# Nishad-Sharma/gpuRaytracer

Measured on AMD Instinct MI355X. Metric: Msamples/sec (pixels×spp) Cornell box 1080p at 1/2/4/8 MI355X; HBM GB/s, higher is better.
Workload: dtype f32; 1 GPU; cornell_1920x1080_256spp_b3; width=1920, height=1080, spp_per_gpu=256, spp_frame=256, bounces=3, parallelism=single GPU

## Files before the change

gpuraytracer_amd/_native.py:

```python
from __future__ import annotations

import ctypes
import os

ABI_VERSION = 11
_HERE = os.path.dirname(os.path.abspath(__file__))
library_path = os.environ.get("RTPT_LIB") or os.path.join(_HERE, "librtpt.so")


class float3(ctypes.Structure):

    _fields_ = [("x", ctypes.c_float), ("y", ctypes.c_float), ("z", ctypes.c_float),
                ("_pad", ctypes.c_float)]

    def __iter__(self):
        return iter((self.x, self.y, self.z))


class float4(ctypes.Structure):
    _fields_ = [("x", ctypes.c_float), ("y", ctypes.c_float), ("z", ctypes.c_float),
                ("w", ctypes.c_float)]


class int2(ctypes.Structure):
# ... 43 lines not shown
                ("device", ctypes.c_int32)]


class RenderParamsC(ctypes.Structure):
    _fields_ = [(n, ctypes.c_uint32) for n in
                ("spp", "bounces", "sample_base", "row_start", "row_step", "row_count",
                 "accumulate", "flags")]


class SceneInfo(ctypes.Structure):
    _fields_ = [(n, ctypes.c_uint32) for n in
                ("n_triangles", "n_triangle_pairs", "n_spheres", "lds_bytes",
                 "n_sphere_nodes", "n_triangle_bvh_nodes", "n_box_clusters", "pair_free_mask",
                 "sphere_kernel_lds_bytes", "kernel_layout", "kernel_lds_bytes")]


class CreateOptions(ctypes.Structure):
    _fields_ = [("scene_layout", ctypes.c_uint32), ("lanes_per_pixel", ctypes.c_uint32),
                ("tri_bvh_build", ctypes.c_uint32), ("tri_leaf_max", ctypes.c_uint32),
                ("tri_leaf_cost", ctypes.c_float), ("sphere_leaf_max", ctypes.c_uint32),
                ("sphere_median", ctypes.c_uint32), ("walk_scheduler", ctypes.c_uint32),
                ("walk_leaf_den", ctypes.c_uint32), ("reserved", ctypes.c_uint32 * 7)]


assert ctypes.sizeof(CreateOptions) == 64

LAYOUTS = {"auto": 0, "pairs": 1, "single": 2, "global": 3, "smem": 3, "pairsmem": 4, "sorted": 5, "bvh": 6}
TRI_BUILDS = {"default": 0, "host": 1, "lbvh": 2, "gpusah": 3}
WALKS = {"auto": 0, "lockstep": 1, "free": 2, "sorted": 3}

RT_OK = 0
RT_OUT_DEVICE, RT_OUT_FP16, RT_OUT_NONE, RT_KEEP_SUM, RT_OUT_RGBA8 = 0x1, 0x2, 0x4, 0x8, 0x10
RT_RAYS_ANY, RT_RAYS_EXACT = 0x100, 0x200
RT_AOV_CENTER = 0x400
RT_RAYS_CHUNK = 2048
RT_MAX_BOUNCES = 4
RT_COMM_ID_BYTES = 128
STATUS = {0: "RT_OK", 1: "RT_ERR_INVALID_ARG", 2: "RT_ERR_NO_DEVICE", 3: "RT_ERR_OUT_OF_MEMORY",
          4: "RT_ERR_LAUNCH", 5: "RT_ERR_STATE", 6: "RT_ERR_COMM"}

class LaunchInfo(ctypes.Structure):
    _fields_ = [("kernel", ctypes.c_char * 96)] + [(n, ctypes.c_uint32) for n in
                ("lanes_per_pixel", "halton_tables", "small_index", "block_threads", "grid_x",
                 "grid_y", "lds_bytes")]

    def as_dict(self) -> dict:
        d = {k: getattr(self, k) for k, _ in self._fields_}
        d["kernel"] = self.kernel.decode()
        return d


class BuildStats(ctypes.Structure):
    _fields_ = [("tri_bvh_build", ctypes.c_uint32), ("tri_bvh_nodes", ctypes.c_uint32),
                ("tri_bvh_build_ms", ctypes.c_float), ("scene_compile_ms", ctypes.c_float),
                ("tri_bvh_temp_kib", ctypes.c_uint32)]


class TriBvhDump(ctypes.Structure):
    _fields_ = [("n_triangles", ctypes.c_uint32), ("nodes_per_layout", ctypes.c_uint32),
                ("leaf_max", ctypes.c_uint32), ("margin", ctypes.c_float),
                ("nodes", ctypes.c_void_p), ("sorted", ctypes.c_void_p),
                ("perm", ctypes.c_void_p), ("isect", ctypes.c_void_p)]


assert ctypes.sizeof(TriBvhDump) == 48

RT_UPDATE_REBUILD = 0x1


class UpdateStats(ctypes.Structure):
    _fields_ = [("tri_bvh", ctypes.c_uint32), ("updates", ctypes.c_uint32), ("compile_ms", ctypes.c_float),
                ("upload_ms", ctypes.c_float), ("tri_bvh_ms", ctypes.c_float), ("total_ms", ctypes.c_float),
                ("reserved", ctypes.c_uint32 * 2)]


assert ctypes.sizeof(UpdateStats) == 32


class TileLayout(ctypes.Structure):
    _fields_ = [("rows", ctypes.c_uint32), ("rows_max", ctypes.c_uint32),
                ("row_bytes", ctypes.c_uint64), ("tile_bytes", ctypes.c_uint64)]


class Ray(ctypes.Structure):
    _fields_ = [("origin", ctypes.c_float * 3), ("tmin", ctypes.c_float),
                ("dir", ctypes.c_float * 3), ("tmax", ctypes.c_float)]


class RayHit(ctypes.Structure):
    _fields_ = [("t", ctypes.c_float), ("id", ctypes.c_int32)]


class RayDomainInfo(ctypes.Structure):
    _fields_ = [(n, ctypes.c_float) for n in ("origin_max", "dir_len2_min", "dir_len2_max", "tmax_max")]


assert ctypes.sizeof(Ray) == 32 and ctypes.sizeof(RayHit) == 8 and Ray.dir.offset == 16


class PathParamsC(ctypes.Structure):
    _fields_ = [("spp", ctypes.c_uint32), ("bounces", ctypes.c_uint32), ("sample_base", ctypes.c_uint32),
                ("lanes_per_ray", ctypes.c_uint32), ("seed_key", ctypes.c_uint64), ("flags", ctypes.c_uint32),
                ("reserved", ctypes.c_uint32)]


assert ctypes.sizeof(PathParamsC) == 32 and PathParamsC.seed_key.offset == 16 and PathParamsC.flags.offset == 24


class AovParams(ctypes.Structure):
    _fields_ = [(n, ctypes.c_uint32) for n in
                ("spp", "sample_base", "row_start", "row_step", "row_count", "flags")]


class AovBuffers(ctypes.Structure):
    _fields_ = [("albedo", ctypes.c_void_p), ("normal_depth", ctypes.c_void_p),
                ("first_hit", ctypes.c_void_p)]


assert ctypes.sizeof(AovParams) == 24 and ctypes.sizeof(AovBuffers) == 24


class DenoiseParams(ctypes.Structure):
    _fields_ = [("iterations", ctypes.c_uint32), ("normal_power_log2", ctypes.c_uint32),
                ("sigma_luminance", ctypes.c_float), ("sigma_depth", ctypes.c_float),
                ("depth_floor", ctypes.c_float), ("flags", ctypes.c_uint32), ("reserved", ctypes.c_uint32 * 2)]


class DenoiseBuffers(ctypes.Structure):
    _fields_ = [(n, ctypes.c_void_p) for n in ("color_a", "color_b", "albedo", "normal_depth", "out")]


assert ctypes.sizeof(DenoiseParams) == 32 and ctypes.sizeof(DenoiseBuffers) == 40 and DenoiseBuffers.out.offset == 32


RT_PLAN_RELATIVE = 0x800


class PlanParams(ctypes.Structure):
    _fields_ = [("budget", ctypes.c_uint64), ("count_min", ctypes.c_uint32), ("count_max", ctypes.c_uint32),
                ("luminance_floor", ctypes.c_float), ("radius", ctypes.c_uint32), ("rows", ctypes.c_uint32),
                ("flags", ctypes.c_uint32), ("reserved", ctypes.c_uint32 * 2)]


class PlanStats(ctypes.Structure):
    _fields_ = [("weight_sum", ctypes.c_uint64), ("samples", ctypes.c_uint64),
                ("count_max_seen", ctypes.c_uint32), ("at_cap", ctypes.c_uint32),
                ("reserved", ctypes.c_uint32 * 2)]

    def as_dict(self) -> dict:
        return {k: int(getattr(self, k)) for k, _ in self._fields_ if k != "reserved"}


assert ctypes.sizeof(PlanParams) == 40 and ctypes.sizeof(PlanStats) == 32


class MisParamsC(ctypes.Structure):
    _fields_ = [(n, ctypes.c_uint32) for n in
                ("camera_rays", "mis_samples", "row_start", "row_step", "row_count", "flags")]


MATH_FNS = {n: k for k, n in enumerate(
    ("sin", "cos", "log", "exp", "pow_gamma", "sqrt", "rcp", "f2h", "h2f", "tonemap", "mis_unit",
     "halton_loop", "halton_small", "halton_tab"))}
RT_MATH_HOST, RT_MATH_DEVICE = 0, 1
RT_MATH_VALUES_MAX = 1 << 24

_P = ctypes.c_void_p
SIGNATURES = {
    "rt_create": (ctypes.c_int, [ctypes.POINTER(SceneDesc), ctypes.POINTER(_P)]),
    "rt_create_ex": (ctypes.c_int, [ctypes.POINTER(SceneDesc), ctypes.POINTER(CreateOptions),
                                    ctypes.POINTER(_P)]),
    "rt_create_options_default": (None, [ctypes.POINTER(CreateOptions)]),
    "rt_set_seeds": (ctypes.c_int, [_P, _P, ctypes.c_int32, ctypes.c_int32]),
    "rt_fill_seeds": (ctypes.c_int, [_P, ctypes.c_uint64]),
    "rt_render": (ctypes.c_int, [_P, ctypes.POINTER(RenderParamsC), _P]),
    "rt_render_async": (ctypes.c_int, [_P, ctypes.POINTER(RenderParamsC), _P, _P]),
    "rt_trace_rays": (ctypes.c_int, [_P, _P, ctypes.c_uint64, ctypes.c_uint32, _P]),
    "rt_trace_rays_async": (ctypes.c_int, [_P, _P, ctypes.c_uint64, ctypes.c_uint32, _P, _P]),
    "rt_path_params_default": (None, [ctypes.POINTER(PathParamsC)]),
    "rt_trace_paths": (ctypes.c_int, [_P, ctypes.POINTER(PathParamsC), _P, _P, ctypes.c_uint64, _P, _P]),
    "rt_trace_paths_async": (ctypes.c_int, [_P, ctypes.POINTER(PathParamsC), _P, _P, ctypes.c_uint64, _P, _P, _P]),
    "rt_render_aov": (ctypes.c_int, [_P, ctypes.POINTER(AovParams), ctypes.POINTER(AovBuffers)]),
    "rt_render_aov_async": (ctypes.c_int, [_P, ctypes.POINTER(AovParams), ctypes.POINTER(AovBuffers), _P]),
    "rt_denoise_params_default": (None, [ctypes.POINTER(DenoiseParams)]),
    "rt_denoise": (ctypes.c_int, [_P, ctypes.POINTER(DenoiseParams), ctypes.POINTER(DenoiseBuffers)]),
    "rt_denoise_async": (ctypes.c_int, [_P, ctypes.POINTER(DenoiseParams), ctypes.POINTER(DenoiseBuffers), _P]),
    "rt_render_counts": (ctypes.c_int, [_P, ctypes.POINTER(RenderParamsC), _P, _P, _P]),
    "rt_render_counts_async": (ctypes.c_int, [_P, ctypes.POINTER(RenderParamsC), _P, _P, _P, _P]),
    "rt_plan_params_default": (None, [ctypes.POINTER(PlanParams)]),
    "rt_plan_samples": (ctypes.c_int, [_P, ctypes.POINTER(PlanParams), _P, _P, _P, ctypes.POINTER(PlanStats)]),
    "rt_plan_samples_async": (ctypes.c_int, [_P, ctypes.POINTER(PlanParams), _P, _P, _P, _P, _P]),
    "rt_plan_samples_host": (ctypes.c_int, [ctypes.c_int32, ctypes.POINTER(PlanParams), _P, _P, _P,
                                            ctypes.POINTER(PlanStats)]),
    "rt_debug_ray_domain": (ctypes.c_int, [ctypes.POINTER(SceneDesc), ctypes.POINTER(RayDomainInfo)]),
    "rt_last_kernel_ms": (ctypes.c_int, [_P, ctypes.POINTER(ctypes.c_float)]),
    "rt_destroy": (ctypes.c_int, [_P]),
    "rt_last_launch": (ctypes.c_int, [_P, ctypes.POINTER(LaunchInfo)]),
    "rt_build_info": (ctypes.c_int, [_P, ctypes.POINTER(BuildStats)]),
    "rt_debug_tri_bvh": (ctypes.c_int, [_P, ctypes.POINTER(TriBvhDump)]),
    "rt_debug_tri_bvh_host": (ctypes.c_int, [ctypes.POINTER(SceneDesc), ctypes.POINTER(CreateOptions),
                                             ctypes.POINTER(TriBvhDump)]),
    "rt_update_scene": (ctypes.c_int, [_P, ctypes.POINTER(SceneDesc), ctypes.c_uint32]),
    "rt_update_info": (ctypes.c_int, [_P, ctypes.POINTER(UpdateStats)]),
    "rt_debug_tri_bvh_refit_host": (ctypes.c_int, [ctypes.POINTER(SceneDesc), ctypes.POINTER(CreateOptions),
                                                   ctypes.POINTER(SceneDesc), ctypes.POINTER(TriBvhDump)]),
    "rt_math_selfcheck": (ctypes.c_int, [ctypes.POINTER(ctypes.c_uint64)]),
    "rt_debug_math_values": (ctypes.c_int, [ctypes.c_uint32, ctypes.c_uint32, _P, ctypes.c_uint64, _P]),
    "rt_debug_math_sums": (ctypes.c_int, [ctypes.c_uint32, ctypes.c_uint32, ctypes.c_uint32, ctypes.c_uint64,
                                          ctypes.c_uint32, ctypes.c_uint32, _P]),
    "rt_comm_unique_id": (ctypes.c_int, [_P]),
    "rt_comm_init": (ctypes.c_int, [_P, ctypes.c_int32, ctypes.c_int32, _P]),
    "rt_render_gather": (ctypes.c_int, [_P, ctypes.POINTER(RenderParamsC), _P, _P]),
    "rt_comm_info": (ctypes.c_int, [_P, ctypes.POINTER(ctypes.c_int32), ctypes.POINTER(ctypes.c_int32)]),
    "rt_tile_layout": (ctypes.c_int, [ctypes.c_int32, ctypes.c_int32, ctypes.c_int32, ctypes.c_int32,
                                      ctypes.c_uint32, ctypes.POINTER(TileLayout)]),
    "rt_place_tiles": (ctypes.c_int, [_P, _P, ctypes.c_int32, ctypes.c_uint32, _P, _P]),
    "rt_place_tiles_host": (ctypes.c_int, [_P, ctypes.c_int32, ctypes.c_int32, ctypes.c_int32,
                                           ctypes.c_uint32, _P]),
    "rt_build_sha": (ctypes.c_char_p, []),
    "rt_debug_stats": (ctypes.c_int, [_P, _P, ctypes.c_int]),
    "rt_last_error": (ctypes.c_char_p, [_P]),
    "rt_status_string": (ctypes.c_char_p, [ctypes.c_int]),
    "rt_abi_version": (ctypes.c_int, []),
    "rt_seed_splitmix": (None, [ctypes.c_uint64, _P, ctypes.c_size_t]),
    "rt_scene_cornell_box": (ctypes.c_int, [ctypes.c_int32, ctypes.c_int32,
                                            ctypes.POINTER(CameraGPU),
                                            ctypes.POINTER(MaterialGPU),
                                            ctypes.POINTER(float3),
                                            ctypes.POINTER(SquareLightGPU),
                                            ctypes.POINTER(ctypes.c_uint32)]),
    "rt_scene_random_spheres": (ctypes.c_int, [ctypes.c_int32, ctypes.c_int32, ctypes.c_uint32,
                                               ctypes.c_uint64, ctypes.POINTER(CameraGPU),
                                               ctypes.POINTER(MaterialGPU),
                                               ctypes.POINTER(float3),
                                               ctypes.POINTER(SquareLightGPU),
                                               ctypes.POINTER(ctypes.c_uint32),
                                               ctypes.POINTER(SphereGPU)]),
    "rt_render_mis": (ctypes.c_int, [_P, ctypes.POINTER(MisParamsC), _P, _P]),
    "rt_scene_cornell_box_mis": (ctypes.c_int, [ctypes.c_int32, ctypes.c_int32,
                                                ctypes.POINTER(CameraGPU),
                                                ctypes.POINTER(MaterialGPU),
                                                ctypes.POINTER(float3),
                                                ctypes.POINTER(SquareLightGPU),
                                                ctypes.POINTER(ctypes.c_uint32)]),
    "rt_tonemap_rgba8": (None, [_P, ctypes.c_size_t, _P]),
    "rt_scene_describe": (ctypes.c_int, [ctypes.POINTER(SceneDesc), ctypes.POINTER(SceneInfo)]),
    "rt_scene_describe_ex": (ctypes.c_int, [ctypes.POINTER(SceneDesc), ctypes.POINTER(CreateOptions),
                                            ctypes.POINTER(SceneInfo)]),
    "rt_debug_camera_candidates": (ctypes.c_int, [ctypes.POINTER(SceneDesc)] + [ctypes.c_int32] * 4 + [_P]),
    "rt_debug_shadow_candidates": (ctypes.c_int, [ctypes.POINTER(SceneDesc)] + [ctypes.c_int32] * 4 +
                                   [_P, ctypes.POINTER(ctypes.c_int32)]),
    "rt_debug_cluster_kinds": (ctypes.c_int, [ctypes.POINTER(SceneDesc), ctypes.POINTER(ctypes.c_uint32),
                                              ctypes.c_uint32, ctypes.POINTER(ctypes.c_uint32)]),
    "rt_debug_light_mask": (ctypes.c_int, [ctypes.POINTER(SceneDesc), ctypes.POINTER(ctypes.c_uint64), _P,
                                           ctypes.c_uint32]),
    "rt_debug_halton_table": (ctypes.c_int, [_P, ctypes.c_uint32, ctypes.POINTER(ctypes.c_uint32), _P, _P]),
    "rt_debug_halton_table_device": (ctypes.c_int, [_P, _P, ctypes.c_uint32]),
}


class RtError(RuntimeError):

    def __init__(self, status: int, message: str):
        super().__init__(f"{STATUS.get(status, status)}: {message}")
        self.status = status


def _preload_hip_runtime():
    if os.environ.get("RTPT_SYSTEM_HIP") == "1":
        return
    import importlib.util
    spec = importlib.util.find_spec("torch")
    if spec is None or not spec.submodule_search_locations:
        return
    for d in spec.submodule_search_locations:
        cand = os.path.join(d, "lib", "libamdhip64.so")
        if os.path.exists(cand):
            ctypes.CDLL(cand, mode=ctypes.RTLD_GLOBAL)
            return


def _load():
    if not os.path.exists(library_path):
        raise ImportError(
            f"{library_path} is missing: build the HIP extension first "
            "(`make` or `python -c 'import __graft_entry__ as g; g.build()'`). "
            "There is no CPU fallback.")
    _preload_hip_runtime()
    handle = ctypes.CDLL(library_path)
    for name, (res, args) in SIGNATURES.items():
        fn = getattr(handle, name)
        fn.restype = res
        fn.argtypes = args
    if handle.rt_abi_version() != ABI_VERSION:
        raise ImportError(f"librtpt.so ABI {handle.rt_abi_version()} != {ABI_VERSION}")
    if not os.environ.get("RTPT_LIB"):
        from .srchash import have_sources, kernel_source_sha
        built = handle.rt_build_sha().decode()
        if not have_sources() or built == "unknown":
            import warnings
            warnings.warn(f"{library_path}: source hash not checked (library hash {built!r}, "
                          f"sources {'present' if have_sources() else 'absent'})")
        elif built != kernel_source_sha():
            raise ImportError(f"{library_path} was built from other sources (hash {built}, "
                              f"tree {kernel_source_sha()}): rebuild it with `make`")
    return handle


lib = _load()
```

gpuraytracer_amd/csrc/rt_api.cpp:

```cpp
#include <rccl/rccl.h>

#include <stdio.h>
#include <stdlib.h>
#include <string.h>

#include <chrono>
#include <new>
#include <vector>

#include "rt_api_internal.hpp"

using namespace rtapi;

namespace {

class DevBuf {
public:
    DevBuf() = default;
    DevBuf(DevBuf&& o) noexcept : p_(o.p_), bytes_(o.bytes_) { o.p_ = nullptr; o.bytes_ = 0; }
    DevBuf& operator=(DevBuf&& o) noexcept {
        std::swap(p_, o.p_);
        std::swap(bytes_, o.bytes_);
        return *this;
    }
    ~DevBuf() { reset(); }

    void reset() {
        if (p_) (void)hipFree(p_);
        p_ = nullptr;
        bytes_ = 0;
    }
    hipError_t reserve(size_t bytes) { return bytes_ >= bytes ? hipSuccess : allocate(bytes); }
    hipError_t resize_exact(size_t bytes) { return bytes_ == bytes ? hipSuccess : allocate(bytes); }
    void adopt(void* p, size_t bytes) {
        reset();
        p_ = p;
        bytes_ = bytes;
    }
    template <typename T>
    T* as() const { return static_cast<T*>(p_); }
    size_t bytes() const { return bytes_; }
    explicit operator bool() const { return p_ != nullptr; }

private:
    hipError_t allocate(size_t bytes) {
        reset();
        if (bytes == 0) return hipSuccess;
        const hipError_t e = hipMalloc(&p_, bytes);
        if (e != hipSuccess) p_ = nullptr;
        else bytes_ = bytes;
        return e;
    }
    void* p_ = nullptr;
    size_t bytes_ = 0;
};

template <typename H, hipError_t (*Destroy)(H)>
struct Owned {
    H h = nullptr;
    Owned() = default;
    Owned(const Owned&) = delete;
    Owned& operator=(const Owned&) = delete;
    ~Owned() { if (h) (void)Destroy(h); }
    operator H() const { return h; }
};
using Stream = Owned<hipStream_t, hipStreamDestroy>;
using Event = Owned<hipEvent_t, hipEventDestroy>;

enum SceneArray {
    kTriIsect, kTriShade, kPairIsect, kClusters, kSphLds, kSphLdsId,
    kSphBox,
    kSphIsect, kSphShade, kSphNodes, kSphPerm, kMisShade, kSceneArrays
};

}

struct rt_ctx {
    int device = 0;
    Stream stream;
    Event ev0, ev1;
    Event ev_u0, ev_u1;
    Event ev_tiles;
    rt::CompiledScene scene;
    DevBuf d_scene[kSceneArrays];
    DevBuf d_tri_nodes;
    uint32_t tri_build = kDefaultTriBuild;
    DevBuf d_tri_sorted, d_tri_perm;
    DevBuf d_refit;
    uint32_t tri_bvh_nodes = 0;
    rt::SceneTables tab{};
    bool sph_compact = false;
    uint64_t light_mask = 0;
    DevBuf d_halton_tab;
    uint32_t tri_bvh_build_used = 0;
    uint32_t tri_leaf_max = 1;
    float tri_bvh_build_ms = 0.0f;
    size_t tri_bvh_temp_bytes = 0;
    float scene_compile_ms = 0.0f;
    DevBuf d_mis_tab;
    uint32_t mis_tab_S = 0;
    DevBuf d_mis_part;
    DevBuf d_out, d_out8;
    DevBuf d_rays, d_hits;
    DevBuf d_ray_seeds, d_radiance;
    DevBuf d_aov[3];
    DevBuf d_den[6];
    DevBuf d_counts, d_totals;
    DevBuf d_plan_in[2];
    DevBuf d_plan;
    DevBuf d_seeds;
    bool seeds_ready = false;
    uint32_t seed_max = 0xFFFFFFFFu;
    DevBuf d_sum;
    bool sum_valid = false;
    uint32_t sum_row_start = 0, sum_row_step = 0, sum_row_count = 0;
    uint32_t sum_first = 0, sum_samples = 0;
    bool sum_counts = false;
    bool timed = false;
    rt::LaunchInfo launch{};
    bool launched = false;
    ncclComm_t comm = nullptr;
    int rank = 0, world = 1;
    DevBuf d_tile;
    DevBuf d_gather;
    bool tiles_pending = false;
    uint32_t lanes = 0;
    rt::SceneMem scene_mem = rt::SceneMem::kAuto;
    uint32_t walk = 0;
    uint32_t walk_leaf_den = 0;
    uint32_t tri_leaf_opt = rt::kTriLeafMax;
    double tri_leaf_cost = 1.0;
    rt::BuildOptions build_opt;
    std::string broken;
    bool updated = false;
    rt_update_stats update{};
    std::string err;

    ~rt_ctx() {
        if (tiles_pending) (void)hipEventSynchronize(ev_tiles);
        if (comm) (void)ncclCommDestroy(comm);
    }
};

namespace {
thread_local std::string g_create_err = "no error";
}

int rtapi::fail(rt_ctx* ctx, int status, const std::string& msg) {
    if (ctx)
        ctx->err = msg;
    else
        g_create_err = msg;
    return status;
}

namespace {

int nccl_fail(rt_ctx* ctx, const char* what, ncclResult_t r) {
    return fail(ctx, RT_ERR_COMM, std::string(what) + ": " + ncclGetErrorString(r));
}

struct DeviceGuard {
    int prev = -1;
    explicit DeviceGuard(int dev) {
        if (hipGetDevice(&prev) != hipSuccess) prev = -1;
        if (prev != dev) (void)hipSetDevice(dev);
    }
    ~DeviceGuard() {
        int cur = -1;
        if (prev >= 0 && hipGetDevice(&cur) == hipSuccess && cur != prev) (void)hipSetDevice(prev);
    }
};

int reserve(rt_ctx* c, DevBuf& b, size_t bytes, const char* what) {
    const hipError_t e = b.reserve(bytes);
    return e == hipSuccess ? RT_OK : hip_fail(c, RT_ERR_OUT_OF_MEMORY, what, e);
}

int copy_down(rt_ctx* c, void* host, const void* dev, size_t bytes, hipStream_t stream, const char* what) {
    const hipError_t e = hipMemcpyAsync(host, dev, bytes, hipMemcpyDeviceToHost, stream);
    return e == hipSuccess ? RT_OK : hip_fail(c, RT_ERR_LAUNCH, what, e);
}

hipError_t upload(DevBuf& b, const void* src, size_t bytes, hipStream_t s) {
    hipError_t e = b.resize_exact(bytes);
    if (e != hipSuccess || bytes == 0) return e;
    if ((e = hipMemcpyAsync(b.as<void>(), src, bytes, hipMemcpyHostToDevice, s)) != hipSuccess) return e;
    return hipStreamSynchronize(s);
}

template <typename F>
int timed_launch(rt_ctx* c, hipStream_t stream, const char* what, rt::LaunchInfo* info, F launch) {
    (void)hipEventRecord(c->ev0, stream);
    const hipError_t e = launch(info);
    if (e != hipSuccess) return hip_fail(c, RT_ERR_LAUNCH, (std::string(what) + " launch").c_str(), e);
    if (info) c->launched = true;
    (void)hipEventRecord(c->ev1, stream);
    c->timed = true;
    return RT_OK;
}

template <typename P>
void set_camera(P* K, const rt::CamConst& cam) {
    memcpy(K->cam_pos, cam.pos, sizeof(K->cam_pos));
    memcpy(K->cam_u, cam.u, sizeof(K->cam_u));
    memcpy(K->cam_v, cam.v, sizeof(K->cam_v));
    memcpy(K->cam_w, cam.w, sizeof(K->cam_w));
    K->halfW = cam.halfW;
    K->halfH = cam.halfH;
    K->W = cam.W;
    K->H = cam.H;
}

uint32_t halton_max_index(const rt_ctx* c, uint32_t sample_base, uint32_t spp) {
    const uint64_t imax = (uint64_t)c->seed_max + sample_base + (spp ? spp - 1u : 0u);
    return imax > 0xFFFFFFFFull ? 0xFFFFFFFFu : (uint32_t)imax;
}

int check_out_format(rt_ctx* c, uint32_t flags) {
    if ((flags & RT_OUT_FP16) && (flags & RT_OUT_RGBA8))
        return fail(c, RT_ERR_INVALID_ARG, "RT_OUT_FP16 and RT_OUT_RGBA8 are exclusive");
    return RT_OK;
}

void set_tables(rt::KParams* K, const rt::SceneTables& t) {
    K->tri_isect = t.tri_isect;
    K->pair_isect = t.pair_isect;
    K->clusters = t.clusters;
    K->sph_isect = t.sph_isect;
    K->sph_nodes = t.sph_nodes;
    K->sph_perm = t.sph_perm;
    K->sph_box = t.sph_box;
    K->tri_nodes = t.tri_nodes;
    K->tri_sorted = t.tri_sorted;
    K->tri_perm = t.tri_perm;
    K->nT = t.nT;
    K->nP = t.nP;
    K->nS = t.nS;
    K->nN = t.nN;
    K->nTN = t.nTN;
    K->nC = t.nC;
    K->pair_free = t.pair_free;
}

void set_scene(rt::KParams* K, const rt_ctx* c) {
    memset(K, 0, sizeof(*K));
    set_tables(K, c->tab);
    K->tri_shade = c->d_scene[kTriShade].as<float4>();
    K->light_mask = c->light_mask;
    K->halton_tab = c->d_halton_tab.as<float>();
    K->sph_lds = c->sph_compact ? c->d_scene[kSphLds].as<uint32_t>() : nullptr;
    K->sph_lds_id = c->d_scene[kSphLdsId].as<uint16_t>();
    K->sph_shade = c->d_scene[kSphShade].as<float4>();
    K->nE = c->scene.sph_lds_entries;
    memcpy(K->light_center, c->scene.light.center, sizeof(K->light_center));
    {
        uint32_t by, bz;
        memcpy(&by, &K->light_center[1], 4);
        memcpy(&bz, &K->light_center[2], 4);
        K->light_plain = (by != 0x80000000u && bz != 0x80000000u) ? 1u : 0u;
    }
    memcpy(K->light_color, c->scene.light.color, sizeof(K->light_color));
}

hipError_t upload_scene(rt_ctx* c) {
    const rt::CompiledScene& s = c->scene;
    hipError_t e = hipSuccess;
    auto put = [&](SceneArray k, const auto& v) {
        const size_t bytes = v.size() * sizeof(v[0]);
        DevBuf& b = c->d_scene[k];
        if (e == hipSuccess) e = b.resize_exact(bytes);
        if (e == hipSuccess && bytes)
            e = hipMemcpyAsync(b.as<void>(), v.data(), bytes, hipMemcpyHostToDevice, c->stream);
    };
    put(kTriIsect, s.tri_isect);
    put(kTriShade, s.tri_shade);
    put(kPairIsect, s.pair_isect);
    put(kClusters, s.clusters);
    put(kSphLds, s.sph_lds);
    put(kSphLdsId, s.sph_lds_id);
    put(kSphBox, s.sph_box);
    put(kSphIsect, s.sph_isect);
    put(kSphShade, s.sph_shade);
    put(kSphNodes, s.sph_nodes);
    put(kSphPerm, s.sph_perm);
    put(kMisShade, s.mis_shade);
    return e != hipSuccess ? e : hipStreamSynchronize(c->stream);
}

bool needs_tri_bvh(const rt_ctx* c) { return rtapi::needs_tri_bvh(scene_counts(c->scene, 0), c->scene_mem); }

void free_tri_bvh(rt_ctx* c) {
    c->d_tri_nodes.reset();
    c->d_tri_sorted.reset();
    c->d_tri_perm.reset();
    c->d_refit.reset();
    c->tri_bvh_nodes = 0;
    c->tri_bvh_build_used = 0;
    c->tri_bvh_temp_bytes = 0;
}

int build_tri_bvh(rt_ctx* c, std::string* msg) {
    using clk = std::chrono::steady_clock;
    free_tri_bvh(c);
    const rt::CompiledScene& s = c->scene;
    const uint32_t nT = (uint32_t)s.tri_isect.size();
    const size_t nn = 2 * (size_t)nT - 1;
    const auto t_build = clk::now();
    hipError_t e;
    if (c->tri_build == RT_TRI_BVH_GPU_SAH || c->tri_build == RT_TRI_BVH_GPU_LBVH) {
        if ((e = c->d_tri_nodes.reserve(rt::kTriCompactLayouts * nn * sizeof(uint4))) != hipSuccess ||
            (e = c->d_tri_sorted.reserve(3 * (size_t)nT * sizeof(float4))) != hipSuccess ||
            (e = c->d_tri_perm.reserve((size_t)nT * sizeof(uint32_t))) != hipSuccess) {
            *msg = std::string("hipMalloc(triangle BVH): ") + hipGetErrorString(e);
            return RT_ERR_OUT_OF_MEMORY;
        }
    }
    const float4* d_tri = c->d_scene[kTriIsect].as<float4>();
    uint4* d_nodes = c->d_tri_nodes.as<uint4>();
    float4* d_sorted = c->d_tri_sorted.as<float4>();
    uint32_t* d_perm = c->d_tri_perm.as<uint32_t>();
    if (c->tri_build == RT_TRI_BVH_GPU_SAH) {
        uint32_t total = 0;
        size_t temp = 0;
        if ((e = rt::build_tri_gsah(d_tri, nT, s.margin, c->tri_leaf_opt, c->tri_leaf_cost, d_nodes, d_sorted, d_perm,
                                    &total, &temp, c->stream)) != hipSuccess) {
            *msg = std::string("triangle BVH build: ") + hipGetErrorString(e);
            return (e == hipErrorInvalidValue) ? RT_ERR_INVALID_ARG
                   : (e == hipErrorOutOfMemory) ? RT_ERR_OUT_OF_MEMORY : RT_ERR_LAUNCH;
        }
        c->tri_bvh_nodes = total;
        c->tri_bvh_temp_bytes = temp;
    } else if (c->tri_build == RT_TRI_BVH_GPU_LBVH) {
        if ((e = rt::build_tri_lbvh(d_tri, nT, s.tri_lo, s.tri_hi, s.margin, d_nodes, d_sorted, d_perm, c->stream)) !=
            hipSuccess) {
            *msg = std::string("triangle BVH build: ") + hipGetErrorString(e);
            return (e == hipErrorInvalidValue) ? RT_ERR_INVALID_ARG : RT_ERR_LAUNCH;
        }
        c->tri_bvh_nodes = (uint32_t)nn;
    } else {
        std::vector<uint32_t> nodes, perm;
        std::vector<rt::TriIsect> sorted;
        if (!rt::build_tri_sah(s.tri_isect, s.margin, &nodes, &sorted, &perm, c->tri_leaf_opt, c->tri_leaf_cost)) {
            *msg = "triangle BVH build: too many triangles (2^24)";
            return RT_ERR_INVALID_ARG;
        }
        if ((e = upload(c->d_tri_nodes, nodes.data(), nodes.size() * sizeof(uint32_t), c->stream)) != hipSuccess ||
            (e = upload(c->d_tri_sorted, sorted.data(), sorted.size() * sizeof(rt::TriIsect), c->stream)) != hipSuccess ||
            (e = upload(c->d_tri_perm, perm.data(), perm.size() * sizeof(uint32_t), c->stream)) != hipSuccess) {
            *msg = std::string("triangle BVH upload: ") + hipGetErrorString(e);
            return RT_ERR_OUT_OF_MEMORY;
        }
        c->tri_bvh_nodes = (uint32_t)(nodes.size() / (4 * rt::kTriCompactLayouts));
    }
    c->tri_leaf_max = c->tri_build == RT_TRI_BVH_GPU_LBVH ? 1u : tri_leaf_clamp(c->tri_leaf_opt);
    c->tri_bvh_build_used = c->tri_build;
    c->tri_bvh_build_ms = std::chrono::duration<float, std::milli>(clk::now() - t_build).count();
    return RT_OK;
}

void finish_scene(rt_ctx* c) {
    c->sph_compact = rt::sphere_compact_usable(c->scene);
    c->light_mask = rt::light_mask(c->scene);
    rt::SceneTables& t = c->tab = scene_counts(c->scene, c->tri_bvh_nodes);
    t.tri_isect = c->d_scene[kTriIsect].as<float4>();
    t.pair_isect = c->d_scene[kPairIsect].as<float4>();
    t.clusters = c->d_scene[kClusters].as<float4>();
    t.sph_isect = c->d_scene[kSphIsect].as<float4>();
    t.sph_nodes = c->d_scene[kSphNodes].as<float4>();
    t.sph_perm = c->d_scene[kSphPerm].as<uint32_t>();
    t.sph_box = c->sph_compact ? c->d_scene[kSphBox].as<uint4>() : nullptr;
    t.tri_nodes = c->d_tri_nodes.as<uint4>();
    t.tri_sorted = c->d_tri_sorted.as<float4>();
    t.tri_perm = c->d_tri_perm.as<uint32_t>();
}

bool resolve_rows(const rt_ctx* c, uint32_t row_start, uint32_t row_step, uint32_t row_count, uint32_t* start,
                  uint32_t* step, uint32_t* count) {
    const uint32_t H = (uint32_t)c->scene.cam.H;
    *start = row_start;
    *step = row_step ? row_step : 1u;
    if (*start >= H) return false;
    const uint32_t avail = (H - 1u - *start) / *step + 1u;
    *count = row_count ? row_count : avail;
    return *count <= avail;
}

struct CountsArgs {
    const uint32_t* counts;
    uint32_t* totals;
};

int render_impl(rt_ctx* c, const rt_render_params* p, void* out, bool out_is_device,
                hipStream_t stream, bool sync, const CountsArgs* ca = nullptr) {
    if (!p) return fail(c, RT_ERR_INVALID_ARG, "params is null");
    if (ca && !ca->counts) return fail(c, RT_ERR_INVALID_ARG, "rt_render_counts: counts is null");
    if (!c->broken.empty()) return fail(c, RT_ERR_STATE, c->broken);
    if (p->bounces > RT_MAX_BOUNCES)
        return fail(c, RT_ERR_INVALID_ARG,
                    "bounces > 4: Halton dimensions would leave primes[24] (sampling.metal:97)");
    if (!c->seeds_ready) return fail(c, RT_ERR_STATE, "seeds not set (rt_set_seeds/rt_fill_seeds)");
    uint32_t start, step, count;
    if (!resolve_rows(c, p->row_start, p->row_step, p->row_count, &start, &step, &count))
        return fail(c, RT_ERR_INVALID_ARG, "row partition outside the frame");
    const bool want_out = !(p->flags & RT_OUT_NONE);
    const bool keep_sum = (p->flags & RT_KEEP_SUM) != 0;
    const bool sums = keep_sum || p->accumulate;
    if (want_out && !out) return fail(c, RT_ERR_INVALID_ARG, "out is null");
    if (p->accumulate) {
        const bool rows_same = c->sum_valid && c->sum_row_start == start && c->sum_row_step == step &&
                               c->sum_row_count == count;
        if (ca) {
            if (!rows_same || c->sum_first != p->sample_base)
                return fail(c, RT_ERR_STATE,
                            "rt_render_counts: accumulate: context sum does not start at sample_base for these rows "
                            "(render with RT_KEEP_SUM first)");
        } else {
            if (rows_same && c->sum_counts)
                return fail(c, RT_ERR_STATE,
                            "accumulate: context sum holds per-pixel sample counts (rt_render_counts): "
                            "continue it with rt_render_counts");
            if (!rows_same || (uint64_t)c->sum_first + c->sum_samples != (uint64_t)p->sample_base)
                return fail(c, RT_ERR_STATE,
                            "accumulate: context sum does not end at sample_base for these rows "
                            "(render with RT_KEEP_SUM first)");
        }
    }
    const uint64_t total = (uint64_t)(p->accumulate ? c->sum_samples : 0u) + p->spp;
    if (ca) {
        if (total > (1ull << 24))
            return fail(c, RT_ERR_INVALID_ARG,
                        "rt_render_counts: the bound of the per-pixel totals (the caps spp of the calls into this "
                        "sum) must stay <= 2^24");
    } else if (total == 0 || total > 0xFFFFFFFFull) {
        return fail(c, RT_ERR_INVALID_ARG, "samples in the sum must be in [1, 2^32)");
    }

    const size_t pixels = (size_t)count * (size_t)c->scene.cam.W;
    int st;
    if ((st = check_out_format(c, p->flags)) != RT_OK) return st;
    const size_t out_bytes = pixels * pixel_bytes(p->flags);
    if (sums) {
        if (c->d_sum.bytes() < pixels * sizeof(float4)) c->sum_valid = false;
        if ((st = reserve(c, c->d_sum, pixels * sizeof(float4), "hipMalloc(sum)")) != RT_OK) return st;
    }
    void* kout = want_out ? out : nullptr;
    if (want_out && !out_is_device) {
        if ((st = reserve(c, c->d_out, out_bytes, "hipMalloc(out staging)")) != RT_OK) return st;
        kout = c->d_out.as<void>();
    }
    const uint32_t* kcounts = ca ? ca->counts : nullptr;
    uint32_t* ktotals = ca ? ca->totals : nullptr;
    if (ca && !out_is_device) {
        if ((st = reserve(c, c->d_counts, pixels * sizeof(uint32_t), "hipMalloc(counts staging)")) != RT_OK) return st;
        const hipError_t e = hipMemcpyAsync(c->d_counts.as<void>(), ca->counts, pixels * sizeof(uint32_t),
                                            hipMemcpyHostToDevice, stream);
        if (e != hipSuccess) return hip_fail(c, RT_ERR_LAUNCH, "hipMemcpyAsync(counts)", e);
        kcounts = c->d_counts.as<uint32_t>();
        if (ca->totals) {
            if ((st = reserve(c, c->d_totals, pixels * sizeof(uint32_t), "hipMalloc(totals staging)")) != RT_OK)
                return st;
            ktotals = c->d_totals.as<uint32_t>();
        }
    }

    rt::KParams K;
    set_scene(&K, c);
    K.seeds = c->d_seeds.as<uint32_t>();
    K.sum = sums ? c->d_sum.as<float4>() : nullptr;
    K.out = kout;
    set_camera(&K, c->scene.cam);
    K.spp = p->spp;
    K.sample_base = p->sample_base;
    K.row_start = start;
    K.row_step = step;
    K.row_count = count;
    K.accumulate = p->accumulate ? 1u : 0u;
    K.samples_total = (uint32_t)total;
    K.flags = ((p->flags & RT_OUT_FP16) ? rt::kOutFp16 : 0u) | ((p->flags & RT_OUT_RGBA8) ? rt::kOutRgba8 : 0u);
    K.lanes = c->lanes;
    K.walk = c->walk;
    K.walk_leaf_den = c->walk_leaf_den;
    K.max_index = halton_max_index(c, p->sample_base, ca ? (uint32_t)total : p->spp);

    if (keep_sum && !p->accumulate) c->sum_valid = false;
    if ((st = timed_launch(c, stream, ca ? "path_counts" : "path_trace", &c->launch, [&](rt::LaunchInfo* info) {
             return ca ? rt::launch_path_counts(K, kcounts, ktotals, p->bounces, c->scene_mem, stream, info)
                       : rt::launch_path_trace(K, p->bounces, c->scene_mem, stream, info);
         })) != RT_OK)
        return st;
    if (sums) {
        c->sum_valid = true;
        c->sum_row_start = start;
        c->sum_row_step = step;
        c->sum_row_count = count;
        if (!p->accumulate) c->sum_first = p->sample_base;
        c->sum_samples = (uint32_t)total;
        c->sum_counts = ca != nullptr;
    }
    if (ca && ca->totals && !out_is_device &&
        (st = copy_down(c, ca->totals, ktotals, pixels * sizeof(uint32_t), stream, "hipMemcpyAsync(totals)")) != RT_OK)
        return st;
    if (want_out && !out_is_device &&
        (st = copy_down(c, out, kout, out_bytes, stream, "hipMemcpyAsync(out)")) != RT_OK)
        return st;
    if (sync) {
        hipError_t e;
        if ((e = hipStreamSynchronize(stream)) != hipSuccess)
            return hip_fail(c, RT_ERR_LAUNCH, "path_trace execution", e);
        uint32_t short_end = 0;
        if (rt::lds_check_result(&short_end) == hipSuccess && short_end)
            return fail(c, RT_ERR_LAUNCH, "LDS overflow: staged records end at byte " + std::to_string(short_end) +
                                              ", past the dispatch's dynamic LDS");
    }
    return RT_OK;
}

int place_tiles_impl(rt_ctx* c, const void* gathered, uint32_t N, uint32_t flags, void* frame,
                     hipStream_t stream) {
    const uint32_t W = (uint32_t)c->scene.cam.W, H = (uint32_t)c->scene.cam.H;
    const TileLayout L = tile_layout(W, H, N, 0, flags);
    const bool dev = (flags & RT_OUT_DEVICE) != 0;
    const size_t frame_bytes = (size_t)H * L.row_bytes;
    void* dst = frame;
    int st;
    if (!dev) {
        if ((st = reserve(c, c->d_out, frame_bytes, "hipMalloc(frame staging)")) != RT_OK) return st;
        dst = c->d_out.as<void>();
    }
    hipError_t e = rt::launch_place_tiles(gathered, dst, L.row_bytes, L.tile_bytes, H, N, stream);
    if (e != hipSuccess) return hip_fail(c, RT_ERR_LAUNCH, "place_tiles launch", e);
    if (!dev) {
        if ((e = hipStreamSynchronize(stream)) != hipSuccess ||
            (e = hipMemcpyAsync(frame, dst, frame_bytes, hipMemcpyDeviceToHost, stream)) != hipSuccess ||
            (e = hipStreamSynchronize(stream)) != hipSuccess)
            return hip_fail(c, RT_ERR_LAUNCH, "frame copy to host", e);
    }
    return RT_OK;
}

int render_gather_impl(rt_ctx* c, const rt_render_params* p, void* frame, hipStream_t stream) {
    if (!p) return fail(c, RT_ERR_INVALID_ARG, "params is null");
    if (!c->comm) return fail(c, RT_ERR_STATE, "no communicator (rt_comm_init)");
    if (p->row_start || p->row_step > 1 || p->row_count)
        return fail(c, RT_ERR_INVALID_ARG, "rt_render_gather partitions the rows itself: "
                                           "params must name the whole frame (row_start 0, "
                                           "row_step 0 or 1, row_count 0)");
    int st;
    if ((st = check_out_format(c, p->flags)) != RT_OK) return st;
    const bool want_out = !(p->flags & RT_OUT_NONE);
    const bool dev = (p->flags & RT_OUT_DEVICE) != 0;
    if (want_out && c->rank == 0 && !frame) return fail(c, RT_ERR_INVALID_ARG, "frame is null on rank 0");
    const uint32_t H = (uint32_t)c->scene.cam.H, W = (uint32_t)c->scene.cam.W, N = (uint32_t)c->world;
    const TileLayout L = tile_layout(W, H, N, (uint32_t)c->rank, p->flags);
    hipError_t e;
    if (c->tiles_pending && (e = hipStreamWaitEvent(stream, c->ev_tiles, 0)) != hipSuccess)
        return hip_fail(c, RT_ERR_LAUNCH, "hipStreamWaitEvent(previous gather)", e);
    if (want_out && (st = reserve(c, c->d_tile, L.tile_bytes, "hipMalloc(tile)")) != RT_OK) return st;
    if (L.rows > 0) {
        rt_render_params q = *p;
        q.row_start = (uint32_t)c->rank;
        q.row_step = N;
        q.row_count = L.rows;
        q.flags = p->flags | RT_OUT_DEVICE;
        if ((st = render_impl(c, &q, c->d_tile.as<void>(), true, stream, false)) != RT_OK) return st;
    }
    if (!want_out) return RT_OK;
    if (c->rank == 0 && (st = reserve(c, c->d_gather, L.tile_bytes * N, "hipMalloc(gather)")) != RT_OK) return st;
    ncclResult_t r = ncclGather(c->d_tile.as<void>(), c->rank == 0 ? c->d_gather.as<void>() : nullptr, L.tile_bytes,
                                ncclUint8, 0, c->comm, stream);
    if (r != ncclSuccess) return nccl_fail(c, "ncclGather", r);
    if (c->rank == 0 && (st = place_tiles_impl(c, c->d_gather.as<void>(), N, p->flags, frame, stream)) != RT_OK)
        return st;
    if ((e = hipEventRecord(c->ev_tiles, stream)) != hipSuccess)
        return hip_fail(c, RT_ERR_LAUNCH, "hipEventRecord(gather)", e);
    c->tiles_pending = true;
    if (!dev) {
        e = hipStreamSynchronize(stream);
        if (e != hipSuccess) return hip_fail(c, RT_ERR_COMM, "render+gather execution", e);
    }
    return RT_OK;
}

int mis_table(rt_ctx* c, uint32_t S) {
    if (c->d_mis_tab && c->mis_tab_S == S) return RT_OK;
    std::vector<float> t((size_t)S * 12u);
    for (uint32_t i = 0; i < S; ++i) {
        float* q = &t[(size_t)i * 12u];
        q[0] = halton_host(i, 0);
        q[1] = halton_host(i, 1);
        q[2] = 0.0f;
        q[3] = 0.0f;
        q[4] = halton_host(i + S, 2);
        q[5] = halton_host(i + S, 3);
        q[6] = halton_host(i, 6);
        q[7] = halton_host(i, 7);
        q[8] = halton_host(i + 2 * S, 4);
        q[9] = halton_host(i + 2 * S, 5);
        q[10] = halton_host(i + S, 6);
        q[11] = halton_host(i + S, 7);
    }
    c->d_mis_tab.reset();
    c->mis_tab_S = 0;
    hipError_t e = upload(c->d_mis_tab, t.data(), t.size() * sizeof(float), c->stream);
    if (e != hipSuccess) return hip_fail(c, RT_ERR_OUT_OF_MEMORY, "MIS table upload", e);
    c->mis_tab_S = S;
    return RT_OK;
}

int render_mis_impl(rt_ctx* c, const rt_mis_params* p, float* out, uint8_t* out8) {
    if (!p) return fail(c, RT_ERR_INVALID_ARG, "params is null");
    if (!c->broken.empty()) return fail(c, RT_ERR_STATE, c->broken);
    if (!out && !out8) return fail(c, RT_ERR_INVALID_ARG, "both outputs are null");
    if (!c->scene.sph_isect.empty())
        return fail(c, RT_ERR_INVALID_ARG,
                    "the MIS integrator traces triangle scenes only (shaders.metal:459-509)");
    if (c->scene.tri_isect.empty()) return fail(c, RT_ERR_INVALID_ARG, "scene has no triangles");
    if (p->camera_rays == 0) return fail(c, RT_ERR_INVALID_ARG, "camera_rays must be >= 1");
    if (p->mis_samples < 3 || p->mis_samples / 3u > (1u << 20))
        return fail(c, RT_ERR_INVALID_ARG, "mis_samples must be in [3, 3 * 2^20]");
    uint32_t start, step, count;
    if (!resolve_rows(c, p->row_start, p->row_step, p->row_count, &start, &step, &count))
        return fail(c, RT_ERR_INVALID_ARG, "row partition outside the frame");
    const uint32_t S = p->mis_samples / 3u;
    int st = mis_table(c, S);
    if (st != RT_OK) return st;
    const bool dev = (p->flags & RT_OUT_DEVICE) != 0;
    const size_t pixels = (size_t)count * (size_t)c->scene.cam.W;
    float4* kout = reinterpret_cast<float4*>(out);
    uchar4* kout8 = reinterpret_cast<uchar4*>(out8);
    if (out && !dev) {
        if ((st = reserve(c, c->d_out, pixels * 16u, "hipMalloc(out staging)")) != RT_OK) return st;
        kout = c->d_out.as<float4>();
    }
    if (out8 && !dev) {
        if ((st = reserve(c, c->d_out8, pixels * 4u, "hipMalloc(out8 staging)")) != RT_OK) return st;
        kout8 = c->d_out8.as<uchar4>();
    }

    rt::MisParams K;
    memset(&K, 0, sizeof(K));
    K.tab = c->tab;
    K.mis_shade = c->d_scene[kMisShade].as<float4>();
// ... 315 lines not shown
    K.count_min = p->count_min;
    K.count_max = p->count_max;
    K.luminance_floor = p->luminance_floor;
    K.radius = p->radius;
    K.W = c->scene.cam.W;
    K.rows = (int32_t)rows;
    K.flags = p->flags & RT_PLAN_RELATIVE;
    if ((st = timed_launch(c, stream, "plan", &c->launch,
                           [&](rt::LaunchInfo* info) { return rt::launch_plan(K, stream, info); })) != RT_OK)
        return st;
    if (!dev && (st = copy_down(c, counts, kcounts, cnt_bytes, stream, "hipMemcpyAsync(counts)")) != RT_OK) return st;
    if (stats) {
        e = hipMemcpyAsync(stats, K.acc, sizeof(rt_plan_stats), sync ? hipMemcpyDeviceToHost : hipMemcpyDeviceToDevice,
                           stream);
        if (e != hipSuccess) return hip_fail(c, RT_ERR_LAUNCH, "hipMemcpyAsync(plan stats)", e);
    }
    if (sync && (e = hipStreamSynchronize(stream)) != hipSuccess)
        return hip_fail(c, RT_ERR_LAUNCH, "plan execution", e);
    return RT_OK;
}

}

extern "C" {

const char* rt_last_error(const rt_ctx* ctx) {
    return ctx ? ctx->err.c_str() : g_create_err.c_str();
}

int rt_create(const rt_scene_desc* d, rt_ctx** out_ctx) { return rt_create_ex(d, nullptr, out_ctx); }

int rt_create_ex(const rt_scene_desc* d, const rt_create_options* opt, rt_ctx** out_ctx) {
    if (!out_ctx) return fail(nullptr, RT_ERR_INVALID_ARG, "out_ctx is null");
    *out_ctx = nullptr;
    if (!d) return fail(nullptr, RT_ERR_INVALID_ARG, "scene desc is null");
    if (!d->camera) return fail(nullptr, RT_ERR_INVALID_ARG, "camera is null");
    if (!d->square_lights || d->n_square_lights < 1)
        return fail(nullptr, RT_ERR_INVALID_ARG, "square_lights[0] is required (raytrace.metal:22)");
    Resolved ro;
    const char* why = nullptr;
    if (!resolve_options(opt, &ro, &why)) return fail(nullptr, RT_ERR_INVALID_ARG, why);
    int count = 0;
    hipError_t e = hipGetDeviceCount(&count);
    if (e != hipSuccess || count <= 0)
        return fail(nullptr, RT_ERR_NO_DEVICE,
                    std::string("no HIP device: ") + (e != hipSuccess ? hipGetErrorString(e) : "count 0"));
    if (d->device < 0 || d->device >= count)
        return fail(nullptr, RT_ERR_NO_DEVICE, "device ordinal out of range");

    rt_ctx* c = new (std::nothrow) rt_ctx();
    if (!c) return fail(nullptr, RT_ERR_OUT_OF_MEMORY, "host allocation");
    c->device = d->device;
    c->lanes = ro.lanes;
    c->tri_build = ro.tri_build;
    c->scene_mem = ro.mem;
    c->walk = ro.walk;
    c->walk_leaf_den = ro.walk_leaf_den;
    c->tri_leaf_opt = ro.tri_leaf_max;
    c->tri_leaf_cost = ro.tri_leaf_cost;
    c->build_opt = ro.build;
    DeviceGuard g(c->device);
    const char* err = nullptr;
    using clk = std::chrono::steady_clock;
    const auto t_compile = clk::now();
    if (!compile_desc(d, ro.build, &c->scene, &err)) {
        delete c;
        return fail(nullptr, RT_ERR_INVALID_ARG, err);
    }
    c->scene_compile_ms = std::chrono::duration<float, std::milli>(clk::now() - t_compile).count();
    int status = RT_OK;
    std::string msg;
    do {
        if ((e = hipStreamCreateWithFlags(&c->stream.h, hipStreamNonBlocking)) != hipSuccess) {
            status = RT_ERR_NO_DEVICE; msg = std::string("hipStreamCreate: ") + hipGetErrorString(e); break;
        }
        if ((e = hipEventCreate(&c->ev0.h)) != hipSuccess || (e = hipEventCreate(&c->ev1.h)) != hipSuccess ||
            (e = hipEventCreateWithFlags(&c->ev_tiles.h, hipEventDisableTiming)) != hipSuccess) {
            status = RT_ERR_NO_DEVICE; msg = std::string("hipEventCreate: ") + hipGetErrorString(e); break;
        }
        if ((e = upload_scene(c)) != hipSuccess) {
            status = RT_ERR_OUT_OF_MEMORY; msg = std::string("scene upload: ") + hipGetErrorString(e); break;
        }
        if (needs_tri_bvh(c) && (status = build_tri_bvh(c, &msg)) != RT_OK) break;
        const size_t npx = (size_t)c->scene.cam.W * (size_t)c->scene.cam.H;
        if ((e = c->d_seeds.reserve(npx * sizeof(uint32_t))) != hipSuccess) {
            status = RT_ERR_OUT_OF_MEMORY; msg = std::string("hipMalloc(seeds): ") + hipGetErrorString(e); break;
        }
        if ((e = c->d_halton_tab.resize_exact(sizeof(float) * rt::kHaltonTabLdsFloats)) != hipSuccess) {
            status = RT_ERR_OUT_OF_MEMORY; msg = std::string("hipMalloc(halton tables): ") + hipGetErrorString(e); break;
        }
        if ((e = rt::launch_fill_halton_tables(c->d_halton_tab.as<float>(), c->stream)) != hipSuccess ||
            (e = hipStreamSynchronize(c->stream)) != hipSuccess) {
            status = RT_ERR_LAUNCH; msg = std::string("halton tables: ") + hipGetErrorString(e); break;
        }
    } while (0);
    if (status != RT_OK) {
        delete c;
        return fail(nullptr, status, msg);
    }
    finish_scene(c);
    *out_ctx = c;
    return RT_OK;
}

int rt_destroy(rt_ctx* c) {
    if (!c) return RT_OK;
    DeviceGuard g(c->device);
    delete c;
    return RT_OK;
}

int rt_update_scene(rt_ctx* c, const rt_scene_desc* d, uint32_t flags) {
    static_assert(sizeof(rt_update_stats) == 32, "rt_update_stats layout");
    if (!c) return fail(nullptr, RT_ERR_INVALID_ARG, "ctx is null");
    if (!d) return fail(c, RT_ERR_INVALID_ARG, "rt_update_scene: scene is null");
    if (!d->camera) return fail(c, RT_ERR_INVALID_ARG, "rt_update_scene: camera is null");
    if (!d->square_lights || d->n_square_lights < 1)
        return fail(c, RT_ERR_INVALID_ARG, "rt_update_scene: square_lights[0] is required");
    if (flags & ~(uint32_t)RT_UPDATE_REBUILD) return fail(c, RT_ERR_INVALID_ARG, "rt_update_scene: unknown bits in flags");
    if (d->n_triangles != c->scene.tri_isect.size())
        return fail(c, RT_ERR_INVALID_ARG, "rt_update_scene: n_triangles differs from the context's (" +
                                               std::to_string(c->scene.tri_isect.size()) + ")");
    if (d->n_spheres != c->scene.sph_shade.size())
        return fail(c, RT_ERR_INVALID_ARG, "rt_update_scene: n_spheres differs from the context's (" +
                                               std::to_string(c->scene.sph_shade.size()) + ")");
    if (d->camera->resolution.x != c->scene.cam.W || d->camera->resolution.y != c->scene.cam.H)
        return fail(c, RT_ERR_INVALID_ARG, "rt_update_scene: camera resolution differs from the context's");
    if (d->device != c->device) return fail(c, RT_ERR_INVALID_ARG, "rt_update_scene: device differs from the context's");
    using clk = std::chrono::steady_clock;
    auto ms_since = [](clk::time_point t) { return std::chrono::duration<float, std::milli>(clk::now() - t).count(); };
    const auto t_all = clk::now();
    rt::CompiledScene next;
    const char* err = nullptr;
    if (!compile_desc(d, c->build_opt, &next, &err))
        return fail(c, RT_ERR_INVALID_ARG, std::string("rt_update_scene: ") + err);
    if (next.tri_isect.size() != c->scene.tri_isect.size() || next.sph_shade.size() != c->scene.sph_shade.size())
        return fail(c, RT_ERR_INVALID_ARG, "rt_update_scene: the compiled scene changed its primitive counts");
    rt_update_stats st{};
    st.compile_ms = ms_since(t_all);

    DeviceGuard g(c->device);
    auto broken = [&](int status, const std::string& what) {
        c->broken = "the context holds a half-updated scene (" + what + "): rt_update_scene must succeed first";
        return fail(c, status, "rt_update_scene: " + what);
    };
    hipError_t e;
    if (c->tiles_pending) (void)hipEventSynchronize(c->ev_tiles);
    if ((e = hipStreamSynchronize(c->stream)) != hipSuccess) return broken(RT_ERR_LAUNCH, std::string("stream: ") + hipGetErrorString(e));
    if (!c->ev_u0.h && ((e = hipEventCreate(&c->ev_u0.h)) != hipSuccess || (e = hipEventCreate(&c->ev_u1.h)) != hipSuccess))
        return broken(RT_ERR_OUT_OF_MEMORY, std::string("hipEventCreate: ") + hipGetErrorString(e));
    c->broken = "rt_update_scene in progress";
    c->sum_valid = false;
    c->scene = std::move(next);
    const auto t_up = clk::now();
    if ((e = upload_scene(c)) != hipSuccess) return broken(RT_ERR_OUT_OF_MEMORY, std::string("scene upload: ") + hipGetErrorString(e));
    st.upload_ms = ms_since(t_up);

    const bool need = needs_tri_bvh(c), have = c->tri_bvh_build_used && c->d_tri_nodes;
    const auto t_bvh = clk::now();
    if (need && have && !(flags & RT_UPDATE_REBUILD)) {
        uint32_t* table = c->d_refit.as<uint32_t>();
        bool table_made = false;
        e = rt::refit_tri_bvh(c->d_scene[kTriIsect].as<float4>(), (uint32_t)c->scene.tri_isect.size(), c->scene.margin,
                              c->d_tri_nodes.as<uint4>(), c->tri_bvh_nodes, c->d_tri_sorted.as<float4>(),
                              c->d_tri_perm.as<uint32_t>(), &table, &table_made, c->ev_u0, c->ev_u1, c->stream);
        if (table_made) c->d_refit.adopt(table, rt::tri_refit_table_bytes(c->tri_bvh_nodes));
        if (e == hipSuccess) e = hipStreamSynchronize(c->stream);
        if (e != hipSuccess)
            return broken(e == hipErrorOutOfMemory ? RT_ERR_OUT_OF_MEMORY : RT_ERR_LAUNCH,
                          std::string("triangle BVH refit: ") + hipGetErrorString(e));
        uint32_t bad = 0;
        if (table_made && ((e = rt::refit_format_errors(table, c->tri_bvh_nodes, &bad)) != hipSuccess || bad))
            return broken(RT_ERR_LAUNCH, "triangle BVH refit: the tree is outside the format of its builders");
        if ((e = hipEventElapsedTime(&st.tri_bvh_ms, c->ev_u0, c->ev_u1)) != hipSuccess)
            return broken(RT_ERR_LAUNCH, std::string("hipEventElapsedTime: ") + hipGetErrorString(e));
        st.tri_bvh = 1;
    } else if (need) {
        std::string msg;
        const int status = build_tri_bvh(c, &msg);
        if (status != RT_OK) return broken(status == RT_ERR_INVALID_ARG ? RT_ERR_LAUNCH : status, msg);
        st.tri_bvh_ms = ms_since(t_bvh);
        st.tri_bvh = 2;
        c->scene_compile_ms = st.compile_ms;
    } else {
        free_tri_bvh(c);
    }
    finish_scene(c);
    c->broken.clear();
    st.updates = c->update.updates + 1;
    st.total_ms = ms_since(t_all);
    c->update = st;
    c->updated = true;
    return RT_OK;
}

int rt_update_info(const rt_ctx* c, rt_update_stats* info) {
    if (!c || !info) return fail(nullptr, RT_ERR_INVALID_ARG, "null argument");
    if (!c->updated)
        return fail(const_cast<rt_ctx*>(c), RT_ERR_STATE, "rt_update_info: no successful rt_update_scene on this context yet");
    *info = c->update;
    return RT_OK;
}

int rt_set_seeds(rt_ctx* c, const uint32_t* seeds, int32_t width, int32_t height) {
    if (!c) return fail(nullptr, RT_ERR_INVALID_ARG, "ctx is null");
    if (!seeds) return fail(c, RT_ERR_INVALID_ARG, "seeds is null");
    if (width != c->scene.cam.W || height != c->scene.cam.H)
        return fail(c, RT_ERR_INVALID_ARG, "seed texture size must equal the camera resolution");
    DeviceGuard g(c->device);
    const size_t bytes = (size_t)width * (size_t)height * sizeof(uint32_t);
    hipError_t e = hipMemcpyAsync(c->d_seeds.as<void>(), seeds, bytes, hipMemcpyHostToDevice, c->stream);
    if (e == hipSuccess) e = hipStreamSynchronize(c->stream);
    if (e != hipSuccess) return hip_fail(c, RT_ERR_LAUNCH, "seed upload", e);
    uint32_t mx = 0;
    for (size_t k = 0, n = (size_t)width * (size_t)height; k < n; ++k) mx = seeds[k] > mx ? seeds[k] : mx;
    c->seed_max = mx;
    c->seeds_ready = true;
    return RT_OK;
}

int rt_fill_seeds(rt_ctx* c, uint64_t key) {
    if (!c) return fail(nullptr, RT_ERR_INVALID_ARG, "ctx is null");
    DeviceGuard g(c->device);
    const uint64_t n = (uint64_t)c->scene.cam.W * (uint64_t)c->scene.cam.H;
    hipError_t e = rt::launch_fill_seeds(c->d_seeds.as<uint32_t>(), key, n, c->stream);
    if (e == hipSuccess) e = hipStreamSynchronize(c->stream);
    if (e != hipSuccess) return hip_fail(c, RT_ERR_LAUNCH, "fill_seeds", e);
    c->seed_max = 0xFFFFFu;
    c->seeds_ready = true;
    return RT_OK;
}

int rt_render(rt_ctx* c, const rt_render_params* p, void* out) {
    if (!c) return fail(nullptr, RT_ERR_INVALID_ARG, "ctx is null");
    DeviceGuard g(c->device);
    const bool dev = p && (p->flags & RT_OUT_DEVICE);
    return render_impl(c, p, out, dev, c->stream, true);
}

int rt_render_async(rt_ctx* c, const rt_render_params* p, void* out_device, void* hip_stream) {
    if (!c) return fail(nullptr, RT_ERR_INVALID_ARG, "ctx is null");
    DeviceGuard g(c->device);
    return render_impl(c, p, out_device, true, (hipStream_t)hip_stream, false);
}

int rt_render_mis(rt_ctx* ctx, const rt_mis_params* params, float* out_rgba32f, uint8_t* out_rgba8) {
    if (!ctx) return fail(nullptr, RT_ERR_INVALID_ARG, "ctx is null");
    DeviceGuard g(ctx->device);
    return render_mis_impl(ctx, params, out_rgba32f, out_rgba8);
}

int rt_trace_rays(rt_ctx* c, const rt_ray* rays, uint64_t n, uint32_t flags, rt_ray_hit* hits) {
    if (!c) return fail(nullptr, RT_ERR_INVALID_ARG, "ctx is null");
    DeviceGuard g(c->device);
    return trace_rays_impl(c, rays, n, flags, hits, (flags & RT_OUT_DEVICE) != 0, c->stream, true);
}

int rt_trace_rays_async(rt_ctx* c, const rt_ray* rays_dev, uint64_t n, uint32_t flags, rt_ray_hit* hits_dev,
                        void* hip_stream) {
    if (!c) return fail(nullptr, RT_ERR_INVALID_ARG, "ctx is null");
    DeviceGuard g(c->device);
    return trace_rays_impl(c, rays_dev, n, flags, hits_dev, true, (hipStream_t)hip_stream, false);
}

int rt_trace_paths(rt_ctx* c, const rt_path_params* p, const rt_ray* rays, const uint32_t* seeds, uint64_t n,
                   float* radiance, rt_ray_hit* first_hits) {
    if (!c) return fail(nullptr, RT_ERR_INVALID_ARG, "ctx is null");
    DeviceGuard g(c->device);
    return trace_paths_impl(c, p, rays, seeds, n, radiance, first_hits, p && (p->flags & RT_OUT_DEVICE), c->stream,
                            true);
}

int rt_trace_paths_async(rt_ctx* c, const rt_path_params* p, const rt_ray* rays_dev, const uint32_t* seeds_dev,
                         uint64_t n, float* radiance_dev, rt_ray_hit* first_hits_dev, void* hip_stream) {
    if (!c) return fail(nullptr, RT_ERR_INVALID_ARG, "ctx is null");
    DeviceGuard g(c->device);
    return trace_paths_impl(c, p, rays_dev, seeds_dev, n, radiance_dev, first_hits_dev, true, (hipStream_t)hip_stream,
                            false);
}

int rt_render_aov(rt_ctx* c, const rt_aov_params* p, const rt_aov_buffers* b) {
    if (!c) return fail(nullptr, RT_ERR_INVALID_ARG, "ctx is null");
    DeviceGuard g(c->device);
    return render_aov_impl(c, p, b, p && (p->flags & RT_OUT_DEVICE), c->stream, true);
}

int rt_render_aov_async(rt_ctx* c, const rt_aov_params* p, const rt_aov_buffers* b_dev, void* hip_stream) {
    if (!c) return fail(nullptr, RT_ERR_INVALID_ARG, "ctx is null");
    DeviceGuard g(c->device);
    return render_aov_impl(c, p, b_dev, true, (hipStream_t)hip_stream, false);
}

int rt_denoise(rt_ctx* c, const rt_denoise_params* p, const rt_denoise_buffers* b) {
    if (!c) return fail(nullptr, RT_ERR_INVALID_ARG, "ctx is null");
    DeviceGuard g(c->device);
    return denoise_impl(c, p, b, p && (p->flags & RT_OUT_DEVICE), c->stream, true);
}

int rt_denoise_async(rt_ctx* c, const rt_denoise_params* p, const rt_denoise_buffers* b_dev, void* hip_stream) {
    if (!c) return fail(nullptr, RT_ERR_INVALID_ARG, "ctx is null");
    DeviceGuard g(c->device);
    return denoise_impl(c, p, b_dev, true, (hipStream_t)hip_stream, false);
}

int rt_render_counts(rt_ctx* c, const rt_render_params* p, const uint32_t* counts, void* out, uint32_t* totals) {
    if (!c) return fail(nullptr, RT_ERR_INVALID_ARG, "ctx is null");
    DeviceGuard g(c->device);
    const CountsArgs ca{counts, totals};
    return render_impl(c, p, out, p && (p->flags & RT_OUT_DEVICE), c->stream, true, &ca);
}

int rt_render_counts_async(rt_ctx* c, const rt_render_params* p, const uint32_t* counts_dev, void* out_dev,
                           uint32_t* totals_dev, void* hip_stream) {
    if (!c) return fail(nullptr, RT_ERR_INVALID_ARG, "ctx is null");
    DeviceGuard g(c->device);
    const CountsArgs ca{counts_dev, totals_dev};
    return render_impl(c, p, out_dev, true, (hipStream_t)hip_stream, false, &ca);
}

int rt_plan_samples(rt_ctx* c, const rt_plan_params* p, const float* first, const float* all, uint32_t* counts,
                    rt_plan_stats* stats) {
    if (!c) return fail(nullptr, RT_ERR_INVALID_ARG, "ctx is null");
    DeviceGuard g(c->device);
    return plan_impl(c, p, first, all, counts, stats, p && (p->flags & RT_OUT_DEVICE), c->stream, true);
}

int rt_plan_samples_async(rt_ctx* c, const rt_plan_params* p, const float* first_dev, const float* all_dev,
                          uint32_t* counts_dev, rt_plan_stats* stats_dev, void* hip_stream) {
    if (!c) return fail(nullptr, RT_ERR_INVALID_ARG, "ctx is null");
    DeviceGuard g(c->device);
    return plan_impl(c, p, first_dev, all_dev, counts_dev, stats_dev, true, (hipStream_t)hip_stream, false);
}

int rt_last_kernel_ms(rt_ctx* c, float* ms) {
    if (!c || !ms) return fail(c, RT_ERR_INVALID_ARG, "null argument");
    if (!c->timed) return fail(c, RT_ERR_STATE, "no render or ray query yet");
    DeviceGuard g(c->device);
    hipError_t e = hipEventSynchronize(c->ev1);
    if (e == hipSuccess) e = hipEventElapsedTime(ms, c->ev0, c->ev1);
    if (e != hipSuccess) return hip_fail(c, RT_ERR_LAUNCH, "hipEventElapsedTime", e);
    return RT_OK;
}

int rt_comm_unique_id(uint8_t id[RT_COMM_ID_BYTES]) {
    if (!id) return fail(nullptr, RT_ERR_INVALID_ARG, "id is null");
    static_assert(sizeof(ncclUniqueId) == RT_COMM_ID_BYTES, "ncclUniqueId size");
    ncclUniqueId u;
    const ncclResult_t r = ncclGetUniqueId(&u);
    if (r != ncclSuccess) return nccl_fail(nullptr, "ncclGetUniqueId", r);
    memcpy(id, &u, sizeof(u));
    return RT_OK;
}

int rt_comm_init(rt_ctx* c, int32_t rank, int32_t world, const uint8_t id[RT_COMM_ID_BYTES]) {
    if (!c) return fail(nullptr, RT_ERR_INVALID_ARG, "ctx is null");
    if (!id) return fail(c, RT_ERR_INVALID_ARG, "id is null");
    if (world < 1 || rank < 0 || rank >= world)
        return fail(c, RT_ERR_INVALID_ARG, "need 0 <= rank < world");
    if (c->comm) return fail(c, RT_ERR_STATE, "context already has a communicator");
    DeviceGuard g(c->device);
    ncclUniqueId u;
    memcpy(&u, id, sizeof(u));
    ncclComm_t comm = nullptr;
    const ncclResult_t r = ncclCommInitRank(&comm, world, u, rank);
    if (r != ncclSuccess) return nccl_fail(c, "ncclCommInitRank", r);
    c->comm = comm;
    c->rank = rank;
    c->world = world;
    return RT_OK;
}

int rt_render_gather(rt_ctx* c, const rt_render_params* p, void* frame, void* hip_stream) {
    if (!c) return fail(nullptr, RT_ERR_INVALID_ARG, "ctx is null");
    DeviceGuard g(c->device);
    hipStream_t s = (hipStream_t)hip_stream;
    return render_gather_impl(c, p, frame, s);
}

int rt_comm_info(const rt_ctx* c, int32_t* count, int32_t* rank) {
    if (!c || !count || !rank) return fail(nullptr, RT_ERR_INVALID_ARG, "null argument");
    rt_ctx* m = const_cast<rt_ctx*>(c);
    if (!c->comm) return fail(m, RT_ERR_STATE, "rt_comm_info: no communicator (rt_comm_init first)");
    int n = 0, r = 0;
    ncclResult_t res = ncclCommCount(c->comm, &n);
    if (res != ncclSuccess) return nccl_fail(m, "ncclCommCount", res);
    res = ncclCommUserRank(c->comm, &r);
    if (res != ncclSuccess) return nccl_fail(m, "ncclCommUserRank", res);
    *count = n;
    *rank = r;
    return RT_OK;
}

int rt_place_tiles(rt_ctx* c, const void* gathered_device, int32_t world, uint32_t flags, void* frame,
                   void* hip_stream) {
    if (!c) return fail(nullptr, RT_ERR_INVALID_ARG, "ctx is null");
    if (!gathered_device || !frame || world < 1) return fail(c, RT_ERR_INVALID_ARG, "null buffer or world < 1");
    if (const int st = check_out_format(c, flags)) return st;
    DeviceGuard g(c->device);
    hipStream_t s = (hipStream_t)hip_stream;
    return place_tiles_impl(c, gathered_device, (uint32_t)world, flags, frame, s);
}

int rt_build_info(const rt_ctx* c, rt_build_stats* info) {
    if (!c || !info) return fail(nullptr, RT_ERR_INVALID_ARG, "null argument");
    memset(info, 0, sizeof(*info));
    info->tri_bvh_build = c->tri_bvh_build_used;
    info->tri_bvh_nodes = c->tri_bvh_nodes;
    info->tri_bvh_build_ms = c->tri_bvh_build_ms;
    info->scene_compile_ms = c->scene_compile_ms;
    info->tri_bvh_temp_kib = (uint32_t)((c->tri_bvh_temp_bytes + 1023) / 1024);
    return RT_OK;
}

int rt_debug_tri_bvh(const rt_ctx* c, rt_tri_bvh_dump* dump) {
    if (!c || !dump) return fail(nullptr, RT_ERR_INVALID_ARG, "null argument");
    if (!c->broken.empty()) return fail(const_cast<rt_ctx*>(c), RT_ERR_STATE, c->broken);
    if (!c->tri_bvh_build_used || !c->d_tri_nodes) return RT_ERR_STATE;
    const size_t nT = c->scene.tri_isect.size(), nn = c->tri_bvh_nodes;
    dump->n_triangles = (uint32_t)nT;
    dump->nodes_per_layout = (uint32_t)nn;
    dump->leaf_max = c->tri_leaf_max;
    dump->margin = c->scene.margin;
    DeviceGuard g(c->device);
    const struct { void* dst; const DevBuf& src; size_t bytes; } copies[4] = {
        {dump->nodes, c->d_tri_nodes, rt::kTriCompactLayouts * nn * sizeof(uint4)},
        {dump->sorted, c->d_tri_sorted, nT * sizeof(rt::TriIsect)},
        {dump->perm, c->d_tri_perm, nT * sizeof(uint32_t)},
        {dump->isect, c->d_scene[kTriIsect], nT * sizeof(rt::TriIsect)}};
    for (const auto& cp : copies) {
        if (!cp.dst) continue;
        const hipError_t e = hipMemcpy(cp.dst, cp.src.as<void>(), cp.bytes, hipMemcpyDeviceToHost);
        if (e != hipSuccess) return RT_ERR_LAUNCH;
    }
    return RT_OK;
}

int rt_debug_halton_table_device(const rt_ctx* c, float* table, uint32_t capacity) {
    if (!c || !table) return fail(nullptr, RT_ERR_INVALID_ARG, "null argument");
    if (capacity < rt::kHaltonTabLdsFloats)
        return fail(const_cast<rt_ctx*>(c), RT_ERR_INVALID_ARG, "rt_debug_halton_table_device: capacity below the table's size");
    if (!c->d_halton_tab) return RT_ERR_STATE;
    DeviceGuard g(c->device);
    const hipError_t e =
        hipMemcpy(table, c->d_halton_tab.as<void>(), sizeof(float) * rt::kHaltonTabLdsFloats, hipMemcpyDeviceToHost);
    return e == hipSuccess ? RT_OK : RT_ERR_LAUNCH;
}

int rt_last_launch(const rt_ctx* c, rt_launch_info* info) {
    if (!c || !info) return fail(nullptr, RT_ERR_INVALID_ARG, "null argument");
    if (!c->launched) return RT_ERR_STATE;
    memset(info, 0, sizeof(*info));
    static_assert(sizeof(info->kernel) == sizeof(c->launch.kernel), "kernel name buffer");
    memcpy(info->kernel, c->launch.kernel, sizeof(info->kernel));
    info->kernel[sizeof(info->kernel) - 1] = 0;
    info->lanes_per_pixel = c->launch.lanes;
    info->halton_tables = c->launch.tables;
    info->small_index = c->launch.small;
    info->block_threads = c->launch.threads;
    info->grid_x = c->launch.grid_x;
    info->grid_y = c->launch.grid_y;
    info->lds_bytes = c->launch.lds;
    return RT_OK;
}

int rt_debug_stats(rt_ctx* c, uint64_t* out, int n) {
    if (!c || !out || n <= 0) return fail(c, RT_ERR_INVALID_ARG, "null argument");
    DeviceGuard g(c->device);
    hipError_t e = rt::read_debug_stats(reinterpret_cast<unsigned long long*>(out), n);
    if (e == hipErrorNotSupported) return fail(c, RT_ERR_STATE, "not an RT_STATS build");
    if (e != hipSuccess) return hip_fail(c, RT_ERR_LAUNCH, "read stats", e);
    return RT_OK;
}

#ifndef RT_SRC_SHA
#define RT_SRC_SHA "unknown"
#endif
const char* rt_build_sha(void) { return RT_SRC_SHA; }

}
```

gpuraytracer_amd/csrc/rt_api_host.cpp:

```cpp
#include <string.h>

#include <thread>
#include <vector>

#include "rt_api_internal.hpp"
#include "rt_beam.hpp"
#include "rt_halton.hpp"
#include "rt_mathcheck.hpp"
#include "rt_shaft.hpp"

namespace rtapi {

bool resolve_options(const rt_create_options* o, Resolved* r, const char** why) {
    *r = Resolved();
    if (!o) return true;
    for (uint32_t v : o->reserved)
        if (v != 0) { *why = "rt_create_options.reserved must be zero"; return false; }
    switch (o->scene_layout) {
        case RT_LAYOUT_AUTO: r->mem = rt::SceneMem::kAuto; break;
        case RT_LAYOUT_PAIRS: r->mem = rt::SceneMem::kPairLds; break;
        case RT_LAYOUT_SINGLE: r->mem = rt::SceneMem::kLdsSingle; break;
        case RT_LAYOUT_GLOBAL: r->mem = rt::SceneMem::kSmem; break;
        case RT_LAYOUT_PAIRS_SMEM: r->mem = rt::SceneMem::kPairSmem; break;
        case RT_LAYOUT_SORTED: r->mem = rt::SceneMem::kPairSorted; break;
// ... 188 lines not shown
    if (const char* why = rtapi::plan_params_error(p, RT_PLAN_RELATIVE))
        return rtapi::fail(nullptr, RT_ERR_INVALID_ARG, std::string("rt_plan_samples_host: ") + why);
    if (!first || !all || !counts)
        return rtapi::fail(nullptr, RT_ERR_INVALID_ARG, "rt_plan_samples_host: first, all or counts is null");
    if (width < 1 || p->rows < 1 || p->rows > 0x7FFFFFFFu)
        return rtapi::fail(nullptr, RT_ERR_INVALID_ARG, "rt_plan_samples_host: width and params->rows must be >= 1");
    const int W = width, H = (int)p->rows, R = (int)p->radius;
    const size_t n = (size_t)W * (size_t)H;
    const bool relative = (p->flags & RT_PLAN_RELATIVE) != 0;
    std::vector<uint32_t> q(n);
    for (size_t k = 0; k < n; ++k) {
        const float* f = first + 4 * k;
        const float* a = all + 4 * k;
        q[k] = rt::plan_weight(f[0], f[1], f[2], a[0], a[1], a[2], relative, p->luminance_floor);
    }
    uint64_t Q = 0;
    for (int y = 0; y < H; ++y)
        for (int x = 0; x < W; ++x) {
            uint32_t m = 0;
            for (int j = std::max(0, y - R); j <= std::min(H - 1, y + R); ++j)
                for (int i = std::max(0, x - R); i <= std::min(W - 1, x + R); ++i)
                    m = std::max(m, q[(size_t)j * (size_t)W + (size_t)i]);
            counts[(size_t)y * (size_t)W + (size_t)x] = m;
            Q += m;
        }
    rt_plan_stats s{};
    s.weight_sum = Q;
    for (size_t k = 0; k < n; ++k) {
        const uint64_t share = rt::plan_share(p->budget, counts[k], Q, p->count_min);
        const bool capped = share > (uint64_t)p->count_max;
        const uint32_t c = capped ? p->count_max : (uint32_t)share;
        counts[k] = c;
        s.samples += c;
        s.at_cap += capped ? 1u : 0u;
        s.count_max_seen = std::max(s.count_max_seen, c);
    }
    if (stats) *stats = s;
    return RT_OK;
}

void rt_denoise_params_default(rt_denoise_params* p) {
    if (!p) return;
    memset(p, 0, sizeof(*p));
    p->iterations = 5;
    p->normal_power_log2 = 7;
    p->sigma_luminance = 4.0f;
    p->sigma_depth = 1.0f;
    p->depth_floor = 0.01f;
}

void rt_path_params_default(rt_path_params* p) {
    if (!p) return;
    memset(p, 0, sizeof(*p));
    p->spp = 1;
    p->bounces = 3;
}

int rt_scene_describe(const rt_scene_desc* d, rt_scene_info* info) {
    return rt_scene_describe_ex(d, nullptr, info);
}

int rt_scene_describe_ex(const rt_scene_desc* d, const rt_create_options* opt, rt_scene_info* info) {
    if (!desc_ok(d) || !info) return fail(nullptr, RT_ERR_INVALID_ARG, "null argument");
    Resolved ro;
    const char* why = nullptr;
    if (!resolve_options(opt, &ro, &why)) return fail(nullptr, RT_ERR_INVALID_ARG, why);
    rt::CompiledScene s;
    const char* err = nullptr;
    if (!compile_desc(d, ro.build, &s, &err)) return fail(nullptr, RT_ERR_INVALID_ARG, err);
    rt::SceneTables t = scene_counts(s, 0);
    info->n_triangles = t.nT;
    info->n_triangle_pairs = t.nP;
    info->n_box_clusters = t.nC;
    info->pair_free_mask = t.pair_free;
    info->n_spheres = t.nS;
    info->n_sphere_nodes = t.nN;
    const size_t lds = rt::kernel_lds_bytes(t.nT, t.nP, t.nS, t.nN);
    const bool bvh = needs_tri_bvh(t, ro.mem);
    info->n_triangle_bvh_nodes = t.nTN = bvh ? 2 * t.nT - 1 : 0u;
    info->sphere_kernel_lds_bytes = (rt::sphere_compact_usable(s) && t.nP > 0 && !bvh &&
                                     ro.mem == rt::SceneMem::kAuto && lds <= rt::kSphPairLdsMaxBytes)
                                        ? (uint32_t)lds
                                        : 0u;
    const size_t lds_clu =
        lds + (t.nS ? 0u : 16 * rt::staged_f4<size_t>(rt::kLayPairClu, t.nT, t.nP, t.nC).clu);
    info->lds_bytes = (!bvh && lds <= rt::kMaxLdsBytes)
                          ? (uint32_t)(lds_clu <= rt::kMaxLdsBytes ? lds_clu : lds)
                          : 0u;
    const rt::KernelChoice kc = rt::choose_kernel(t, rt::sphere_compact_usable(s), 3, ro.mem, ro.walk);
    info->kernel_layout = (uint32_t)kc.layout;
    info->kernel_lds_bytes = (uint32_t)kc.lds_bytes;
    return RT_OK;
}

int rt_debug_ray_domain(const rt_scene_desc* d, rt_ray_domain_info* info) {
    if (!desc_ok(d) || !info) return fail(nullptr, RT_ERR_INVALID_ARG, "null argument");
    rt::CompiledScene s;
    const char* err = nullptr;
    if (!compile_desc(d, rt::BuildOptions(), &s, &err)) return fail(nullptr, RT_ERR_INVALID_ARG, err);
    const rt::RayDomain D = rt::ray_domain(s.extent);
    info->origin_max = D.origin_max;
    info->dir_len2_min = D.dir_len2_min;
    info->dir_len2_max = D.dir_len2_max;
    info->tmax_max = D.tmax_max;
    return RT_OK;
}

int rt_debug_camera_candidates(const rt_scene_desc* d, int32_t x0, int32_t x1, int32_t y0, int32_t y1,
                               uint8_t* may_hit) {
    if (!desc_ok(d) || !may_hit || x1 < x0 || y1 < y0 || x0 < 0 || y0 < 0)
        return fail(nullptr, RT_ERR_INVALID_ARG, "null argument or empty rectangle");
    rt::CompiledScene s;
    const char* err = nullptr;
    if (!compile_desc(d, rt::BuildOptions(), &s, &err)) return fail(nullptr, RT_ERR_INVALID_ARG, err);
    memset(may_hit, 1, d->n_triangles);
    const rt::Beam beam = desc_beam(s.cam, x0, x1, y0, y1);
    for (size_t k = 0; k < s.pair_isect.size(); ++k)
        if (rt::beam_excludes_pair(beam, s.pair_isect[k].q)) may_hit[2 * k] = may_hit[2 * k + 1] = 0;
    return RT_OK;
}

int rt_debug_shadow_candidates(const rt_scene_desc* d, int32_t x0, int32_t x1, int32_t y0, int32_t y1,
                               uint8_t* may_occlude, int32_t* available) {
    if (!desc_ok(d) || !may_occlude || !available || x1 < x0 || y1 < y0 || x0 < 0 || y0 < 0)
        return fail(nullptr, RT_ERR_INVALID_ARG, "null argument or empty rectangle");
    rt::CompiledScene s;
    const char* err = nullptr;
    if (!compile_desc(d, rt::BuildOptions(), &s, &err)) return fail(nullptr, RT_ERR_INVALID_ARG, err);
    memset(may_occlude, 1, d->n_triangles);
    *available = 0;
    const size_t nP = s.pair_isect.size();
    if (nP == 0) return RT_OK;
    const rt::Beam beam = desc_beam(s.cam, x0, x1, y0, y1);
    const rt::ShaftLight L = rt::shaft_light(rt::f3{s.light.center[0], s.light.center[1], s.light.center[2]});
    std::vector<uint8_t> keep(nP, 0);
    bool ok = true;
    for (size_t k = 0; k < nP; ++k) {
        if (rt::beam_excludes_pair(beam, s.pair_isect[k].q)) continue;
        for (int tb = 0; tb < 2; ++tb) {
            const float* sh = s.tri_shade[2 * k + tb].s;
            if (sh[3] != 0.0f) continue;
            const rt::ShaftSrc S = rt::shaft_source(beam, s.pair_isect[k].q, tb, rt::f3{sh[0], sh[1], sh[2]}, L);
            ok = ok && S.ok;
            for (size_t j = 0; j < nP; ++j)
                if (!rt::shaft_excludes_pair(S, L, s.pair_isect[j].q)) keep[j] = 1;
        }
    }
    if (!ok) return RT_OK;
    *available = 1;
    for (size_t j = 0; j < nP; ++j) may_occlude[2 * j] = may_occlude[2 * j + 1] = keep[j];
    return RT_OK;
}

int rt_debug_cluster_kinds(const rt_scene_desc* d, uint32_t* flags, uint32_t capacity, uint32_t* n_clusters) {
    if (!desc_ok(d) || !n_clusters || (!flags && capacity)) return fail(nullptr, RT_ERR_INVALID_ARG, "null argument");
    rt::CompiledScene s;
    const char* err = nullptr;
    if (!compile_desc(d, rt::BuildOptions(), &s, &err)) return fail(nullptr, RT_ERR_INVALID_ARG, err);
    const size_t rec = 4 * rt::kCluF4, nC = s.clusters.size() / rec;
    *n_clusters = (uint32_t)nC;
    for (size_t c = 0; c < nC && c < capacity; ++c) memcpy(&flags[c], &s.clusters[c * rec + 15], 4);
    return RT_OK;
}

int rt_debug_light_mask(const rt_scene_desc* d, uint64_t* mask, float* records, uint32_t capacity_triangles) {
    if (!desc_ok(d) || !mask || (!records && capacity_triangles))
        return fail(nullptr, RT_ERR_INVALID_ARG, "null argument");
    rt::CompiledScene s;
    const char* err = nullptr;
    if (!compile_desc(d, rt::BuildOptions(), &s, &err)) return fail(nullptr, RT_ERR_INVALID_ARG, err);
    *mask = rt::light_mask(s);
    for (size_t k = 0; k < s.tri_shade.size() && k < capacity_triangles; ++k)
        memcpy(records + 16 * k, s.tri_shade[k].s, sizeof(s.tri_shade[k].s));
    return RT_OK;
}

int rt_debug_halton_table(float* table, uint32_t capacity, uint32_t* n_floats, uint32_t* offsets, uint32_t* sizes) {
    static_assert(rt::kHaltonTabFloats == rt::kHaltonTabLdsFloats, "rt_kernel.hpp's size of the tables");
    if (!n_floats || (!table && capacity)) return fail(nullptr, RT_ERR_INVALID_ARG, "null argument");
    *n_floats = rt::kHaltonTabFloats;
    for (int D = 0; D < 24; ++D) {
        if (offsets) offsets[D] = rt::tab_offset(D);
        if (sizes) sizes[D] = rt::tab_size(D);
    }
    if (!table) return RT_OK;
    if (capacity < rt::kHaltonTabFloats)
        return fail(nullptr, RT_ERR_INVALID_ARG, "rt_debug_halton_table: capacity below the table's size");
    rt::fill_halton_tables(table, 0u, 1u);
    return RT_OK;
}

int rt_debug_tri_bvh_host(const rt_scene_desc* d, const rt_create_options* opt, rt_tri_bvh_dump* dump) {
    if (!desc_ok(d) || !dump) return fail(nullptr, RT_ERR_INVALID_ARG, "null argument");
    Resolved ro;
    const char* why = nullptr;
    if (!resolve_options(opt, &ro, &why)) return fail(nullptr, RT_ERR_INVALID_ARG, why);
    rt::CompiledScene s;
    const char* err = nullptr;
    if (!compile_desc(d, ro.build, &s, &err)) return fail(nullptr, RT_ERR_INVALID_ARG, err);
    const size_t nT = s.tri_isect.size();
    dump->n_triangles = (uint32_t)nT;
    dump->nodes_per_layout = 0;
    dump->leaf_max = tri_leaf_clamp(ro.tri_leaf_max);
    dump->margin = s.margin;
    if (nT == 0) return fail(nullptr, RT_ERR_INVALID_ARG, "the scene has no triangles");
    if (dump->isect) memcpy(dump->isect, s.tri_isect.data(), nT * sizeof(rt::TriIsect));
    if (!dump->nodes && !dump->sorted && !dump->perm) return RT_OK;
    HostTree t;
    if (!rt::build_tri_sah(s.tri_isect, s.margin, &t.nodes, &t.sorted, &t.perm, ro.tri_leaf_max, ro.tri_leaf_cost))
        return fail(nullptr, RT_ERR_INVALID_ARG, "triangle BVH build: too many triangles (2^24)");
    dump_host_tree(t, dump);
    return RT_OK;
}

int rt_debug_tri_bvh_refit_host(const rt_scene_desc* from, const rt_create_options* opt, const rt_scene_desc* to,
                                rt_tri_bvh_dump* dump) {
    if (!desc_ok(from) || !desc_ok(to) || !dump) return fail(nullptr, RT_ERR_INVALID_ARG, "null argument");
    if (from->n_triangles != to->n_triangles)
        return fail(nullptr, RT_ERR_INVALID_ARG, "rt_debug_tri_bvh_refit_host: n_triangles of the two scenes differ");
    Resolved ro;
    const char* why = nullptr;
    if (!resolve_options(opt, &ro, &why)) return fail(nullptr, RT_ERR_INVALID_ARG, why);
    rt::CompiledScene a, b;
    const char* err = nullptr;
    if (!compile_desc(from, ro.build, &a, &err) || !compile_desc(to, ro.build, &b, &err))
        return fail(nullptr, RT_ERR_INVALID_ARG, err);
    const size_t nT = a.tri_isect.size();
    if (nT == 0) return fail(nullptr, RT_ERR_INVALID_ARG, "the scene has no triangles");
    if (b.tri_isect.size() != nT) return fail(nullptr, RT_ERR_INVALID_ARG, "n_triangles of the compiled scenes differ");
    HostTree t;
    if (!rt::build_tri_sah(a.tri_isect, a.margin, &t.nodes, &t.sorted, &t.perm, ro.tri_leaf_max, ro.tri_leaf_cost))
        return fail(nullptr, RT_ERR_INVALID_ARG, "triangle BVH build: too many triangles (2^24)");
    if (!rt::refit_tri_bvh_host(b.tri_isect, b.margin, &t.nodes, t.perm, &t.sorted))
        return fail(nullptr, RT_ERR_STATE, "triangle BVH refit: the tree is outside the format");
    dump->n_triangles = (uint32_t)nT;
    dump->leaf_max = tri_leaf_clamp(ro.tri_leaf_max);
    dump->margin = b.margin;
    dump_host_tree(t, dump);
    if (dump->isect) memcpy(dump->isect, b.tri_isect.data(), nT * sizeof(rt::TriIsect));
    return RT_OK;
}

int rt_tile_layout(int32_t width, int32_t height, int32_t world, int32_t rank, uint32_t flags,
                   rt_tile_layout_info* out) {
    if (!out || !tile_args_ok(width, height, world) || rank < 0 || rank >= world)
        return RT_ERR_INVALID_ARG;
    const TileLayout L = tile_layout((uint32_t)width, (uint32_t)height, (uint32_t)world, (uint32_t)rank, flags);
    out->rows = L.rows;
    out->rows_max = L.rows_max;
    out->row_bytes = L.row_bytes;
    out->tile_bytes = L.tile_bytes;
    return RT_OK;
}

int rt_place_tiles_host(const void* gathered, int32_t width, int32_t height, int32_t world, uint32_t flags,
                        void* frame) {
    if (!gathered || !frame || !tile_args_ok(width, height, world)) return RT_ERR_INVALID_ARG;
    const uint32_t W = (uint32_t)width, H = (uint32_t)height, N = (uint32_t)world;
    for (uint32_t k = 0; k < N && k < H; ++k) {
        const TileLayout L = tile_layout(W, H, N, k, flags);
        for (uint32_t j = 0; j < L.rows; ++j)
            memcpy(static_cast<char*>(frame) + (size_t)(k + j * N) * L.row_bytes,
                   static_cast<const char*>(gathered) + k * L.tile_bytes + j * L.row_bytes, L.row_bytes);
    }
    return RT_OK;
}

int rt_math_selfcheck(uint64_t* mismatches) {
    if (!mismatches) return fail(nullptr, RT_ERR_INVALID_ARG, "null argument");
    if (const int st = math_device_ready()) return st;
    unsigned long long bad[2] = {0, 0};
    const hipError_t e = rt::math_selfcheck(bad);
    if (e != hipSuccess) return hip_fail(nullptr, RT_ERR_LAUNCH, "math_selfcheck", e);
    mismatches[0] = bad[0];
    mismatches[1] = bad[1];
    return RT_OK;
}

int rt_debug_math_values(uint32_t fn_word, uint32_t where, const uint32_t* in_bits, uint64_t n, uint32_t* out_bits) {
    if (n == 0) return RT_OK;
    if (!in_bits || !out_bits) return fail(nullptr, RT_ERR_INVALID_ARG, "null argument");
    if (n > RT_MATH_VALUES_MAX) return fail(nullptr, RT_ERR_INVALID_ARG, "n > RT_MATH_VALUES_MAX");
    uint32_t fn, D, top = 0;
    if ((fn_word & 0xFFu) >= RT_MATH_HALTON_SMALL)
        for (uint64_t j = 0; j < n; ++j) top = std::max(top, in_bits[j]);
    if (const char* why = math_fn_args(fn_word, where, top, &fn, &D)) return fail(nullptr, RT_ERR_INVALID_ARG, why);
    if (where == RT_MATH_HOST) {
        for (uint64_t j = 0; j < n; ++j) out_bits[j] = math_eval_host(fn, D, in_bits[j]);
        return RT_OK;
    }
    if (const int st = math_device_ready()) return st;
    const hipError_t e = rt::math_values_device(fn, D, in_bits, (uint32_t)n, out_bits);
    if (e != hipSuccess) return hip_fail(nullptr, RT_ERR_LAUNCH, "math_values", e);
    return RT_OK;
}

int rt_debug_math_sums(uint32_t fn_word, uint32_t where, uint32_t first_bits, uint64_t count, uint32_t chunk_log2,
                       uint32_t host_threads, uint64_t* sums) {
    if (count == 0) return RT_OK;
    if (!sums) return fail(nullptr, RT_ERR_INVALID_ARG, "null argument");
    if (chunk_log2 < rt::kMathChunkLog2Min || chunk_log2 > rt::kMathChunkLog2Max)
        return fail(nullptr, RT_ERR_INVALID_ARG, "chunk_log2 outside 6..31");
    if ((uint64_t)first_bits + count > (1ull << 32))
        return fail(nullptr, RT_ERR_INVALID_ARG, "first_bits + count > 2^32");
    uint32_t fn, D;
    if (const char* why = math_fn_args(fn_word, where, (uint64_t)first_bits + count - 1, &fn, &D))
// ... 63 lines not shown
```

gpuraytracer_amd/csrc/rt_api_internal.hpp:

```cpp
#pragma once
#include <hip/hip_runtime.h>

#include <algorithm>
#include <string>

#include "../../include/rtpt.h"
#include "rt_kernel.hpp"
#include "rt_plan.hpp"
#include "rt_scene.hpp"

namespace rtapi {

constexpr uint32_t kDefaultTriBuild = RT_TRI_BVH_GPU_SAH;

int fail(rt_ctx* ctx, int status, const std::string& msg);

inline int hip_fail(rt_ctx* ctx, int status, const char* what, hipError_t e) {
    return fail(ctx, status, std::string(what) + ": " + hipGetErrorString(e));
}

struct Resolved {
    uint32_t lanes = 0, tri_build = RT_TRI_BVH_HOST_SAH, walk = RT_WALK_AUTO, walk_leaf_den = 0;
    rt::SceneMem mem = rt::SceneMem::kAuto;
    uint32_t tri_leaf_max = rt::kTriLeafMax;
    double tri_leaf_cost = 1.0;
    rt::BuildOptions build;
};
bool resolve_options(const rt_create_options* o, Resolved* r, const char** why);

inline bool desc_ok(const rt_scene_desc* d) { return d && d->camera && d->square_lights; }

inline bool compile_desc(const rt_scene_desc* d, const rt::BuildOptions& build, rt::CompiledScene* s,
                         const char** err) {
    return rt::compile_scene(*d->camera, d->materials, d->vertices, d->n_triangles, d->square_lights[0], d->spheres,
                             d->n_spheres, s, err, build);
}

inline rt::SceneTables scene_counts(const rt::CompiledScene& s, uint32_t nTN) {
    rt::SceneTables t{};
    t.nT = (uint32_t)s.tri_isect.size();
    t.nP = (uint32_t)s.pair_isect.size();
    t.nS = (uint32_t)s.sph_isect.size();
    t.nN = s.sph_layout_nodes;
    t.nTN = nTN;
    t.nC = (uint32_t)(s.clusters.size() / (4 * rt::kCluF4));
    t.pair_free = s.pair_free_mask;
    return t;
}

inline bool needs_tri_bvh(const rt::SceneTables& t, rt::SceneMem mem) {
    const size_t lds_pairs = rt::kernel_lds_bytes(t.nT, t.nP, 0, 0);
    const size_t lds_single = rt::kernel_lds_bytes(t.nT, 0, 0, 0);
    return t.nT > 0 && (mem == rt::SceneMem::kTriBvh ||
                        (mem == rt::SceneMem::kAuto &&
                         (t.nT > rt::kTriBvhMinTriangles || std::min(lds_pairs, lds_single) > rt::kMaxLdsBytes)));
}

inline uint32_t tri_leaf_clamp(uint32_t leaf_max) { return std::min(128u, std::max(1u, leaf_max)); }

inline size_t pixel_bytes(uint32_t flags) { return (flags & RT_OUT_RGBA8) ? 4u : (flags & RT_OUT_FP16) ? 8u : 16u; }

struct TileLayout {
    uint32_t rows, rows_max;
    size_t row_bytes, tile_bytes;
};

inline TileLayout tile_layout(uint32_t W, uint32_t H, uint32_t N, uint32_t rank, uint32_t flags) {
    TileLayout L;
    L.rows = rank < H ? (H - 1u - rank) / N + 1u : 0u;
    L.rows_max = (H + N - 1u) / N;
    L.row_bytes = (size_t)W * pixel_bytes(flags);
    L.tile_bytes = (size_t)L.rows_max * L.row_bytes;
    return L;
}

inline const char* plan_params_error(const rt_plan_params* p, uint32_t flags_ok) {
    static_assert(sizeof(rt_plan_params) == 40 && sizeof(rt_plan_stats) == 32 && sizeof(rt::PlanStats) == 32,
                  "rt_plan_params / rt_plan_stats layout");
    if (!p) return "params is null";
    if (p->flags & ~flags_ok) return "unknown flag bits";
    if (p->reserved[0] || p->reserved[1]) return "reserved must be 0";
    if (p->count_max > rt::kPlanCountMax) return "count_max must be <= 2^24";
    if (p->count_min > p->count_max) return "count_min must be <= count_max";
    if (p->budget >= rt::kPlanBudgetEnd) return "budget must be < 2^38";
    if (p->radius > rt::kPlanRadiusMax) return "radius must be in [0, 2]";
    if ((p->flags & RT_PLAN_RELATIVE) && !(p->luminance_floor > 0.0f))
        return "luminance_floor must be > 0 with RT_PLAN_RELATIVE";
    return nullptr;
}

float halton_host(uint32_t i, uint32_t d);

}
```

gpuraytracer_amd/csrc/rt_kernel.hip:

```cpp
#include <hip/hip_runtime.h>
#include <hip/hip_fp16.h>

#include <stddef.h>
#include <stdio.h>
#ifdef RT_LDS_CHECK
#include <hsa/hsa.h>
#endif

#include "rt_kernel.hpp"
#include "rt_halton.hpp"
#include "rt_beam.hpp"
#include "rt_shaft.hpp"
#include "rt_pixel.hpp"
#include "rt_trace.hpp"

namespace rt {

#ifdef RT_LDS_CHECK
__device__ uint32_t g_lds_overflow;
__device__ __forceinline__ bool lds_short(size_t end) {
    const uint32_t grp = ((const uint32_t*)__builtin_amdgcn_dispatch_ptr())[7];
    const size_t dyn = grp - __builtin_amdgcn_groupstaticsize();
    if (end <= dyn) return false;
    if (threadIdx.x == 0) atomicMax(&g_lds_overflow, (uint32_t)end);
// ... 308 lines not shown
    if (P.sum) P.sum[o] = make_float4(lum.x, lum.y, lum.z, (float)P.samples_total);
    if (P.out) {
        const float fs = (float)P.samples_total;
        const float r = lum.x / fs, g = lum.y / fs, bl = lum.z / fs;
        store_pixel(P, o, r, g, bl);
    }
}

constexpr uint32_t kSortBuckets = 9;
constexpr uint32_t kSortA = 0;
constexpr uint32_t kSortB = kBlockThreads;
constexpr uint32_t kSortC = 2 * kBlockThreads;
constexpr uint32_t kSortD = 3 * kBlockThreads;
constexpr uint32_t kSortLum = kSortD + kBlockThreads / 2;
constexpr uint32_t kSortCnt = kSortLum + 3 * kBlockThreads / 4;
constexpr uint32_t kSortF4 = kSortCnt + (kSortBuckets * 4 + 3) / 4;

__device__ __forceinline__ uint32_t sort_octant(f3 d) {
    return (d.x > 0.0f ? 4u : 0u) | (d.y > 0.0f ? 2u : 0u) | (d.z > 0.0f ? 1u : 0u);
}

__device__ __forceinline__ void sort_paths(float4* lds, PathState& s, uint32_t& owner,
                                           bool& alive) {
    const uint32_t tid = threadIdx.x, wave = tid >> 6, lane = tid & 63u;
    uint32_t* counts = reinterpret_cast<uint32_t*>(lds + kSortCnt);
    const uint32_t key = alive ? sort_octant(s.d) : 8u;
    uint32_t my_count = 0, slot = 0;
#pragma unroll
    for (uint32_t k = 0; k < kSortBuckets - 1; ++k) {
        const unsigned long long m = __ballot(key == k);
        if (lane == k) my_count = (uint32_t)__popcll(m);
        if (key == k) slot = (uint32_t)__popcll(m & ((1ull << lane) - 1ull));
    }
    if (lane < kSortBuckets - 1) counts[lane * 4u + wave] = my_count;
    __syncthreads();
    const uint32_t idx = lane & 31u;
    const uint32_t c = counts[idx];
    uint32_t v = c;
#pragma unroll
    for (uint32_t off = 1; off < 32; off <<= 1) {
        const uint32_t t = __shfl_up(v, off);
        if (idx >= off) v += t;
    }
    const uint32_t live = __shfl(v, 31);
    slot += __shfl(v - c, (int)(key * 4u + wave));
    if (alive) {
        lds[kSortA + slot] = make_float4(s.o.x, s.o.y, s.o.z, s.thr.x);
        lds[kSortB + slot] = make_float4(s.d.x, s.d.y, s.d.z, s.thr.y);
        lds[kSortC + slot] = make_float4(s.acc.x, s.acc.y, s.acc.z, s.thr.z);
        reinterpret_cast<uint2*>(lds + kSortD)[slot] = make_uint2(s.i, owner);
    }
    s.thr = f3{0.0f, 0.0f, 0.0f};
    s.acc = f3{0.0f, 0.0f, 0.0f};
    __syncthreads();
    alive = tid < live;
    if (alive) {
        const float4 a = lds[kSortA + tid], bq = lds[kSortB + tid];
        const uint2 dd = reinterpret_cast<const uint2*>(lds + kSortD)[tid];
        s.o = f3{a.x, a.y, a.z};
        s.d = f3{bq.x, bq.y, bq.z};
        s.i = dd.x;
        owner = dd.y;
    }
}

__device__ __forceinline__ void load_thr_acc(const float4* lds, PathState& s) {
    const uint32_t tid = threadIdx.x;
    const float4 c = lds[kSortC + tid];
    s.thr = f3{lds[kSortA + tid].w, lds[kSortB + tid].w, c.w};
    s.acc = f3{c.x, c.y, c.z};
}

__device__ __forceinline__ void deliver(float4* lds, uint32_t owner, f3 acc) {
    float* sum = reinterpret_cast<float*>(lds + kSortLum);
    sum[owner] = sum[owner] + acc.x;
    sum[kBlockThreads + owner] = sum[kBlockThreads + owner] + acc.y;
    sum[2 * kBlockThreads + owner] = sum[2 * kBlockThreads + owner] + acc.z;
}

template <int b, int B, int GEO, bool SPH, bool SMALL>
struct SortedChain {
    __device__ __forceinline__ static void run(const KParams& P, const SceneView& sv, float4* lds,
                                               PathState& s, uint32_t& owner, bool& alive) {
        if (b > 0) sort_paths(lds, s, owner, alive);
        if (alive) {
            float t = 1000.0f;
            constexpr bool cull = GEO == kGeoTriBvh ? b == 0 : true;
            const int id = closest_hit<GEO, SPH, cull, (b == 0 ? 0 : 1)>(sv, s.o, s.d, 0.001f, &t);
            if (b > 0) load_thr_acc(lds, s);
            alive = id >= 0 && shade<b, B, GEO, SPH, SMALL>(P, sv, s, id, t);
            if (!alive || b + 1 == B) deliver(lds, owner, s.acc);
        }
        SortedChain<b + 1, B, GEO, SPH, SMALL>::run(P, sv, lds, s, owner, alive);
    }
};
template <int B, int GEO, bool SPH, bool SMALL>
struct SortedChain<B, B, GEO, SPH, SMALL> {
    __device__ __forceinline__ static void run(const KParams&, const SceneView&, float4*,
                                               PathState&, uint32_t&, bool&) {}
};


}

constexpr int kMinWavesPerEu = 8;
constexpr int kMinWavesPerEuSph = 8;
#ifndef RT_CLU_WAVES
#define RT_CLU_WAVES 7
#endif
constexpr int kMinWavesPerEuClu = RT_CLU_WAVES;
constexpr uint32_t block_threads(int geo) { return geo == kGeoSphLds ? kSphBlockThreads : kBlockThreads; }
constexpr uint32_t waves_per_row(int geo) { return block_threads(geo) >= 128 ? 2u : 1u; }
constexpr uint32_t waves_per_col(int geo) { return block_threads(geo) / 64u / waves_per_row(geo); }

template <int B, int GEO, bool SPH, bool SMALL, int L = 1>
#ifndef RT_TRI_WAVES
#define RT_TRI_WAVES 8
#endif
__global__ __launch_bounds__(block_threads(GEO),
                             SPH ? kMinWavesPerEuSph
                                 : (GEO == kGeoPairClu ? kMinWavesPerEuClu
                                                       : (GEO == kGeoTriBvh ? RT_TRI_WAVES : kMinWavesPerEu)))
void path_trace_kernel(KParams P) {
    constexpr uint32_t NT = block_threads(GEO), WR = waves_per_row(GEO), WC = waves_per_col(GEO);
    extern __shared__ float4 lds[];
    SceneView sv;
    const SceneTables T = tables_of(P);
    if (geo_staged(GEO)) {
        const StagedF4<uint32_t> n = staged_f4(GEO, T.nT, T.nP, T.nC);
        RT_LDS_GUARD(16 * (size_t)(n.rec + n.clu) + (GEO == kGeoPairClu ? 4 * (size_t)kHaltonTabFloats : 0));
        stage_records<GEO, NT>(lds, T);
        if (GEO == kGeoSphLds) {
            __shared__ float sph_stash[GEO == kGeoSphLds ? 6 * kSphBlockThreads : 1];
            sv.xstash = sph_stash;
        }
        if (GEO == kGeoPairClu) {
            const uint32_t tab0 = n.rec + n.clu;
            const bool tab = halton_tables_on(GEO, SMALL, P.spp, L);
            sv.htab = tab ? reinterpret_cast<const float*>(lds + tab0) : nullptr;
            if (tab) copy_halton_tables<NT>(reinterpret_cast<float*>(lds + tab0), P.halton_tab, threadIdx.x);
        }
        __syncthreads();
    }
    bind_scene<GEO, SPH>(sv, T, lds);

    const uint32_t kWX = (L == 1) ? 8u : P.wave_w, kWY = (64u / L) / kWX;
    uint32_t bx, by;
    xcd_tile(bx, by);
    auto pixel_of = [&](uint32_t t, uint32_t& x, uint32_t& j) {
        const uint32_t lane = t & 63u, wave = t >> 6, pix = lane / L;
        x = bx * (WR * kWX) + (wave % WR) * kWX + (pix % kWX);
        j = by * (WC * kWY) + (wave / WR) * kWY + (pix / kWX);
    };
    if constexpr (RT_CAM_CAND && GEO == kGeoPairClu) {
        if (sv.nP - 1u < 32u) {
            const uint32_t wave = wave_uniform(threadIdx.x >> 6);
            const uint32_t wx0 = bx * (WR * kWX) + (wave % WR) * kWX;
            const uint32_t wj0 = by * (WC * kWY) + (wave / WR) * kWY;
            const float y0 = (float)(P.row_start + wj0 * P.row_step);
            const float y1 = (float)(P.row_start + (wj0 + kWY - 1u) * P.row_step);
            const Beam beam = make_beam(ld_f3(P.cam_pos), ld_f3(P.cam_u), ld_f3(P.cam_v), ld_f3(P.cam_w), P.halfW,
                                        P.halfH, (float)P.W, (float)P.H, (float)wx0, (float)(wx0 + kWX - 1u), y0, y1);
            const uint32_t k = threadIdx.x & 63u;
            const uint32_t kc = min(k, sv.nP - 1u);
            const bool keep = !beam_excludes_pair(beam, reinterpret_cast<const float*>(sv.pair + kPairF4 * kc));
            sv.cam_mask = wave_uniform((uint32_t)__builtin_amdgcn_ballot_w64(k < sv.nP && keep));
            sv.cam_avail = true;
            if constexpr (RT_SHD_CAND) {
                const uint32_t tb = k >> 5, kt = min(k & 31u, sv.nP - 1u);
                bool occ = false, bad = (sv.cam_mask & (sv.cam_mask - 1u)) != 0u;
                if (sv.cam_mask != 0u && !bad) {
                    const uint32_t sp = (uint32_t)__builtin_ctz(sv.cam_mask);
                    const float4 s0 = P.tri_shade[4 * (2u * sp + tb)];
                    if (s0.w == 0.0f) {
                        const ShaftLight lq = shaft_light(ld_f3(P.light_center));
                        const ShaftSrc src = shaft_source(beam, reinterpret_cast<const float*>(sv.pair + kPairF4 * sp),
                                                          (int)tb, f3{s0.x, s0.y, s0.z}, lq);
                        bad = !src.ok;
                        occ = !shaft_excludes_pair(src, lq, reinterpret_cast<const float*>(sv.pair + kPairF4 * kt));
                    }
                }
                const unsigned long long ob = __builtin_amdgcn_ballot_w64((k & 31u) < sv.nP && occ);
                sv.shd_mask = wave_uniform((uint32_t)ob | (uint32_t)(ob >> 32));
                sv.shd_avail = __builtin_amdgcn_ballot_w64(bad) == 0ull && sv.nC <= 32u;
                if (sv.nC != 0u) {
                    const uint32_t kc2 = min(k, sv.nC - 1u);
                    const uint32_t all = __float_as_uint(reinterpret_cast<const float*>(sv.clu + kCluF4 * kc2)[22]);
                    sv.shd_cskip = wave_uniform(
                        (uint32_t)__builtin_amdgcn_ballot_w64(k < sv.nC && (all & sv.shd_mask) == 0u));
                }
            }
        }
    }
    constexpr bool kRemat = GEO == kGeoPairClu || GEO == kGeoSphLds;
    auto opaque_tid = []() {
        uint32_t t = threadIdx.x;
        if constexpr (kRemat) asm volatile("" : "+v"(t));
        return t;
    };
    {
        uint32_t x, j;
        pixel_of(threadIdx.x, x, j);
        if (x >= (uint32_t)P.W || j >= P.row_count) return;
    }
    __shared__ uint32_t seed_s[NT];
    __shared__ float lum_s[L > 1 ? 3 * (NT / L) : 1];
    f3 lum{0.0f, 0.0f, 0.0f};
    {
        const uint32_t t = threadIdx.x, sub = t % L;
        uint32_t x, j;
        pixel_of(t, x, j);
        const uint32_t y = P.row_start + j * P.row_step;
        seed_s[t] = P.seeds[(size_t)y * (size_t)P.W + x] + P.sample_base;
        if (P.accumulate) {
            const float4 prev = P.sum[(size_t)j * (size_t)P.W + x];
            lum = f3{prev.x, prev.y, prev.z};
        }
        const uint32_t slot = t / L;
        if (L > 1 && sub == 0) {
            lum_s[3 * slot] = lum.x;
            lum_s[3 * slot + 1] = lum.y;
            lum_s[3 * slot + 2] = lum.z;
        }
    }
    const f3 cu = ld_f3(P.cam_u), cv = ld_f3(P.cam_v), cw = ld_f3(P.cam_w);
    const float fW = (float)P.W, fH = (float)P.H;
    uint32_t rounds = (P.spp + (L - 1)) / L;
    constexpr bool kDeadSkip = RT_CAM_CAND && RT_DEAD_SKIP && GEO == kGeoPairClu && !SPH;
    bool dead = false;
    if constexpr (kDeadSkip) {
        dead = sv.cam_avail && sv.cam_mask == 0u;
        if (dead) rounds = 0u;
    }
    for (uint32_t r = 0; r < rounds; ++r) {
#ifdef RT_STATS
        const unsigned long long t_round = clock64();
#endif
        const uint32_t t = opaque_tid(), sub = t % L;
        const uint32_t n = (L == 1) ? r : min(r * L + sub, P.spp - 1u);
        PathState s;
        s.acc = f3{0.0f, 0.0f, 0.0f};
        {
            uint32_t x, j;
            pixel_of(t, x, j);
            const float fx = (float)x, fy = (float)(P.row_start + j * P.row_step);
            s.i = seed_s[t] + n;
            const float jx = halton_dim<0, SMALL>(s.i);
            const float jy = halton_dim<1, SMALL, GEO == kGeoPairClu>(s.i, sv.htab);
            s.d = camera_dir<GEO == kGeoTriBvh>(P, cu, cv, cw, fW, fH, fx, fy, jx, jy);
            s.o = ld_f3(P.cam_pos);
            s.thr = f3{1.0f, 1.0f, 1.0f};
#if RT_CENSUS == 1
            {
                const uint32_t i2 = cz(s.i);
                const float jx2 = halton_dim<0, SMALL>(i2);
                const float jy2 = halton_dim<1, SMALL, GEO == kGeoPairClu>(i2, sv.htab);
                cz_sink(camera_dir(P, cu, cv, cw, fW, fH, cz(fx), cz(fy), jx2, jy2));
            }
#endif
#ifndef RT_TIMING_NO_TRACE
            trace_path<B, GEO, SPH, SMALL>(P, sv, s);
#else
            s.acc = s.d;
#endif
        }
        if (L == 1) {
            lum = lum + s.acc;
        } else if (L <= 16 && !SPH) {
            const uint32_t t2 = opaque_tid(), sub2 = t2 % L, slot = t2 / L;
            f3 acc{lum_s[3 * slot], lum_s[3 * slot + 1], lum_s[3 * slot + 2]};
#if RT_CENSUS == 6
            {
                f3 a2 = cz(acc);
                row_sum_in_order<L, 0>::run(a2, cz(s.acc), r * L, P.spp);
                cz_sink(a2);
            }
#endif
            row_sum_in_order<L, 0>::run(acc, s.acc, r * L, P.spp);
            if (sub2 == 0) {
                lum_s[3 * slot] = acc.x;
                lum_s[3 * slot + 1] = acc.y;
                lum_s[3 * slot + 2] = acc.z;
            }
        } else {
            const uint32_t t2 = opaque_tid(), lane = t2 & 63u, sub2 = t2 % L, slot = t2 / L;
            const int base = (int)(lane - sub2);
            f3 c[L];
#pragma unroll
            for (int k = 0; k < L; ++k)
                c[k] = f3{__shfl(s.acc.x, base + k), __shfl(s.acc.y, base + k),
                          __shfl(s.acc.z, base + k)};
            if (sub2 == 0) {
                f3 acc{lum_s[3 * slot], lum_s[3 * slot + 1], lum_s[3 * slot + 2]};
#pragma unroll
                for (int k = 0; k < L; ++k)
                    if (r * L + (uint32_t)k < P.spp) acc = acc + c[k];
                lum_s[3 * slot] = acc.x;
                lum_s[3 * slot + 1] = acc.y;
                lum_s[3 * slot + 2] = acc.z;
            }
        }
#ifdef RT_STATS
        if (!SPH && GEO != kGeoTriBvh) {
            RT_STAT(24, clock64() - t_round);
            RT_STAT(25, 1);
        }
#endif
    }
    uint32_t t = threadIdx.x;
    asm volatile("" : "+v"(t));
    if (L > 1) {
        if (t % L != 0) return;
        const uint32_t slot = t / L;
        lum = f3{lum_s[3 * slot], lum_s[3 * slot + 1], lum_s[3 * slot + 2]};
    }
    if constexpr (kDeadSkip) {
        if (dead && P.spp != 0u) lum = lum + f3{0.0f, 0.0f, 0.0f};
    }
    uint32_t x, j;
    pixel_of(t, x, j);
    const size_t o = (size_t)j * (size_t)P.W + x;
    if (P.sum) P.sum[o] = make_float4(lum.x, lum.y, lum.z, (float)P.samples_total);
    if (P.out) {
        const float fs = (float)P.samples_total;
        const float r = lum.x / fs, g = lum.y / fs, bl = lum.z / fs;
        store_pixel(P, o, r, g, bl);
    }
}

#include "rt_free.hpp"

#ifndef RT_SORTED_BVH_WAVES
#define RT_SORTED_BVH_WAVES 4
#endif
template <int B, int GEO, bool SPH, bool SMALL>
__global__ __launch_bounds__(kBlockThreads, GEO == kGeoPairLds ? kMinWavesPerEu : RT_SORTED_BVH_WAVES)
void path_trace_sorted_kernel(
    KParams P) {
    extern __shared__ float4 lds[];
    SceneView sv;
    const SceneTables T = tables_of(P);
    RT_LDS_GUARD(16 * (size_t)(kSortF4 + staged_f4(GEO, T.nT, T.nP, T.nC).rec));
    float4* scene = lds + kSortF4;
    stage_records<GEO, kBlockThreads>(scene, T);
    bind_scene<GEO, SPH>(sv, T, scene);

    const uint32_t tid = threadIdx.x, lane = tid & 63u, wave = tid >> 6;
    const uint32_t x = blockIdx.x * kTile + (wave & 1u) * 8u + (lane & 7u);
    const uint32_t j = blockIdx.y * kTile + (wave >> 1) * 8u + (lane >> 3);
    const bool valid = x < (uint32_t)P.W && j < P.row_count;
    const uint32_t y = P.row_start + j * P.row_step;
    const size_t o = (size_t)j * (size_t)P.W + x;
    const uint32_t seed = valid ? P.seeds[(size_t)y * (size_t)P.W + x] : 0u;
    float* sum = reinterpret_cast<float*>(lds + kSortLum);
    {
        float4 prev = make_float4(0.0f, 0.0f, 0.0f, 0.0f);
        if (valid && P.accumulate) prev = P.sum[o];
        sum[tid] = prev.x;
        sum[kBlockThreads + tid] = prev.y;
        sum[2 * kBlockThreads + tid] = prev.z;
    }
    __syncthreads();
    const float fx = (float)x, fy = (float)y, fW = (float)P.W, fH = (float)P.H;
    for (uint32_t n = 0; n < P.spp; ++n) {
        PathState s;
        s.i = seed + (P.sample_base + n);
        s.acc = f3{0.0f, 0.0f, 0.0f};
        s.thr = f3{1.0f, 1.0f, 1.0f};
        s.o = ld_f3(P.cam_pos);
        s.d = f3{0.0f, 0.0f, 0.0f};
        if (valid) {
            const float jx = halton_dim<0, SMALL>(s.i), jy = halton_dim<1, SMALL>(s.i);
            s.d = camera_dir(P, ld_f3(P.cam_u), ld_f3(P.cam_v), ld_f3(P.cam_w), fW, fH, fx, fy, jx, jy);
        }
        uint32_t owner = tid;
        bool alive = valid;
        SortedChain<0, B, GEO, SPH, SMALL>::run(P, sv, lds, s, owner, alive);
        __syncthreads();
    }
    if (!valid) return;
    finish_pixel(P, o, f3{sum[tid], sum[kBlockThreads + tid], sum[2 * kBlockThreads + tid]});
}

__global__ void math_check_kernel(uint32_t lo, uint32_t n, unsigned long long* bad) {
    for (uint32_t i = blockIdx.x * blockDim.x + threadIdx.x; i < n; i += gridDim.x * blockDim.x) {
        const float x = __uint_as_float(lo + i);
        float y = x;
        asm volatile("" : "+v"(y));
        const float s = sqrt_cr(x), sr = sqrtf(y);
        const float r = rcp_cr(x), rr = 1.0f / y;
        const bool sbad = !(__float_as_uint(s) == __float_as_uint(sr) || (s != s && sr != sr));
        const bool rbad = !(__float_as_uint(r) == __float_as_uint(rr) || (r != r && rr != rr));
        if (sbad) atomicAdd(&bad[0], 1ull);
        if (rbad) atomicAdd(&bad[1], 1ull);
    }
}

__global__ void fill_seeds_kernel(uint32_t* seeds, uint64_t key, uint64_t n) {
    for (uint64_t p = (uint64_t)blockIdx.x * blockDim.x + threadIdx.x; p < n;
         p += (uint64_t)gridDim.x * blockDim.x) {
        uint64_t z = key + p + 0x9E3779B97F4A7C15ULL;
        z = (z ^ (z >> 30)) * 0xBF58476D1CE4E5B9ULL;
        z = (z ^ (z >> 27)) * 0x94D049BB133111EBULL;
        z = z ^ (z >> 31);
        seeds[p] = (uint32_t)(z & 0xFFFFFu);
    }
}

__global__ __launch_bounds__(kBlockThreads) void halton_tables_kernel(float* tab) {
    fill_halton_tables(tab, threadIdx.x, kBlockThreads);
}

template <typename U>
__global__ void place_tiles_kernel(const U* __restrict__ gathered, U* __restrict__ frame, uint32_t row_u,
                                   size_t tile_u, uint32_t H, uint32_t N) {
    for (uint32_t y = blockIdx.y; y < H; y += gridDim.y) {
        const uint32_t k = y % N, j = y / N;
        const U* src = gathered + k * tile_u + (size_t)j * row_u;
        U* dst = frame + (size_t)y * row_u;
        for (uint32_t u = blockIdx.x * blockDim.x + threadIdx.x; u < row_u; u += gridDim.x * blockDim.x)
            dst[u] = src[u];
    }
}

hipError_t launch_place_tiles(const void* gathered, void* frame, size_t row_bytes, size_t tile_bytes,
                              uint32_t H, uint32_t N, hipStream_t stream) {
    if (H == 0 || N == 0 || row_bytes == 0) return hipSuccess;
    if (row_bytes % 4 || tile_bytes % 4) return hipErrorInvalidValue;
    const bool wide = row_bytes % 16 == 0 && tile_bytes % 16 == 0 &&
                      reinterpret_cast<uintptr_t>(gathered) % 16 == 0 && reinterpret_cast<uintptr_t>(frame) % 16 == 0;
    const size_t unit = wide ? 16 : 4;
    const uint32_t row_u = (uint32_t)(row_bytes / unit);
    const dim3 grid((row_u + 255u) / 256u, H < 65535u ? H : 65535u);
    if (wide)
        hipLaunchKernelGGL(place_tiles_kernel<uint4>, grid, dim3(256), 0, stream,
                           static_cast<const uint4*>(gathered), static_cast<uint4*>(frame), row_u,
                           tile_bytes / 16, H, N);
    else
        hipLaunchKernelGGL(place_tiles_kernel<uint32_t>, grid, dim3(256), 0, stream,
                           static_cast<const uint32_t*>(gathered), static_cast<uint32_t*>(frame), row_u,
                           tile_bytes / 4, H, N);
    return hipGetLastError();
}

namespace {

inline int lanes_per_pixel(const KParams& P, int geo) {
    if (P.lanes == 1 || P.lanes == 4 || P.lanes == 16) return P.spp >= P.lanes ? (int)P.lanes : 1;
    const uint64_t px = (uint64_t)P.W * P.row_count;
    const bool share16 = P.row_step > 1 && P.spp >= 16u * kHaltonTabMinRounds;
    const int want = (px >= 1000000ull && geo != kGeoSphLds && geo != kGeoTriBvh && !share16) ? 4 : 16;
    if (P.spp >= (uint32_t)want) return want;
    return P.spp >= 4 ? 4 : 1;
}

constexpr int kGeoPairSorted = kLayPairSorted;
constexpr int kGeoFreeSph = kLayFreeSph;
constexpr int kGeoFreeTri = kLayFreeTri;
constexpr int kGeoSortSph = kLaySortSph;
constexpr int kGeoSortTri = kLaySortTri;
static_assert(kGeoTriLds == kLayTriLds && kGeoPairLds == kLayPairLds && kGeoTriGlobal == kLayTriGlobal &&
                  kGeoPairSmem == kLayPairSmem && kGeoTriBvh == kLayTriBvh && kGeoPairClu == kLayPairClu &&
                  kGeoSphLds == kLaySphLds,
              "rt_trace.hpp Geo == rt_kernel.hpp KernelLayout");
static_assert(kHaltonTabLdsFloats == kHaltonTabFloats && kSortLdsF4 == kSortF4, "staged_lds_bytes terms");

thread_local LaunchInfo g_last;

template <int B, int GEO, bool SPH, bool SMALL, int L>
void note_launch(const char* name, const KParams& P, dim3 grid, uint32_t threads, size_t lds) {
    LaunchInfo& I = g_last;
    snprintf(I.kernel, sizeof(I.kernel), "rt::%s<%d, %d, %s, %s, %d>", name, B, GEO,
             SPH ? "true" : "false", SMALL ? "true" : "false", L);
    I.lanes = (uint32_t)L;
    I.tables = halton_tables_on(GEO, SMALL, P.spp, (uint32_t)L) ? 1u : 0u;
    I.small = SMALL ? 1u : 0u;
    I.threads = threads;
    I.grid_x = grid.x;
    I.grid_y = grid.y;
    I.lds = (uint32_t)lds;
}

inline hipError_t allow_lds(const void* kernel, size_t bytes) {
    if (bytes <= 65536) return hipSuccess;
    return hipFuncSetAttribute(kernel, hipFuncAttributeMaxDynamicSharedMemorySize, (int)bytes);
}

template <int B, int GEO, bool SPH, bool SMALL, int L>
hipError_t launch_tl(const KParams& P, size_t lds_bytes, hipStream_t stream) {
    KParams Q = P;
    if (L > 1) Q.wave_w = (P.row_step > 1) ? 64u / L : (L == 4 ? 4u : 2u);
    constexpr uint32_t WR = waves_per_row(GEO), WC = waves_per_col(GEO);
    const uint32_t WX = (L == 1) ? 8u : Q.wave_w;
    const uint32_t TX = WR * WX, TY = WC * ((64u / L) / WX);
    const dim3 grid((P.W + TX - 1) / TX, (P.row_count + TY - 1) / TY);
    if (GEO == kGeoSphLds) {
        const hipError_t e = allow_lds((const void*)path_trace_kernel<B, GEO, SPH, SMALL, L>, lds_bytes);
        if (e != hipSuccess) return e;
    }
    note_launch<B, GEO, SPH, SMALL, L>("path_trace_kernel", Q, grid, block_threads(GEO), lds_bytes);
    hipLaunchKernelGGL((path_trace_kernel<B, GEO, SPH, SMALL, L>), grid, dim3(block_threads(GEO)),
                       lds_bytes, stream, Q);
    return hipGetLastError();
}

template <int B, int GEO, bool SPH, bool SMALL>
hipError_t launch_t(const KParams& P, size_t lds_bytes, hipStream_t stream) {
    if (SMALL) {
        const int lpp = lanes_per_pixel(P, GEO);
        if (lpp == 16) return launch_tl<B, GEO, SPH, SMALL, 16>(P, lds_bytes, stream);
        if (lpp == 4) return launch_tl<B, GEO, SPH, SMALL, 4>(P, lds_bytes, stream);
    }
    return launch_tl<B, GEO, SPH, SMALL, 1>(P, lds_bytes, stream);
}

template <int B, int GEO, bool SPH, bool SMALL>
hipError_t launch_sorted_t(const KParams& P, size_t lds_bytes, hipStream_t stream) {
    const dim3 grid((P.W + kTile - 1) / kTile, (P.row_count + kTile - 1) / kTile);
    note_launch<B, GEO, SPH, SMALL, 1>("path_trace_sorted_kernel", P, grid, kBlockThreads, lds_bytes);
    hipLaunchKernelGGL((path_trace_sorted_kernel<B, GEO, SPH, SMALL>), grid, dim3(kBlockThreads),
                       lds_bytes, stream, P);
    return hipGetLastError();
}

template <int B, int GEO, bool SORTED, bool SPH, bool SMALL>
hipError_t launch_k(const KParams& P, size_t lds_bytes, hipStream_t stream) {
    if constexpr (SORTED)
        return launch_sorted_t<B, GEO, SPH, SMALL>(P, lds_bytes, stream);
    else
        return launch_t<B, GEO, SPH, SMALL>(P, lds_bytes, stream);
}

template <int B, int GEO, bool SORTED, bool SPH>
hipError_t launch_h(const KParams& P, size_t lds_bytes, hipStream_t stream) {
    return P.max_index < kSmallIndexMax ? launch_k<B, GEO, SORTED, SPH, true>(P, lds_bytes, stream)
                                        : launch_k<B, GEO, SORTED, SPH, false>(P, lds_bytes, stream);
}

template <int B, int GEO, bool SORTED = false>
hipError_t launch_g(const KParams& P, size_t lds_bytes, hipStream_t stream) {
    if constexpr (GEO == (SORTED ? kGeoTriBvh : kGeoPairClu))
        return launch_h<B, GEO, SORTED, false>(P, lds_bytes, stream);
    if (GEO == kGeoSphLds || P.nS > 0) return launch_h<B, GEO, SORTED, true>(P, lds_bytes, stream);
    return launch_h<B, GEO, SORTED, false>(P, lds_bytes, stream);
}

template <int B, int GEO, bool SMALL>
hipError_t launch_free_t(const KParams& P, size_t lds_bytes, hipStream_t stream) {
    KParams Q = P;
    Q.wave_w = (P.row_step > 1) ? 64u : 8u;
    const uint32_t TY = 64u / Q.wave_w;
    const dim3 grid((P.W + Q.wave_w - 1) / Q.wave_w, (P.row_count + TY - 1) / TY);
    note_launch<B, GEO, GEO == kGeoSphLds, SMALL, 1>("path_free_kernel", Q, grid, kFreeThreads, lds_bytes);
    hipLaunchKernelGGL((path_free_kernel<B, GEO, SMALL>), grid, dim3(kFreeThreads), lds_bytes, stream,
                       Q);
    return hipGetLastError();
}

template <int B, int GEO>
hipError_t launch_free(const KParams& P, size_t lds_bytes, hipStream_t stream) {
    if constexpr (B < 1) {
        return hipErrorInvalidValue;
    } else {
        return P.max_index < kSmallIndexMax ? launch_free_t<B, GEO, true>(P, lds_bytes, stream)
                                            : launch_free_t<B, GEO, false>(P, lds_bytes, stream);
    }
}

template <int B>
hipError_t launch_b(const KParams& P, int geo, size_t lds_bytes, hipStream_t stream) {
    if (geo == kGeoFreeSph) return launch_free<B, kGeoSphLds>(P, lds_bytes, stream);
    if (geo == kGeoFreeTri) return launch_free<B, kGeoTriBvh>(P, lds_bytes, stream);
    if (geo == kGeoPairSorted) return launch_g<B, kGeoPairLds, true>(P, lds_bytes, stream);
    if (geo == kGeoSortSph) return launch_g<B, kGeoSphLds, true>(P, lds_bytes, stream);
    if (geo == kGeoSortTri) return launch_g<B, kGeoTriBvh, true>(P, lds_bytes, stream);
    switch (geo) {
        case kGeoPairLds: return launch_g<B, kGeoPairLds>(P, lds_bytes, stream);
        case kGeoPairClu: return launch_g<B, kGeoPairClu>(P, lds_bytes, stream);
        case kGeoSphLds: return launch_g<B, kGeoSphLds>(P, lds_bytes, stream);
        case kGeoPairSmem: return launch_g<B, kGeoPairSmem>(P, lds_bytes, stream);
        case kGeoTriBvh: return launch_g<B, kGeoTriBvh>(P, lds_bytes, stream);
        case kGeoTriLds: return launch_g<B, kGeoTriLds>(P, lds_bytes, stream);
        default: return launch_g<B, kGeoTriGlobal>(P, lds_bytes, stream);
    }
}

}

size_t kernel_lds_bytes(uint32_t n_tri, uint32_t n_pairs, uint32_t n_sph, uint32_t n_nodes) {
    (void)n_sph;
    (void)n_nodes;
    return n_pairs ? staged_lds_bytes(kLayPairLds, n_tri, n_pairs, 0) : staged_lds_bytes(kLayTriLds, n_tri, 0, 0);
}

KernelChoice choose_kernel(const SceneTables& t, bool sph_compact, uint32_t bounces, SceneMem mem, uint32_t walk) {
    const uint32_t nP = t.nP, nS = t.nS, nC = t.nC, nTN = t.nTN;
    auto lds = [&](int lay) { return staged_lds_bytes(lay, t.nT, nP, nC); };
    const bool pairs = nP > 0 && mem != SceneMem::kLdsSingle;
    int geo = kGeoTriGlobal;
    if (mem != SceneMem::kSmem && lds(pairs ? kGeoPairLds : kGeoTriLds) <= kMaxLdsBytes)
        geo = pairs ? kGeoPairLds : kGeoTriLds;
    if (mem == SceneMem::kPairSmem && nP > 0) geo = kGeoPairSmem;
    if (nTN > 0 && (mem == SceneMem::kTriBvh || mem == SceneMem::kAuto)) geo = kGeoTriBvh;
    if (geo == kGeoPairLds && nS > 0 && sph_compact && mem == SceneMem::kAuto &&
        lds(kGeoSphLds) <= kSphPairLdsMaxBytes)
        geo = kGeoSphLds;
    if (geo == kGeoPairLds && nC > 0 && nS == 0 && mem == SceneMem::kAuto && lds(kGeoPairClu) <= kMaxLdsBytes)
        geo = kGeoPairClu;
    if (geo == kGeoPairLds && mem == SceneMem::kPairSorted && lds(kGeoPairSorted) <= kMaxLdsBytes)
        geo = kGeoPairSorted;
    if (bounces >= 1 && walk == kWalkFree) {
        if (geo == kGeoSphLds) geo = kGeoFreeSph;
        if (geo == kGeoTriBvh && nS == 0) geo = kGeoFreeTri;
    }
    if (walk == kWalkSorted) {
        if (geo == kGeoSphLds) geo = kGeoSortSph;
        if (geo == kGeoTriBvh && nS == 0) geo = kGeoSortTri;
    }
    return KernelChoice{geo, lds(geo)};
}

namespace {
hipError_t launch_path_trace_impl(const KParams& P, uint32_t bounces, SceneMem mem,
                                  hipStream_t stream) {
    const KernelChoice kc = choose_kernel(tables_of(P), P.sph_lds != nullptr, bounces, mem, P.walk);
    const int geo = kc.layout;
    const size_t lds_total = kc.lds_bytes;
#ifdef RT_LDS_UNDERSIZE
    const size_t lds_req = lds_total >= 16 ? lds_total - 16 : lds_total;
#else
    const size_t lds_req = lds_total;
#endif
#ifdef RT_DEV_ISA
    if (bounces != 3) return hipErrorInvalidValue;
    if (geo == kGeoFreeSph) return launch_free<3, kGeoSphLds>(P, lds_req, stream);
    if (geo == kGeoFreeTri) return launch_free<3, kGeoTriBvh>(P, lds_req, stream);
    if (geo == kGeoSortSph) return launch_g<3, kGeoSphLds, true>(P, lds_req, stream);
    if (geo == kGeoSortTri) return launch_g<3, kGeoTriBvh, true>(P, lds_req, stream);
    if (geo == kGeoTriBvh) return launch_g<3, kGeoTriBvh>(P, lds_req, stream);
    return geo == kGeoPairClu ? launch_g<3, kGeoPairClu>(P, lds_req, stream)
                              : launch_g<3, kGeoSphLds>(P, lds_req, stream);
#endif
    switch (bounces) {
        case 0: return launch_b<0>(P, geo, lds_req, stream);
        case 1: return launch_b<1>(P, geo, lds_req, stream);
        case 2: return launch_b<2>(P, geo, lds_req, stream);
        case 3: return launch_b<3>(P, geo, lds_req, stream);
        case 4: return launch_b<4>(P, geo, lds_req, stream);
        default: return hipErrorInvalidValue;
    }
}
}

hipError_t launch_path_trace(const KParams& P, uint32_t bounces, SceneMem mem,
                             hipStream_t stream, LaunchInfo* info) {
    const hipError_t e = launch_path_trace_impl(P, bounces, mem, stream);
    if (info) *info = g_last;
    return e;
}

#include "rt_counts.hpp"
#include "rt_paths.hpp"

hipError_t lds_check_result(uint32_t* end) {
    *end = 0;
#ifdef RT_LDS_CHECK
    hipError_t e = hipMemcpyFromSymbol(end, HIP_SYMBOL(g_lds_overflow), sizeof(uint32_t));
    if (e != hipSuccess) return e;
    const uint32_t zero = 0;
    return hipMemcpyToSymbol(HIP_SYMBOL(g_lds_overflow), &zero, sizeof(zero));
#else
    return hipSuccess;
#endif
}

hipError_t read_debug_stats(unsigned long long* out, int n) {
#if defined(RT_FREE_DEBUG)
    constexpr int kWords = (int)(sizeof(g_free_dbg) / 8);
    if (n > kWords) n = kWords;
    hipError_t e = hipMemcpyFromSymbol(out, HIP_SYMBOL(g_free_dbg), n * sizeof(unsigned long long));
    if (e != hipSuccess) return e;
    static const uint32_t zero[4] = {0, 0, 0, 0};
    return hipMemcpyToSymbol(HIP_SYMBOL(g_free_dbg), zero, sizeof(zero));
#elif defined(RT_STATS)
    if (n > 40) n = 40;
    hipError_t e = hipMemcpyFromSymbol(out, HIP_SYMBOL(g_rt_stats), n * sizeof(unsigned long long));
    if (e != hipSuccess) return e;
    const unsigned long long zero[40] = {0};
    return hipMemcpyToSymbol(HIP_SYMBOL(g_rt_stats), zero, sizeof(zero));
#else
    (void)out;
    (void)n;
    return hipErrorNotSupported;
#endif
}

hipError_t math_selfcheck(unsigned long long bad[2]) {
    unsigned long long* d = nullptr;
    hipError_t e = hipMalloc((void**)&d, 2 * sizeof(unsigned long long));
    if (e != hipSuccess) return e;
    if ((e = hipMemset(d, 0, 2 * sizeof(unsigned long long))) == hipSuccess) {
        hipLaunchKernelGGL(math_check_kernel, dim3(16384), dim3(256), 0, 0, 0u, 0x80000000u, d);
        hipLaunchKernelGGL(math_check_kernel, dim3(16384), dim3(256), 0, 0, 0x80000000u, 0x80000000u, d);
        if ((e = hipGetLastError()) == hipSuccess && (e = hipDeviceSynchronize()) == hipSuccess)
            e = hipMemcpy(bad, d, 2 * sizeof(unsigned long long), hipMemcpyDeviceToHost);
    }
    (void)hipFree(d);
    return e;
}

hipError_t launch_fill_halton_tables(float* tab, hipStream_t stream) {
    hipLaunchKernelGGL(halton_tables_kernel, dim3(1), dim3(kBlockThreads), 0, stream, tab);
    return hipGetLastError();
}

hipError_t launch_fill_seeds(uint32_t* seeds, uint64_t key, uint64_t n, hipStream_t stream) {
    if (n == 0) return hipSuccess;
    uint64_t blocks = (n + 255) / 256;
    if (blocks > 8192) blocks = 8192;
    hipLaunchKernelGGL(fill_seeds_kernel, dim3((unsigned)blocks), dim3(256), 0, stream, seeds,
                       key, n);
    return hipGetLastError();
}

}
```

gpuraytracer_amd/csrc/rt_kernel.hpp:

```cpp
#pragma once

#include <hip/hip_runtime.h>
#include <stddef.h>
#include <stdint.h>

#include "rt_math.h"
#include "rt_raydomain.h"

namespace rt {

constexpr uint32_t kBlockThreads = 256;
constexpr uint32_t kTile = 16;
constexpr size_t kMaxLdsBytes = 64 * 1024;
constexpr uint32_t kOutFp16 = 0x2u;
constexpr uint32_t kOutRgba8 = 0x10u;
constexpr uint32_t kPairF4 = 7;
constexpr uint32_t kSphBlockThreads = 64;
constexpr size_t kSphPairLdsMaxBytes = 6 * 1024;
constexpr uint32_t kCluF4 = 7;
#ifndef RT_CAM_CAND
#define RT_CAM_CAND 1
#endif
#ifndef RT_SHD_CAND
#define RT_SHD_CAND 1
#endif
#ifndef RT_SHD_SHORT
#define RT_SHD_SHORT 3
#endif
#ifndef RT_DEAD_SKIP
#define RT_DEAD_SKIP 1
#endif
#ifndef RT_CLU_ORDER
#define RT_CLU_ORDER 1
#endif
#ifndef RT_CLU_LEAN
#define RT_CLU_LEAN 1
#endif
constexpr uint32_t kTriCompactLayouts = 8;
constexpr uint32_t kTriBvhMinTriangles = 384;

struct SceneTables {
    const float4* tri_isect;
    const float4* pair_isect;
    const float4* clusters;
    const float4* sph_isect;
    const float4* sph_nodes;
    const uint32_t* sph_perm;
    const uint4* sph_box;
    const uint4* tri_nodes;
    const float4* tri_sorted;
    const uint32_t* tri_perm;
    uint32_t nT, nP, nS, nN;
    uint32_t nTN;
    uint32_t nC;
    uint32_t pair_free;
};
struct KParams {
    const float4* tri_isect;
    const float4* pair_isect;
    const float4* tri_shade;
    const float4* sph_isect;
    const float4* sph_nodes;
    const uint32_t* sph_perm;
    const float4* sph_shade;
    const uint32_t* sph_lds;
    const uint16_t* sph_lds_id;
    const uint4* sph_box;
    const uint4* tri_nodes;
    const float4* tri_sorted;
    const uint32_t* tri_perm;
    const uint32_t* seeds;
    float4* sum;
    void* out;
    uint32_t nT, nP, nS, nN;
    uint32_t nE;
    uint32_t nTN;
    float cam_pos[3], cam_u[3], cam_v[3], cam_w[3];
    float halfW, halfH;
    int32_t W, H;
    float light_center[3], light_color[3];
    uint32_t spp, sample_base;
    uint32_t row_start, row_step, row_count;
    uint32_t accumulate;
    uint32_t samples_total;
    uint32_t flags;
    uint32_t max_index;
    uint32_t lanes;
    uint32_t walk;
    uint32_t wave_w;
    uint32_t walk_leaf_den;
    uint32_t light_plain;
    const float4* clusters;
    uint32_t nC;
    uint32_t pair_free;
    uint64_t light_mask;
    const float* halton_tab;
};

size_t kernel_lds_bytes(uint32_t n_tri, uint32_t n_pairs, uint32_t n_sph, uint32_t n_nodes);

enum KernelLayout : int {
    kLayTriLds = 0,
    kLayPairLds = 1,
    kLayTriGlobal = 2,
    kLayPairSorted = 3,
    kLayPairSmem = 4,
    kLayTriBvh = 5,
    kLayPairClu = 6,
    kLaySphLds = 7,
    kLayFreeSph = 8,
    kLayFreeTri = 9,
    kLaySortSph = 10,
    kLaySortTri = 11,
};
template <typename N>
struct StagedF4 {
    N rec, clu;
};
template <typename N = uint32_t>
__host__ __device__ __forceinline__ constexpr StagedF4<N> staged_f4(int lay, N nT, N nP, N nC) {
    return StagedF4<N>{lay == kLayTriLds ? 3u * nT
                       : (lay == kLayPairLds || lay == kLayPairClu || lay == kLaySphLds || lay == kLayFreeSph ||
                          lay == kLayPairSorted || lay == kLaySortSph)
                           ? kPairF4 * nP
                           : N(0),
                       lay == kLayPairClu ? kCluF4 * nC : N(0)};
}
constexpr uint32_t kHaltonTabLdsFloats = 4679;
constexpr uint32_t kSortLdsF4 = 1097;
__host__ __device__ constexpr size_t staged_lds_bytes(int lay, uint32_t nT, uint32_t nP, uint32_t nC) {
    const StagedF4<size_t> n = staged_f4<size_t>(lay, nT, nP, nC);
    return 16 * (n.rec + n.clu) + (lay == kLayPairClu ? (size_t)4 * kHaltonTabLdsFloats : (size_t)0) +
           ((lay == kLayPairSorted || lay == kLaySortSph || lay == kLaySortTri) ? (size_t)16 * kSortLdsF4 : (size_t)0);
}
constexpr uint32_t kHaltonTabMinRounds = 8;
__host__ __device__ constexpr bool halton_tables_on(int geo, bool small, uint32_t spp, uint32_t L) {
    return geo == kLayPairClu && small && (spp + L - 1) / L >= kHaltonTabMinRounds;
}
struct KernelChoice {
    int layout;
    size_t lds_bytes;
};
struct LaunchInfo {
    char kernel[96];
    uint32_t lanes, tables, small, threads, grid_x, grid_y, lds;
};
constexpr uint32_t kWalkAuto = 0, kWalkLockstep = 1, kWalkFree = 2, kWalkSorted = 3;
enum class SceneMem { kAuto = 0, kLdsSingle = 1, kSmem = 2, kPairSorted = 3, kPairSmem = 4, kTriBvh = 5, kPairLds = 6 };
hipError_t launch_path_trace(const KParams& P, uint32_t bounces, SceneMem mem, hipStream_t stream,
                             LaunchInfo* info);
KernelChoice choose_kernel(const SceneTables& t, bool sph_compact, uint32_t bounces, SceneMem mem, uint32_t walk);
hipError_t launch_path_counts(const KParams& P, const uint32_t* counts, uint32_t* totals, uint32_t bounces,
                              SceneMem mem, hipStream_t stream, LaunchInfo* info);
hipError_t read_debug_stats(unsigned long long* out, int n);
hipError_t lds_check_result(uint32_t* end);
struct MisParams {
    SceneTables tab;
    const float4* mis_shade;
    const float4* u_tab;
    float4* out;
    uchar4* out8;
    float cam_pos[3], cam_u[3], cam_v[3], cam_w[3];
    float halfW, halfH;
    int32_t W, H;
    float l_center[3], l_tangent[3], l_bitangent[3], l_radiance[3];
    float l_width, l_depth, l_area, exposure;
    uint32_t camera_rays, S;
    uint32_t row_start, row_step, row_count;
    float4* part;
};
constexpr uint32_t kRaysAny = 0x100u;
constexpr uint32_t kRaysExact = 0x200u;
constexpr uint32_t kRayChunk = 2048;
constexpr int ray_query_layout(int lay) {
    return (lay == kLayFreeSph || lay == kLaySortSph)   ? (int)kLaySphLds
           : (lay == kLayFreeTri || lay == kLaySortTri) ? (int)kLayTriBvh
           : lay == kLayPairSorted                      ? (int)kLayPairLds
                                                        : lay;
}
__host__ __device__ constexpr size_t ray_query_lds_bytes(int lay, uint32_t nT, uint32_t nP, uint32_t nC) {
    const StagedF4<size_t> n = staged_f4<size_t>(lay, nT, nP, nC);
    return 16 * (n.rec + n.clu);
}
struct RayQueryParams {
    SceneTables tab;
    uint32_t sph_compact;
    const float4* rays;
    uint2* hits;
    uint32_t n;
    uint32_t flags;
    RayDomain dom;
};
hipError_t launch_ray_query(const RayQueryParams& P, SceneMem mem, hipStream_t stream, LaunchInfo* info);

struct PathQueryArgs {
    const float4* rays;
    const uint32_t* seeds;
    float4* radiance;
    uint2* hits;
    uint32_t n;
    uint64_t seed_key;
    RayDomain dom;
};
constexpr bool path_auto_lanes16(uint32_t spp, uint32_t n) {
    return spp >= 16u || (spp >= 8u && n <= 65536u) || (spp >= 4u && n <= 4096u);
}
__host__ __device__ __forceinline__ constexpr bool path_query_tables_on(int geo, bool small, uint32_t spp, uint32_t L) {
    return geo == kLayPairClu && small && (spp + L - 1) / L >= kHaltonTabMinRounds;
}
static_assert(path_query_tables_on(kLayPairClu, true, 128, 16) == halton_tables_on(kLayPairClu, true, 128, 16) &&
                  path_query_tables_on(kLayPairClu, true, 127, 16) == halton_tables_on(kLayPairClu, true, 127, 16) &&
                  path_query_tables_on(kLayPairClu, false, 128, 1) == halton_tables_on(kLayPairClu, false, 128, 1) &&
                  path_query_tables_on(kLayPairLds, true, 128, 1) == halton_tables_on(kLayPairLds, true, 128, 1) &&
                  path_query_tables_on(kLayPairClu, true, 8, 1) == halton_tables_on(kLayPairClu, true, 8, 1) &&
                  path_query_tables_on(kLayPairClu, true, 7, 1) == halton_tables_on(kLayPairClu, true, 7, 1),
              "one rule for the Halton tables");
__host__ __device__ constexpr size_t path_query_lds_bytes(int lay, uint32_t nT, uint32_t nP, uint32_t nC, bool tables) {
    return ray_query_lds_bytes(lay, nT, nP, nC) + (tables ? (size_t)4 * kHaltonTabLdsFloats : (size_t)0);
}
hipError_t launch_path_query(const KParams& P, const PathQueryArgs& A, uint32_t bounces, SceneMem mem,
                             hipStream_t stream, LaunchInfo* info);

constexpr uint32_t kAovCenter = 0x400u;
constexpr uint32_t kAovTabLdsFloats = 729;
__host__ __device__ constexpr size_t aov_lds_bytes(int lay, uint32_t nT, uint32_t nP, uint32_t nC, bool tables) {
    return ray_query_lds_bytes(lay, nT, nP, nC) + (tables ? (size_t)4 * kAovTabLdsFloats : (size_t)0);
}
struct AovParams {
    SceneTables tab;
    uint32_t sph_compact;
    const float4* tri_shade;
    const float4* sph_shade;
    const uint32_t* seeds;
    float4* albedo;
    float4* normal_depth;
    uint2* first_hit;
    float cam_pos[3], cam_u[3], cam_v[3], cam_w[3];
    float halfW, halfH;
    int32_t W, H;
    uint32_t spp, sample_base;
    uint32_t row_start, row_step, row_count;
    uint32_t flags;
    uint32_t max_index;
};
hipError_t launch_aov(const AovParams& P, SceneMem mem, hipStream_t stream, LaunchInfo* info);

constexpr uint32_t kDenoiseTile = 16;
#ifndef RT_DENOISE_LDS_MAX_STEP
#define RT_DENOISE_LDS_MAX_STEP 4
#endif
static_assert(RT_DENOISE_LDS_MAX_STEP <= 8, "a step-16 footprint (80 x 80 texels of 32 B) is past the CU's 160 KiB of LDS");
__host__ __device__ constexpr size_t denoise_lds_bytes(uint32_t step) {
    return step <= RT_DENOISE_LDS_MAX_STEP ? (size_t)32 * (kDenoiseTile + 4 * step) * (kDenoiseTile + 4 * step)
                                           : (size_t)0;
}
struct DenoiseParams {
    const float4* color_a;
    const float4* color_b;
    const float4* albedo;
    const float4* normal_depth;
    float4* out;
    float4* scratch[2];
    int32_t W, H;
    uint32_t iterations;
    uint32_t normal_power_log2;
    float sigma_luminance, sigma_depth, depth_floor;
};
hipError_t launch_denoise(const DenoiseParams& P, hipStream_t stream, LaunchInfo* info);

constexpr uint32_t kPlanTile = 16;
struct PlanStats {
    unsigned long long weight_sum, samples;
    uint32_t count_max_seen, at_cap;
    uint32_t reserved[2];
};
struct PlanParams {
    const float4* first;
    const float4* all;
    uint32_t* counts;
    PlanStats* acc;
    unsigned long long budget;
    uint32_t count_min, count_max;
    float luminance_floor;
    uint32_t radius;
    int32_t W, rows;
    uint32_t flags;
};
hipError_t launch_plan(const PlanParams& P, hipStream_t stream, LaunchInfo* info);

hipError_t launch_mis(const MisParams& P, SceneMem mem, hipStream_t stream);
size_t mis_lds_bytes(uint32_t n_tri, uint32_t n_pairs);
size_t mis_part_bytes(uint32_t camera_rays, size_t pixels);

hipError_t build_tri_lbvh(const float4* d_tri, uint32_t n, const float lo[3], const float hi[3],
                          float margin, uint4* d_nodes, float4* d_sorted, uint32_t* d_perm,
                          hipStream_t s);

hipError_t build_tri_gsah(const float4* d_tri, uint32_t n, float margin, uint32_t leaf_max, double trav_cost,
                          uint4* d_nodes, float4* d_sorted, uint32_t* d_perm, uint32_t* total_nodes,
                          size_t* temp_bytes, hipStream_t s);
hipError_t scan_u32(const uint32_t* in, uint32_t* out, uint32_t n, uint32_t* tile_sums, hipStream_t s);

size_t tri_refit_table_bytes(uint32_t total);
hipError_t refit_tri_bvh(const float4* d_tri, uint32_t n, float margin, uint4* d_nodes, uint32_t total,
// ... 13 lines not shown
```

gpuraytracer_amd/host.py:

```python
from __future__ import annotations

import ctypes
import os
from dataclasses import dataclass, fields

import numpy as np

from ._native import (MATH_FNS, RT_MATH_DEVICE, RT_MATH_HOST, RT_MATH_VALUES_MAX, LAYOUTS, RT_AOV_CENTER, RT_COMM_ID_BYTES, RT_KEEP_SUM, RT_OK, RT_OUT_DEVICE, RT_OUT_FP16,
                      RT_OUT_NONE, RT_OUT_RGBA8, RT_RAYS_ANY, RT_RAYS_EXACT, RT_UPDATE_REBUILD, TRI_BUILDS, WALKS,
                      AovBuffers, AovParams, BuildStats, CameraGPU, CreateOptions, DenoiseBuffers, DenoiseParams, LaunchInfo, MaterialGPU, MisParamsC, RayDomainInfo,
                      PathParamsC, PlanParams, PlanStats, RT_PLAN_RELATIVE, RenderParamsC,
                      RtError, SceneDesc, SceneInfo, SphereGPU, SquareLightGPU, TileLayout, TriBvhDump, UpdateStats, float3,
                      lib)

DEFAULT_SEED_KEY = 0x5EED00000000


def _check(status: int, ctx=None):
    if status != RT_OK:
        raise RtError(status, lib.rt_last_error(ctx).decode())


def seed_splitmix(width: int, height: int, key: int = DEFAULT_SEED_KEY) -> np.ndarray:
    n = int(width) * int(height)
    out = np.empty(n, dtype=np.uint32)
    lib.rt_seed_splitmix(ctypes.c_uint64(key), out.ctypes.data_as(ctypes.c_void_p), n)
    return out.reshape(height, width)


def tonemap_rgba8(rgba32f: np.ndarray) -> np.ndarray:
    a = np.ascontiguousarray(rgba32f, dtype=np.float32)
    n = a.size // 4
    out = np.empty(a.shape[:-1] + (4,), dtype=np.uint8)
    lib.rt_tonemap_rgba8(a.ctypes.data_as(ctypes.c_void_p), n,
                         out.ctypes.data_as(ctypes.c_void_p))
    return out


def _math_fn(fn: str, dim: int, where: str) -> tuple[int, int]:
    if fn not in MATH_FNS or where not in ("host", "device"):
        raise ValueError(f"unknown function {fn!r} or side {where!r}")
    return MATH_FNS[fn] | (int(dim) << 8), RT_MATH_DEVICE if where == "device" else RT_MATH_HOST


def math_values(fn: str, in_bits, where: str = "host", dim: int = 0) -> np.ndarray:
    word, side = _math_fn(fn, dim, where)
    a = np.ascontiguousarray(in_bits, dtype=np.uint32).ravel()
    out = np.empty(a.size, np.uint32)
    for lo in range(0, a.size, RT_MATH_VALUES_MAX):
        part = a[lo:lo + RT_MATH_VALUES_MAX]
        _check(lib.rt_debug_math_values(word, side, part.ctypes.data_as(ctypes.c_void_p), part.size,
                                        out[lo:].ctypes.data_as(ctypes.c_void_p)))
    return out


def math_sums(fn: str, first: int, count: int, chunk_log2: int = 16, where: str = "host", dim: int = 0,
              host_threads: int = 1) -> np.ndarray:
    word, side = _math_fn(fn, dim, where)
    if not 6 <= chunk_log2 <= 31 or count < 0:
        raise ValueError("chunk_log2 outside 6..31 or a negative count")
    sums = np.zeros(((int(count) + (1 << chunk_log2) - 1) >> chunk_log2, 2), np.uint64)
    _check(lib.rt_debug_math_sums(word, side, first, count, chunk_log2, host_threads,
                                  sums.ctypes.data_as(ctypes.c_void_p)))
    return sums


def comm_unique_id() -> bytes:
    buf = (ctypes.c_uint8 * RT_COMM_ID_BYTES)()
    _check(lib.rt_comm_unique_id(buf))
    return bytes(buf)


def _pixel_flags(fp16: bool = False, rgba8: bool = False) -> int:
    return (RT_OUT_FP16 if fp16 else 0) | (RT_OUT_RGBA8 if rgba8 else 0)


def tile_layout(width: int, height: int, world: int, rank: int, fp16: bool = False,
                rgba8: bool = False) -> dict:
    t = TileLayout()
    _check(lib.rt_tile_layout(width, height, world, rank, _pixel_flags(fp16, rgba8), ctypes.byref(t)))
    return {k: getattr(t, k) for k, _ in TileLayout._fields_}


def place_tiles_host(gathered: np.ndarray, width: int, height: int, world: int) -> np.ndarray:
    g = np.ascontiguousarray(gathered)
    fp16, rgba8 = g.dtype == np.uint16, g.dtype == np.uint8
    if g.dtype not in (np.float32, np.uint16, np.uint8):
        raise ValueError("gathered pixels must be float32, uint16 (fp16 bits) or uint8")
    lay = tile_layout(width, height, world, 0, fp16, rgba8)
    if g.nbytes != world * lay["tile_bytes"]:
        raise ValueError(f"gathered holds {g.nbytes} bytes, expected {world} x {lay['tile_bytes']}")
    frame = np.empty((height, width, 4), g.dtype)
    _check(lib.rt_place_tiles_host(g.ctypes.data_as(ctypes.c_void_p), width, height, world,
                                   _pixel_flags(fp16, rgba8), frame.ctypes.data_as(ctypes.c_void_p)))
    return frame


def _plan_params(budget, count_min, count_max, radius, relative, luminance_floor) -> PlanParams:
    p = PlanParams()
    lib.rt_plan_params_default(ctypes.byref(p))
    p.budget, p.count_min, p.count_max, p.radius = budget, count_min, count_max, radius
    p.luminance_floor = luminance_floor
    p.flags = RT_PLAN_RELATIVE if relative else 0
    return p


def _plan_images(first, all, width=None):
    f = np.ascontiguousarray(first, dtype=np.float32)
    a = np.ascontiguousarray(all, dtype=np.float32)
    if f.ndim != 3 or f.shape[2] != 4 or a.shape != f.shape or (width is not None and f.shape[1] != width):
        raise ValueError("first and all must be (rows, W, 4) float32 images of one shape")
    return f, a


def plan_samples_host(first, all, budget: int, count_min: int = 0, count_max: int = 1 << 24, radius: int = 1,
                      relative: bool = False, luminance_floor: float = 0.01, return_stats: bool = False):
    f, a = _plan_images(first, all)
    p = _plan_params(budget, count_min, count_max, radius, relative, luminance_floor)
    p.rows = f.shape[0]
    counts = np.empty(f.shape[:2], np.uint32)
    s = PlanStats()
    _check(lib.rt_plan_samples_host(f.shape[1], ctypes.byref(p), f.ctypes.data_as(ctypes.c_void_p),
                                    a.ctypes.data_as(ctypes.c_void_p), counts.ctypes.data_as(ctypes.c_void_p),
                                    ctypes.byref(s)))
    return (counts, s.as_dict()) if return_stats else counts


def _tri_bvh_dump(call, n: int, nodes_cap: int) -> dict:
    nodes = np.zeros((8 * nodes_cap, 4), np.uint32)
    srt = np.zeros((n, 12), np.float32)
    perm = np.zeros(n, np.uint32)
    isect = np.zeros((n, 12), np.float32)
    d = TriBvhDump()
    d.nodes, d.sorted, d.perm, d.isect = (a.ctypes.data for a in (nodes, srt, perm, isect))
    call(d)
    total = int(d.nodes_per_layout)
    assert int(d.n_triangles) == n and total <= nodes_cap
    return {"n_triangles": n, "nodes_per_layout": total, "leaf_max": int(d.leaf_max),
            "margin": np.float32(d.margin), "nodes": nodes[:8 * total].reshape(8, total, 4).copy(),
            "sorted": srt, "perm": perm, "isect": isect}


@dataclass
class Options:

    layout: str = "auto"
    lanes: int = 0
    tri_build: str = "default"
    tri_leaf_max: int = 0
    tri_leaf_cost: float = 0.0
    sphere_leaf_max: int = 0
    sphere_median: bool = False
    walk: str = "auto"
    walk_leaf_den: int = 0

    def c(self) -> CreateOptions:
        o = CreateOptions()
        o.scene_layout = LAYOUTS[self.layout]
        o.lanes_per_pixel = self.lanes
        o.tri_bvh_build = TRI_BUILDS[self.tri_build]
        o.tri_leaf_max = self.tri_leaf_max
        o.tri_leaf_cost = self.tri_leaf_cost
        o.sphere_leaf_max = self.sphere_leaf_max
        o.sphere_median = 1 if self.sphere_median else 0
        o.walk_scheduler = WALKS[self.walk]
        o.walk_leaf_den = self.walk_leaf_den
        return o

    _ENV = {"layout": "RTPT_SCENE_MEM", "lanes": "RTPT_LANES", "tri_build": "RTPT_TRI_BUILD",
            "tri_leaf_max": "RTPT_TRI_LEAF", "tri_leaf_cost": "RTPT_TRI_CT",
            "sphere_leaf_max": "RTPT_BVH_LEAF", "walk": "RTPT_WALK"}

    @classmethod
    def from_env(cls, env=None) -> "Options":
        env = os.environ if env is None else env
        o = cls()
        for f in fields(cls):
            v = env.get(cls._ENV.get(f.name, ""))
            if v:
                setattr(o, f.name, type(getattr(o, f.name))(v) if f.type != "str" else v)
        if env.get("RTPT_BVH_SAH") == "0":
            o.sphere_median = True
        return o


class Scene:

    def __init__(self, camera: CameraGPU, materials, vertices, light: SquareLightGPU,
                 spheres=None):
# ... 562 lines not shown
        st = torch.empty(ctypes.sizeof(PlanStats), dtype=torch.uint8, device=first.device) if return_stats else None
        cur, handle = self._stream_handle(stream)
        _check(lib.rt_plan_samples_async(self._ctx, ctypes.byref(p), ctypes.c_void_p(first.data_ptr()),
                                         ctypes.c_void_p(all.data_ptr()), ctypes.c_void_p(cn.data_ptr()),
                                         ctypes.c_void_p(None if st is None else st.data_ptr()),
                                         ctypes.c_void_p(handle)), self._ctx)
        if cur is not None:
            cur.synchronize()
        if not return_stats:
            return cn
        if cur is None:
            torch.cuda.synchronize(first.device) if not hasattr(stream, "synchronize") else stream.synchronize()
        return cn, PlanStats.from_buffer_copy(st.cpu().numpy().tobytes()).as_dict()

    def render_adaptive(self, params: RenderParams, pilot_spp: int, mean_spp: int, radius: int = 1,
                        relative: bool = False, luminance_floor: float = 0.01, count_min: int = 0,
                        return_totals: bool = False, return_stats: bool = False, device: bool = False, stream=None):
        p = params
        if pilot_spp < 2 or pilot_spp % 2:
            raise ValueError("render_adaptive needs an even pilot_spp >= 2 (two halves)")
        if mean_spp < pilot_spp or p.spp < pilot_spp:
            raise ValueError("render_adaptive needs pilot_spp <= mean_spp and pilot_spp <= params.spp (the cap)")
        if p.accumulate or p.fp16 or p.rgba8:
            raise ValueError("render_adaptive renders float32 frames from a new sum (no accumulate, fp16, rgba8)")
        rows, W, h = p.rows(self.scene.height), self.scene.width, pilot_spp // 2
        part = dict(bounces=p.bounces, row_start=p.row_start, row_step=p.row_step, row_count=p.row_count)
        first_p = RenderParams(spp=h, sample_base=p.sample_base, keep_sum=True, **part)
        all_p = RenderParams(spp=h, sample_base=p.sample_base + h, accumulate=True, keep_sum=True, **part)
        rest_p = RenderParams(spp=p.spp - pilot_spp, sample_base=p.sample_base, accumulate=True, keep_sum=True, **part)
        plan = dict(budget=(mean_spp - pilot_spp) * rows * W, count_min=count_min, count_max=max(p.spp - pilot_spp, count_min),
                    radius=radius, relative=relative, luminance_floor=luminance_floor, return_stats=True)
        if not device:
            first, both = self.render(first_p), self.render(all_p)
            counts, stats = self.plan_samples(first, both, **plan)
            img, totals = self.render_counts(rest_p, counts, totals=True)
        else:
            import torch
            dev = torch.device("cuda", self.device)
            s = torch.cuda.current_stream(dev) if stream is None else stream
            first = torch.empty((rows, W, 4), dtype=torch.float32, device=dev)
            both = torch.empty_like(first)
            self.render(first_p, out=first, stream=s)
            self.render(all_p, out=both, stream=s)
            counts, stats = self.plan_samples(first, both, stream=s, **plan)
            img, totals = self.render_counts(rest_p, counts, out=first, totals=True, stream=s)
            if hasattr(s, "synchronize"):
                s.synchronize()
        res = (img,) + ((totals,) if return_totals else ()) + ((stats,) if return_stats else ())
        return res if len(res) > 1 else img

    def render_progressive(self, params: RenderParams, batch_spp: int, out, stream=None,
                           gather: bool = False):
        if stream is None:
            import torch
            stream = torch.cuda.current_stream().cuda_stream
        elif hasattr(stream, "cuda_stream"):
            stream = stream.cuda_stream
        total, done = params.spp, 0
        ptr = out if (out is None or isinstance(out, int)) else out.data_ptr()
        while done < total:
            n = min(batch_spp, total - done)
            last = done + n == total
            p = RenderParams(spp=n, bounces=params.bounces, sample_base=params.sample_base + done,
                             row_start=params.row_start, row_step=params.row_step,
                             row_count=params.row_count, accumulate=done > 0, keep_sum=True,
                             fp16=params.fp16, rgba8=params.rgba8)
            flags = RT_OUT_DEVICE if last else (RT_OUT_DEVICE | RT_OUT_NONE)
            fn = lib.rt_render_gather if gather else lib.rt_render_async
            _check(fn(self._ctx, ctypes.byref(p.c(flags)), ctypes.c_void_p(ptr if last else None),
                      ctypes.c_void_p(stream)), self._ctx)
            done += n
        return out

    def accumulate(self, params: RenderParams):
        _check(lib.rt_render(self._ctx, ctypes.byref(params.c(RT_OUT_NONE | RT_KEEP_SUM)), None),
               self._ctx)

    def draw(self, spp: int = 400, bounces: int = 3) -> np.ndarray:
        return self.render(RenderParams(spp=spp, bounces=bounces))

    def render_mis(self, params: MisParams | None = None, out=None, out8=None):
        p = params or MisParams()
        if out is None and out8 is None:
            rows = p.rows(self.scene.height)
            img = np.empty((rows, self.scene.width, 4), dtype=np.float32)
            img8 = np.empty((rows, self.scene.width, 4), dtype=np.uint8)
            _check(lib.rt_render_mis(self._ctx, ctypes.byref(p.c()),
                                     img.ctypes.data_as(ctypes.c_void_p),
                                     img8.ctypes.data_as(ctypes.c_void_p)), self._ctx)
            return img, img8
        ptr = lambda t: None if t is None else ctypes.c_void_p(t if isinstance(t, int) else t.data_ptr())
        _check(lib.rt_render_mis(self._ctx, ctypes.byref(p.c(RT_OUT_DEVICE)), ptr(out), ptr(out8)),
               self._ctx)
        return out, out8

    def comm_init(self, rank: int, world: int, comm_id: bytes):
        if len(comm_id) != RT_COMM_ID_BYTES:
            raise ValueError("comm_id must be the 128 bytes of rt_comm_unique_id()")
        buf = (ctypes.c_uint8 * RT_COMM_ID_BYTES).from_buffer_copy(comm_id)
        _check(lib.rt_comm_init(self._ctx, rank, world, buf), self._ctx)
        self.rank, self.world = rank, world

    def render_gather(self, params: RenderParams | None = None, out=None, stream=None):
        p = params or RenderParams()
        if out is None:
            frame = None
            if getattr(self, "rank", 0) == 0 and not (p.c().flags & RT_OUT_NONE):
                dt = np.uint8 if p.rgba8 else np.uint16 if p.fp16 else np.float32
                frame = np.empty((self.scene.height, self.scene.width, 4), dtype=dt)
            ptr = None if frame is None else frame.ctypes.data_as(ctypes.c_void_p)
            _check(lib.rt_render_gather(self._ctx, ctypes.byref(p.c()), ptr, None), self._ctx)
            return frame
        if stream is None:
            import torch
            stream = torch.cuda.current_stream().cuda_stream
        elif hasattr(stream, "cuda_stream"):
            stream = stream.cuda_stream
        ptr = out if isinstance(out, int) else out.data_ptr()
        _check(lib.rt_render_gather(self._ctx, ctypes.byref(p.c(RT_OUT_DEVICE)), ctypes.c_void_p(ptr),
                                    ctypes.c_void_p(stream)), self._ctx)
        return out

    def comm_info(self) -> tuple[int, int]:
        n, r = ctypes.c_int32(), ctypes.c_int32()
        _check(lib.rt_comm_info(self._ctx, ctypes.byref(n), ctypes.byref(r)), self._ctx)
        return n.value, r.value

    def place_tiles(self, gathered, world: int, out=None, fp16: bool = False, rgba8: bool = False,
                    stream=None):
        gp = gathered if isinstance(gathered, int) else gathered.data_ptr()
        flags = _pixel_flags(fp16, rgba8)
        if stream is None:
            import torch
            stream = torch.cuda.current_stream().cuda_stream
        elif hasattr(stream, "cuda_stream"):
            stream = stream.cuda_stream
        if out is None:
            dt = np.uint8 if rgba8 else np.uint16 if fp16 else np.float32
            frame = np.empty((self.scene.height, self.scene.width, 4), dt)
            _check(lib.rt_place_tiles(self._ctx, ctypes.c_void_p(gp), world, flags,
                                      frame.ctypes.data_as(ctypes.c_void_p), ctypes.c_void_p(stream)),
                   self._ctx)
            return frame
        ptr = out if isinstance(out, int) else out.data_ptr()
        _check(lib.rt_place_tiles(self._ctx, ctypes.c_void_p(gp), world, flags | RT_OUT_DEVICE,
                                  ctypes.c_void_p(ptr), ctypes.c_void_p(stream)), self._ctx)
        return out

    def last_launch(self) -> dict:
        info = LaunchInfo()
        _check(lib.rt_last_launch(self._ctx, ctypes.byref(info)), self._ctx)
        return info.as_dict()

    def build_info(self) -> dict:
        b = BuildStats()
        _check(lib.rt_build_info(self._ctx, ctypes.byref(b)), self._ctx)
        return {k: getattr(b, k) for k, _ in BuildStats._fields_}

    def tri_bvh(self) -> dict:
        sizes = TriBvhDump()
        _check(lib.rt_debug_tri_bvh(self._ctx, ctypes.byref(sizes)), self._ctx)
        return _tri_bvh_dump(lambda d: _check(lib.rt_debug_tri_bvh(self._ctx, ctypes.byref(d)), self._ctx),
                             int(sizes.n_triangles), int(sizes.nodes_per_layout))

    def last_kernel_ms(self) -> float:
        ms = ctypes.c_float()
        _check(lib.rt_last_kernel_ms(self._ctx, ctypes.byref(ms)), self._ctx)
        return float(ms.value)
```

include/rtpt.h:

```cpp
#ifndef RTPT_H
#define RTPT_H

#include "rt_types.h"

#ifdef __cplusplus
extern "C" {
#endif

#define RTPT_ABI_VERSION 11

#define RT_MAX_BOUNCES 4

typedef enum rt_status {
    RT_OK = 0,
    RT_ERR_INVALID_ARG = 1,
    RT_ERR_NO_DEVICE = 2,
    RT_ERR_OUT_OF_MEMORY = 3,
    RT_ERR_LAUNCH = 4,
    RT_ERR_STATE = 5,
    RT_ERR_COMM = 6
} rt_status;

typedef struct rt_ctx rt_ctx;

// ... 229 lines not shown
    uint32_t lanes_per_ray;
    uint64_t seed_key;
    uint32_t flags;
    uint32_t reserved;
} rt_path_params;

void rt_path_params_default(rt_path_params* params);

int rt_trace_paths(rt_ctx* ctx, const rt_path_params* params, const rt_ray* rays, const uint32_t* seeds,
                   uint64_t n, float* radiance, rt_ray_hit* first_hits);

int rt_trace_paths_async(rt_ctx* ctx, const rt_path_params* params, const rt_ray* rays_dev,
                         const uint32_t* seeds_dev, uint64_t n, float* radiance_dev, rt_ray_hit* first_hits_dev,
                         void* hip_stream);

typedef struct rt_ray_domain_info {
    float origin_max, dir_len2_min, dir_len2_max, tmax_max;
} rt_ray_domain_info;
int rt_debug_ray_domain(const rt_scene_desc* scene, rt_ray_domain_info* info);

typedef struct rt_build_stats {
    uint32_t tri_bvh_build;
    uint32_t tri_bvh_nodes;
    float tri_bvh_build_ms;
    float scene_compile_ms;
    uint32_t tri_bvh_temp_kib;
} rt_build_stats;
int rt_build_info(const rt_ctx* ctx, rt_build_stats* info);

typedef struct rt_tri_bvh_dump {
    uint32_t n_triangles;
    uint32_t nodes_per_layout;
    uint32_t leaf_max;
    float margin;
    uint32_t* nodes;
    float* sorted;
    uint32_t* perm;
    float* isect;
} rt_tri_bvh_dump;

int rt_debug_tri_bvh(const rt_ctx* ctx, rt_tri_bvh_dump* dump);

int rt_debug_tri_bvh_host(const rt_scene_desc* scene, const rt_create_options* opt, rt_tri_bvh_dump* dump);

#define RT_UPDATE_REBUILD 0x1u

int rt_update_scene(rt_ctx* ctx, const rt_scene_desc* scene, uint32_t flags);

typedef struct rt_update_stats {
    uint32_t tri_bvh;
    uint32_t updates;
    float compile_ms;
    float upload_ms;
    float tri_bvh_ms;
    float total_ms;
    uint32_t reserved[2];
} rt_update_stats;
int rt_update_info(const rt_ctx* ctx, rt_update_stats* info);

int rt_debug_tri_bvh_refit_host(const rt_scene_desc* built_from, const rt_create_options* opt,
                                const rt_scene_desc* updated, rt_tri_bvh_dump* dump);

int rt_math_selfcheck(uint64_t* mismatches);

typedef enum rt_math_fn {
    RT_MATH_SIN = 0,
    RT_MATH_COS = 1,
    RT_MATH_LOG = 2,
    RT_MATH_EXP = 3,
    RT_MATH_POW_GAMMA = 4,
    RT_MATH_SQRT = 5,
    RT_MATH_RCP = 6,
    RT_MATH_F2H = 7,
    RT_MATH_H2F = 8,
    RT_MATH_TONEMAP = 9,
    RT_MATH_MIS_UNIT = 10,
    RT_MATH_HALTON_LOOP = 11,
    RT_MATH_HALTON_SMALL = 12,
    RT_MATH_HALTON_TAB = 13
} rt_math_fn;
#define RT_MATH_HALTON(form, D) ((uint32_t)(form) | ((uint32_t)(D) << 8))
#define RT_MATH_HOST   0u
#define RT_MATH_DEVICE 1u
#define RT_MATH_VALUES_MAX (1u << 24)

int rt_debug_math_values(uint32_t fn, uint32_t where, const uint32_t* in_bits, uint64_t n, uint32_t* out_bits);

int rt_debug_math_sums(uint32_t fn, uint32_t where, uint32_t first_bits, uint64_t count, uint32_t chunk_log2,
                       uint32_t host_threads, uint64_t* sums);

const char* rt_build_sha(void);

int rt_debug_stats(rt_ctx* ctx, uint64_t* out, int n);

const char* rt_last_error(const rt_ctx* ctx);
const char* rt_status_string(int status);
int rt_abi_version(void);


void rt_seed_splitmix(uint64_t key, uint32_t* seeds, size_t n);

#define RT_CORNELL_TRIANGLES 36
int rt_scene_cornell_box(int32_t width, int32_t height, CameraGPU* camera,
                         MaterialGPU* materials, rt_float3* vertices,
                         SquareLightGPU* light, uint32_t* n_triangles);

#define RT_SPHERE_SCENE_TRIANGLES 12
int rt_scene_random_spheres(int32_t width, int32_t height, uint32_t n_spheres,
                            uint64_t seed, CameraGPU* camera, MaterialGPU* materials,
                            rt_float3* vertices, SquareLightGPU* light,
                            uint32_t* n_triangles, SphereGPU* spheres);

typedef struct rt_mis_params {
    uint32_t camera_rays;
    uint32_t mis_samples;
    uint32_t row_start, row_step, row_count;
    uint32_t flags;
} rt_mis_params;

int rt_render_mis(rt_ctx* ctx, const rt_mis_params* params, float* out_rgba32f,
                  uint8_t* out_rgba8);

int rt_scene_cornell_box_mis(int32_t width, int32_t height, CameraGPU* camera,
                             MaterialGPU* materials, rt_float3* vertices,
                             SquareLightGPU* light, uint32_t* n_triangles);

typedef struct rt_scene_info {
    uint32_t n_triangles;
    uint32_t n_triangle_pairs;
    uint32_t n_spheres;
    uint32_t lds_bytes;
    uint32_t n_sphere_nodes;
    uint32_t n_triangle_bvh_nodes;
    uint32_t n_box_clusters;
    uint32_t pair_free_mask;
    uint32_t sphere_kernel_lds_bytes;
    uint32_t kernel_layout;
    uint32_t kernel_lds_bytes;
} rt_scene_info;
int rt_scene_describe(const rt_scene_desc* scene, rt_scene_info* info);
int rt_scene_describe_ex(const rt_scene_desc* scene, const rt_create_options* opt, rt_scene_info* info);

int rt_debug_camera_candidates(const rt_scene_desc* scene, int32_t x0, int32_t x1, int32_t y0, int32_t y1,
                               uint8_t* may_hit);

int rt_debug_shadow_candidates(const rt_scene_desc* scene, int32_t x0, int32_t x1, int32_t y0, int32_t y1,
                               uint8_t* may_occlude, int32_t* available);

int rt_debug_cluster_kinds(const rt_scene_desc* scene, uint32_t* flags, uint32_t capacity, uint32_t* n_clusters);

int rt_debug_halton_table(float* table, uint32_t capacity, uint32_t* n_floats, uint32_t* offsets, uint32_t* sizes);
int rt_debug_halton_table_device(const rt_ctx* ctx, float* table, uint32_t capacity);

int rt_debug_light_mask(const rt_scene_desc* scene, uint64_t* mask, float* records, uint32_t capacity_triangles);

void rt_tonemap_rgba8(const float* rgba32f, size_t n_pixels, uint8_t* rgba8);

#ifdef __cplusplus
}
#endif

#endif
```

Baseline: 29240 Msamples/s.

## Precompute per-wave camera/shadow candidate masks in a cached table kernel

Moves the per-wave beam and shaft culling that the path-trace kernel computed in its prologue into a separate kernel. That kernel writes one uint4 mask record per wave into a device table. The table is cached across launches, keyed on camera, light, row partition, wave grid and a scene epoch, and event tracking makes sure readers finish before it is refilled. The trace kernel then does a single load per wave instead of the culling work, and the new kernel also handles multiple visible pairs when building the shadow mask (MULTI). The cost is an extra launch whenever the key changes, plus host-side key comparison and event bookkeeping on every render.

```diff
diff --git a/gpuraytracer_amd/_native.py b/gpuraytracer_amd/_native.py
--- a/gpuraytracer_amd/_native.py
+++ b/gpuraytracer_amd/_native.py
@@ -219,6 +219,14 @@
 
 
 assert ctypes.sizeof(PlanParams) == 40 and ctypes.sizeof(PlanStats) == 32
+
+
+class WaveMask(ctypes.Structure):
+    _fields_ = [(n, ctypes.c_uint32) for n in ("cam_mask", "shd_mask", "shd_cskip", "shd_available")] + \
+               [(n, ctypes.c_int32) for n in ("x0", "x1", "y0", "y1")]
+
+
+assert ctypes.sizeof(WaveMask) == 32
 
 
 class MisParamsC(ctypes.Structure):
@@ -323,6 +331,11 @@
                                            ctypes.c_uint32]),
     "rt_debug_halton_table": (ctypes.c_int, [_P, ctypes.c_uint32, ctypes.POINTER(ctypes.c_uint32), _P, _P]),
     "rt_debug_halton_table_device": (ctypes.c_int, [_P, _P, ctypes.c_uint32]),
+    "rt_debug_wave_rects": (ctypes.c_int, [ctypes.c_int32, ctypes.c_int32] + [ctypes.c_uint32] * 4 +
+                            [_P, ctypes.c_uint32, ctypes.POINTER(ctypes.c_uint32), ctypes.POINTER(ctypes.c_uint32)]),
+    "rt_debug_wave_masks": (ctypes.c_int, [_P, ctypes.POINTER(RenderParamsC), ctypes.c_uint32, _P, ctypes.c_uint32,
+                                           ctypes.POINTER(ctypes.c_uint32), ctypes.POINTER(ctypes.c_uint32),
+                                           ctypes.POINTER(ctypes.c_uint64)]),
 }
 
 
diff --git a/gpuraytracer_amd/csrc/rt_api.cpp b/gpuraytracer_amd/csrc/rt_api.cpp
--- a/gpuraytracer_amd/csrc/rt_api.cpp
+++ b/gpuraytracer_amd/csrc/rt_api.cpp
@@ -71,6 +71,20 @@
     kTriIsect, kTriShade, kPairIsect, kClusters, kSphLds, kSphLdsId,
     kSphBox,
     kSphIsect, kSphShade, kSphNodes, kSphPerm, kMisShade, kSceneArrays
+};
+
+struct MaskKey {
+    float cam[14];
+    float light_center[3];
+    int32_t W, H;
+    uint32_t row_start, row_step, row_count;
+    uint32_t L, wave_w, wave_h;
+    uint64_t scene_epoch;
+};
+
+struct MaskReader {
+    hipStream_t stream;
+    hipEvent_t done;
 };
 
 }
@@ -92,6 +106,13 @@
     bool sph_compact = false;
     uint64_t light_mask = 0;
     DevBuf d_halton_tab;
+    DevBuf d_wave_masks;
+    MaskKey mask_key{};
+    bool mask_valid = false;
+    uint64_t scene_epoch = 0;
+    uint64_t mask_fills = 0;
+    Event ev_mask_fill;
+    std::vector<MaskReader> mask_readers;
     uint32_t tri_bvh_build_used = 0;
     uint32_t tri_leaf_max = 1;
     float tri_bvh_build_ms = 0.0f;
@@ -139,6 +160,7 @@
     ~rt_ctx() {
         if (tiles_pending) (void)hipEventSynchronize(ev_tiles);
         if (comm) (void)ncclCommDestroy(comm);
+        for (const MaskReader& r : mask_readers) (void)hipEventDestroy(r.done);
     }
 };
 
@@ -377,13 +399,85 @@
 
 bool resolve_rows(const rt_ctx* c, uint32_t row_start, uint32_t row_step, uint32_t row_count, uint32_t* start,
                   uint32_t* step, uint32_t* count) {
-    const uint32_t H = (uint32_t)c->scene.cam.H;
-    *start = row_start;
-    *step = row_step ? row_step : 1u;
-    if (*start >= H) return false;
-    const uint32_t avail = (H - 1u - *start) / *step + 1u;
-    *count = row_count ? row_count : avail;
-    return *count <= avail;
+    return rtapi::resolve_rows((uint32_t)c->scene.cam.H, row_start, row_step, row_count, start, step, count);
+}
+
+void set_launch(rt::KParams* K, const rt_ctx* c, const rt_render_params* p, uint32_t start, uint32_t step,
+                uint32_t count) {
+    set_camera(K, c->scene.cam);
+    K->spp = p->spp;
+    K->sample_base = p->sample_base;
+    K->row_start = start;
+    K->row_step = step;
+    K->row_count = count;
+    K->lanes = c->lanes;
+    K->walk = c->walk;
+    K->walk_leaf_den = c->walk_leaf_den;
+}
+
+int ensure_wave_masks(rt_ctx* c, rt::KParams* K, const rt::WaveGrid& g, hipStream_t stream) {
+    MaskKey key;
+    memset(&key, 0, sizeof(key));
+    memcpy(key.cam, K->cam_pos, sizeof(K->cam_pos));
+    memcpy(key.cam + 3, K->cam_u, sizeof(K->cam_u));
+    memcpy(key.cam + 6, K->cam_v, sizeof(K->cam_v));
+    memcpy(key.cam + 9, K->cam_w, sizeof(K->cam_w));
+    key.cam[12] = K->halfW;
+    key.cam[13] = K->halfH;
+    memcpy(key.light_center, K->light_center, sizeof(key.light_center));
+    key.W = K->W;
+    key.H = K->H;
+    key.row_start = K->row_start;
+    key.row_step = K->row_step;
+    key.row_count = K->row_count;
+    key.L = g.L;
+    key.wave_w = g.wave_w;
+    key.wave_h = g.wave_h;
+    key.scene_epoch = c->scene_epoch;
+    hipError_t e;
+    if (!c->ev_mask_fill.h && (e = hipEventCreateWithFlags(&c->ev_mask_fill.h, hipEventDisableTiming)) != hipSuccess)
+        return hip_fail(c, RT_ERR_OUT_OF_MEMORY, "hipEventCreate(mask fill)", e);
+    const size_t bytes = (size_t)g.waves_x * g.waves_y * sizeof(rt::WaveMask);
+    if (!c->mask_valid || memcmp(&key, &c->mask_key, sizeof(key)) != 0 || c->d_wave_masks.bytes() < bytes) {
+        c->mask_valid = false;
+        for (const MaskReader& r : c->mask_readers)
+            if ((e = hipStreamWaitEvent(stream, r.done, 0)) != hipSuccess)
+                return hip_fail(c, RT_ERR_LAUNCH, "hipStreamWaitEvent(mask table readers)", e);
+        if ((e = hipStreamWaitEvent(stream, c->ev_mask_fill, 0)) != hipSuccess)
+            return hip_fail(c, RT_ERR_LAUNCH, "hipStreamWaitEvent(mask table fill)", e);
+        for (const MaskReader& r : c->mask_readers) (void)hipEventDestroy(r.done);
+        c->mask_readers.clear();
+        int st;
+        if ((st = reserve(c, c->d_wave_masks, bytes, "hipMalloc(wave masks)")) != RT_OK) return st;
+        if ((e = rt::launch_wave_masks(*K, g, c->d_wave_masks.as<uint4>(), stream)) != hipSuccess)
+            return hip_fail(c, RT_ERR_LAUNCH, "wave_masks launch", e);
+        if ((e = hipEventRecord(c->ev_mask_fill, stream)) != hipSuccess)
+            return hip_fail(c, RT_ERR_LAUNCH, "hipEventRecord(mask fill)", e);
+        c->mask_key = key;
+        c->mask_valid = true;
+        ++c->mask_fills;
+    } else if ((e = hipStreamWaitEvent(stream, c->ev_mask_fill, 0)) != hipSuccess) {
+        return hip_fail(c, RT_ERR_LAUNCH, "hipStreamWaitEvent(mask table fill)", e);
+    }
+    K->wave_masks = c->d_wave_masks.as<uint4>();
+    return RT_OK;
+}
+
+int note_mask_reader(rt_ctx* c, hipStream_t stream) {
+    MaskReader* r = nullptr;
+    for (MaskReader& q : c->mask_readers)
+        if (q.stream == stream) r = &q;
+    hipError_t e;
+    if (!r) {
+        hipEvent_t ev = nullptr;
+        if ((e = hipEventCreateWithFlags(&ev, hipEventDisableTiming)) != hipSuccess)
+            return hip_fail(c, RT_ERR_OUT_OF_MEMORY, "hipEventCreate(mask reader)", e);
+        c->mask_readers.push_back(MaskReader{stream, ev});
+        r = &c->mask_readers.back();
+    }
+    if ((e = hipEventRecord(r->done, stream)) != hipSuccess)
+        return hip_fail(c, RT_ERR_LAUNCH, "hipEventRecord(mask reader)", e);
+    return RT_OK;
 }
 
 struct CountsArgs {
@@ -469,19 +563,15 @@
     K.seeds = c->d_seeds.as<uint32_t>();
     K.sum = sums ? c->d_sum.as<float4>() : nullptr;
     K.out = kout;
-    set_camera(&K, c->scene.cam);
-    K.spp = p->spp;
-    K.sample_base = p->sample_base;
-    K.row_start = start;
-    K.row_step = step;
-    K.row_count = count;
+    set_launch(&K, c, p, start, step, count);
     K.accumulate = p->accumulate ? 1u : 0u;
     K.samples_total = (uint32_t)total;
     K.flags = ((p->flags & RT_OUT_FP16) ? rt::kOutFp16 : 0u) | ((p->flags & RT_OUT_RGBA8) ? rt::kOutRgba8 : 0u);
-    K.lanes = c->lanes;
-    K.walk = c->walk;
-    K.walk_leaf_den = c->walk_leaf_den;
     K.max_index = halton_max_index(c, p->sample_base, ca ? (uint32_t)total : p->spp);
+
+    rt::WaveGrid wg{};
+    const bool masks = !ca && rt::wave_mask_grid(K, p->bounces, c->scene_mem, 0, &wg);
+    if (masks && (st = ensure_wave_masks(c, &K, wg, stream)) != RT_OK) return st;
 
     if (keep_sum && !p->accumulate) c->sum_valid = false;
     if ((st = timed_launch(c, stream, ca ? "path_counts" : "path_trace", &c->launch, [&](rt::LaunchInfo* info) {
@@ -489,6 +579,7 @@
                        : rt::launch_path_trace(K, p->bounces, c->scene_mem, stream, info);
          })) != RT_OK)
         return st;
+    if (masks && (st = note_mask_reader(c, stream)) != RT_OK) return st;
     if (sums) {
         c->sum_valid = true;
         c->sum_row_start = start;
@@ -1110,6 +1201,7 @@
     c->broken = "rt_update_scene in progress";
     c->sum_valid = false;
     c->scene = std::move(next);
+    ++c->scene_epoch;
     const auto t_up = clk::now();
     if ((e = upload_scene(c)) != hipSuccess) return broken(RT_ERR_OUT_OF_MEMORY, std::string("scene upload: ") + hipGetErrorString(e));
     st.upload_ms = ms_since(t_up);
@@ -1404,6 +1496,49 @@
     return e == hipSuccess ? RT_OK : RT_ERR_LAUNCH;
 }
 
+int rt_debug_wave_masks(rt_ctx* c, const rt_render_params* p, uint32_t lanes, rt_wave_mask* masks, uint32_t capacity,
+                        uint32_t* waves_x, uint32_t* waves_y, uint64_t* fills) {
+    static_assert(sizeof(rt_wave_mask) == 32 && sizeof(rt::WaveMask) == 16, "rt_wave_mask / WaveMask layout");
+    if (!c) return fail(nullptr, RT_ERR_INVALID_ARG, "ctx is null");
+    if (!p || !waves_x || !waves_y || (!masks && capacity))
+        return fail(c, RT_ERR_INVALID_ARG, "rt_debug_wave_masks: null argument");
+    if (lanes != 0 && lanes != 1 && lanes != 4 && lanes != 16)
+        return fail(c, RT_ERR_INVALID_ARG, "rt_debug_wave_masks: lanes_per_pixel must be 0, 1, 4 or 16");
+    if (!c->broken.empty()) return fail(c, RT_ERR_STATE, c->broken);
+    if (p->bounces > RT_MAX_BOUNCES) return fail(c, RT_ERR_INVALID_ARG, "bounces > 4");
+    uint32_t start, step, count;
+    if (!resolve_rows(c, p->row_start, p->row_step, p->row_count, &start, &step, &count))
+        return fail(c, RT_ERR_INVALID_ARG, "row partition outside the frame");
+    DeviceGuard g(c->device);
+    rt::KParams K;
+    set_scene(&K, c);
+    set_launch(&K, c, p, start, step, count);
+    K.max_index = halton_max_index(c, p->sample_base, p->spp);
+    *waves_x = *waves_y = 0;
+    if (fills) *fills = c->mask_fills;
+    rt::WaveGrid wg{};
+    if (!rt::wave_mask_grid(K, p->bounces, c->scene_mem, lanes, &wg)) return RT_OK;
+    int st;
+    if ((st = ensure_wave_masks(c, &K, wg, c->stream)) != RT_OK) return st;
+    if (fills) *fills = c->mask_fills;
+    const uint32_t n = wg.waves_x * wg.waves_y;
+    std::vector<rt::WaveMask> host(n);
+    hipError_t e = hipMemcpyAsync(host.data(), c->d_wave_masks.as<void>(), (size_t)n * sizeof(rt::WaveMask),
+                                  hipMemcpyDeviceToHost, c->stream);
+    if (e == hipSuccess) e = hipStreamSynchronize(c->stream);
+    if (e != hipSuccess) return hip_fail(c, RT_ERR_LAUNCH, "rt_debug_wave_masks: read-back", e);
+    *waves_x = wg.waves_x;
+    *waves_y = wg.waves_y;
+    wave_rects(wg, start, step, masks, capacity);
+    for (uint32_t w = 0; w < n && w < capacity; ++w) {
+        masks[w].cam_mask = host[w].cam_mask;
+        masks[w].shd_mask = host[w].shd_mask;
+        masks[w].shd_cskip = host[w].shd_cskip;
+        masks[w].shd_available = host[w].shd_avail;
+    }
+    return RT_OK;
+}
+
 int rt_last_launch(const rt_ctx* c, rt_launch_info* info) {
     if (!c || !info) return fail(nullptr, RT_ERR_INVALID_ARG, "null argument");
     if (!c->launched) return RT_ERR_STATE;
diff --git a/gpuraytracer_amd/csrc/rt_api_host.cpp b/gpuraytracer_amd/csrc/rt_api_host.cpp
--- a/gpuraytracer_amd/csrc/rt_api_host.cpp
+++ b/gpuraytracer_amd/csrc/rt_api_host.cpp
@@ -364,6 +364,23 @@
     return RT_OK;
 }
 
+int rt_debug_wave_rects(int32_t width, int32_t height, uint32_t row_start, uint32_t row_step, uint32_t row_count,
+                        uint32_t lanes, rt_wave_mask* masks, uint32_t capacity, uint32_t* waves_x, uint32_t* waves_y) {
+    static_assert(sizeof(rt_wave_mask) == 32, "rt_wave_mask layout");
+    if (width < 1 || height < 1 || !waves_x || !waves_y || (!masks && capacity))
+        return fail(nullptr, RT_ERR_INVALID_ARG, "rt_debug_wave_rects: empty frame or null argument");
+    if (lanes != 1 && lanes != 4 && lanes != 16)
+        return fail(nullptr, RT_ERR_INVALID_ARG, "rt_debug_wave_rects: lanes_per_pixel must be 1, 4 or 16");
+    uint32_t start, step, count;
+    if (!resolve_rows((uint32_t)height, row_start, row_step, row_count, &start, &step, &count))
+        return fail(nullptr, RT_ERR_INVALID_ARG, "row partition outside the frame");
+    const rt::WaveGrid g = rt::clu_wave_grid((uint32_t)width, count, step, lanes);
+    *waves_x = g.waves_x;
+    *waves_y = g.waves_y;
+    wave_rects(g, start, step, masks, capacity);
+    return RT_OK;
+}
+
 int rt_debug_cluster_kinds(const rt_scene_desc* d, uint32_t* flags, uint32_t capacity, uint32_t* n_clusters) {
     if (!desc_ok(d) || !n_clusters || (!flags && capacity)) return fail(nullptr, RT_ERR_INVALID_ARG, "null argument");
     rt::CompiledScene s;
diff --git a/gpuraytracer_amd/csrc/rt_api_internal.hpp b/gpuraytracer_amd/csrc/rt_api_internal.hpp
--- a/gpuraytracer_amd/csrc/rt_api_internal.hpp
+++ b/gpuraytracer_amd/csrc/rt_api_internal.hpp
@@ -74,6 +74,28 @@
     return L;
 }
 
+inline void wave_rects(const rt::WaveGrid& g, uint32_t row_start, uint32_t row_step, rt_wave_mask* out,
+                       uint32_t capacity) {
+    const uint32_t n = g.waves_x * g.waves_y;
+    for (uint32_t w = 0; w < n && w < capacity; ++w) {
+        const uint32_t wx0 = (w % g.waves_x) * g.wave_w, wj0 = (w / g.waves_x) * g.wave_h;
+        out[w].x0 = (int32_t)wx0;
+        out[w].x1 = (int32_t)(wx0 + g.wave_w - 1u);
+        out[w].y0 = (int32_t)(row_start + wj0 * row_step);
+        out[w].y1 = (int32_t)(row_start + (wj0 + g.wave_h - 1u) * row_step);
+    }
+}
+
+inline bool resolve_rows(uint32_t H, uint32_t row_start, uint32_t row_step, uint32_t row_count, uint32_t* start,
+                         uint32_t* step, uint32_t* count) {
+    *start = row_start;
+    *step = row_step ? row_step : 1u;
+    if (*start >= H) return false;
+    const uint32_t avail = (H - 1u - *start) / *step + 1u;
+    *count = row_count ? row_count : avail;
+    return *count <= avail;
+}
+
 inline const char* plan_params_error(const rt_plan_params* p, uint32_t flags_ok) {
     static_assert(sizeof(rt_plan_params) == 40 && sizeof(rt_plan_stats) == 32 && sizeof(rt::PlanStats) == 32,
                   "rt_plan_params / rt_plan_stats layout");
diff --git a/gpuraytracer_amd/csrc/rt_kernel.hip b/gpuraytracer_amd/csrc/rt_kernel.hip
--- a/gpuraytracer_amd/csrc/rt_kernel.hip
+++ b/gpuraytracer_amd/csrc/rt_kernel.hip
@@ -484,46 +484,6 @@
         x = bx * (WR * kWX) + (wave % WR) * kWX + (pix % kWX);
         j = by * (WC * kWY) + (wave / WR) * kWY + (pix / kWX);
     };
-    if constexpr (RT_CAM_CAND && GEO == kGeoPairClu) {
-        if (sv.nP - 1u < 32u) {
-            const uint32_t wave = wave_uniform(threadIdx.x >> 6);
-            const uint32_t wx0 = bx * (WR * kWX) + (wave % WR) * kWX;
-            const uint32_t wj0 = by * (WC * kWY) + (wave / WR) * kWY;
-            const float y0 = (float)(P.row_start + wj0 * P.row_step);
-            const float y1 = (float)(P.row_start + (wj0 + kWY - 1u) * P.row_step);
-            const Beam beam = make_beam(ld_f3(P.cam_pos), ld_f3(P.cam_u), ld_f3(P.cam_v), ld_f3(P.cam_w), P.halfW,
-                                        P.halfH, (float)P.W, (float)P.H, (float)wx0, (float)(wx0 + kWX - 1u), y0, y1);
-            const uint32_t k = threadIdx.x & 63u;
-            const uint32_t kc = min(k, sv.nP - 1u);
-            const bool keep = !beam_excludes_pair(beam, reinterpret_cast<const float*>(sv.pair + kPairF4 * kc));
-            sv.cam_mask = wave_uniform((uint32_t)__builtin_amdgcn_ballot_w64(k < sv.nP && keep));
-            sv.cam_avail = true;
-            if constexpr (RT_SHD_CAND) {
-                const uint32_t tb = k >> 5, kt = min(k & 31u, sv.nP - 1u);
-                bool occ = false, bad = (sv.cam_mask & (sv.cam_mask - 1u)) != 0u;
-                if (sv.cam_mask != 0u && !bad) {
-                    const uint32_t sp = (uint32_t)__builtin_ctz(sv.cam_mask);
-                    const float4 s0 = P.tri_shade[4 * (2u * sp + tb)];
-                    if (s0.w == 0.0f) {
-                        const ShaftLight lq = shaft_light(ld_f3(P.light_center));
-                        const ShaftSrc src = shaft_source(beam, reinterpret_cast<const float*>(sv.pair + kPairF4 * sp),
-                                                          (int)tb, f3{s0.x, s0.y, s0.z}, lq);
-                        bad = !src.ok;
-                        occ = !shaft_excludes_pair(src, lq, reinterpret_cast<const float*>(sv.pair + kPairF4 * kt));
-                    }
-                }
-                const unsigned long long ob = __builtin_amdgcn_ballot_w64((k & 31u) < sv.nP && occ);
-                sv.shd_mask = wave_uniform((uint32_t)ob | (uint32_t)(ob >> 32));
-                sv.shd_avail = __builtin_amdgcn_ballot_w64(bad) == 0ull && sv.nC <= 32u;
-                if (sv.nC != 0u) {
-                    const uint32_t kc2 = min(k, sv.nC - 1u);
-                    const uint32_t all = __float_as_uint(reinterpret_cast<const float*>(sv.clu + kCluF4 * kc2)[22]);
-                    sv.shd_cskip = wave_uniform(
-                        (uint32_t)__builtin_amdgcn_ballot_w64(k < sv.nC && (all & sv.shd_mask) == 0u));
-                }
-            }
-        }
-    }
     constexpr bool kRemat = GEO == kGeoPairClu || GEO == kGeoSphLds;
     auto opaque_tid = []() {
         uint32_t t = threadIdx.x;
@@ -553,6 +513,20 @@
             lum_s[3 * slot] = lum.x;
             lum_s[3 * slot + 1] = lum.y;
             lum_s[3 * slot + 2] = lum.z;
+        }
+    }
+    if constexpr (RT_CAM_CAND && GEO == kGeoPairClu) {
+        if (sv.nP - 1u < 32u) {
+            const uint32_t wave = wave_uniform(threadIdx.x >> 6);
+            const uint32_t wx = bx * WR + wave % WR, wy = by * WC + wave / WR;
+            const uint4 m = P.wave_masks[wave_uniform(wy * (gridDim.x * WR) + wx)];
+            sv.cam_mask = wave_uniform(m.x);
+            sv.cam_avail = true;
+            if constexpr (RT_SHD_CAND) {
+                sv.shd_mask = wave_uniform(m.y);
+                sv.shd_cskip = wave_uniform(m.z);
+                sv.shd_avail = wave_uniform(m.w) != 0u;
+            }
         }
     }
     const f3 cu = ld_f3(P.cam_u), cv = ld_f3(P.cam_v), cw = ld_f3(P.cam_w);
@@ -821,11 +795,10 @@
 template <int B, int GEO, bool SPH, bool SMALL, int L>
 hipError_t launch_tl(const KParams& P, size_t lds_bytes, hipStream_t stream) {
     KParams Q = P;
-    if (L > 1) Q.wave_w = (P.row_step > 1) ? 64u / L : (L == 4 ? 4u : 2u);
-    constexpr uint32_t WR = waves_per_row(GEO), WC = waves_per_col(GEO);
-    const uint32_t WX = (L == 1) ? 8u : Q.wave_w;
-    const uint32_t TX = WR * WX, TY = WC * ((64u / L) / WX);
-    const dim3 grid((P.W + TX - 1) / TX, (P.row_count + TY - 1) / TY);
+    const WaveGrid g = wave_grid((uint32_t)P.W, P.row_count, P.row_step, (uint32_t)L, waves_per_row(GEO), waves_per_col(GEO));
+    if (L > 1) Q.wave_w = g.wave_w;
+    const dim3 grid(g.grid_x, g.grid_y);
+    if (RT_CAM_CAND && GEO == kGeoPairClu && P.nP - 1u < 32u && !P.wave_masks) return hipErrorInvalidValue;
     if (GEO == kGeoSphLds) {
         const hipError_t e = allow_lds((const void*)path_trace_kernel<B, GEO, SPH, SMALL, L>, lds_bytes);
         if (e != hipSuccess) return e;
@@ -991,6 +964,16 @@
     return e;
 }
 
+bool wave_mask_grid(const KParams& P, uint32_t bounces, SceneMem mem, uint32_t lanes_override, WaveGrid* g) {
+    if (!RT_CAM_CAND || P.nP - 1u >= 32u) return false;
+    if (choose_kernel(tables_of(P), P.sph_lds != nullptr, bounces, mem, P.walk).layout != kGeoPairClu) return false;
+    KParams Q = P;
+    if (lanes_override) Q.lanes = lanes_override;
+    const int L = P.max_index < kSmallIndexMax ? lanes_per_pixel(Q, kGeoPairClu) : 1;
+    *g = clu_wave_grid((uint32_t)P.W, P.row_count, P.row_step, (uint32_t)(L == 16 || L == 4 ? L : 1));
+    return true;
+}
+
 #include "rt_counts.hpp"
 #include "rt_paths.hpp"
 
@@ -1055,4 +1038,57 @@
     return hipGetLastError();
 }
 
-}
+template <bool MULTI>
+__global__ __launch_bounds__(kBlockThreads) void wave_masks_kernel(KParams P, uint4* table, uint32_t waves_x,
+                                                                   uint32_t n_waves, uint32_t kWX, uint32_t kWY) {
+    const uint32_t w = wave_uniform(blockIdx.x * (kBlockThreads / 64u) + (threadIdx.x >> 6));
+    if (w >= n_waves) return;
+    const uint32_t nP = P.nP, nC = P.nC;
+    const float* pair = reinterpret_cast<const float*>(P.pair_isect);
+    const uint32_t wx0 = (w % waves_x) * kWX, wj0 = (w / waves_x) * kWY;
+    const float y0 = (float)(P.row_start + wj0 * P.row_step);
+    const float y1 = (float)(P.row_start + (wj0 + kWY - 1u) * P.row_step);
+    const Beam beam = make_beam(ld_f3(P.cam_pos), ld_f3(P.cam_u), ld_f3(P.cam_v), ld_f3(P.cam_w), P.halfW, P.halfH,
+                                (float)P.W, (float)P.H, (float)wx0, (float)(wx0 + kWX - 1u), y0, y1);
+    const uint32_t k = threadIdx.x & 63u;
+    const uint32_t kc = min(k, nP - 1u);
+    const bool keep = !beam_excludes_pair(beam, pair + 4u * kPairF4 * kc);
+    const uint32_t cam_mask = wave_uniform((uint32_t)__builtin_amdgcn_ballot_w64(k < nP && keep));
+    uint32_t shd_mask = 0u, shd_cskip = 0u;
+    bool shd_avail = false;
+    if constexpr (RT_SHD_CAND) {
+        const uint32_t tb = k >> 5, kt = min(k & 31u, nP - 1u);
+        const ShaftLight lq = shaft_light(ld_f3(P.light_center));
+        bool undecided = !MULTI && (cam_mask & (cam_mask - 1u)) != 0u;
+        for (uint32_t m = undecided ? 0u : cam_mask; m != 0u; m &= m - 1u) {
+            const uint32_t sp = (uint32_t)__builtin_ctz(m);
+            const float4 s0 = P.tri_shade[4 * (2u * sp + tb)];
+            bool occ = false, bad = false;
+            if (s0.w == 0.0f) {
+                const ShaftSrc src = shaft_source(beam, pair + 4u * kPairF4 * sp, (int)tb, f3{s0.x, s0.y, s0.z}, lq);
+                bad = !src.ok;
+                occ = !shaft_excludes_pair(src, lq, pair + 4u * kPairF4 * kt);
+            }
+            const unsigned long long ob = __builtin_amdgcn_ballot_w64((k & 31u) < nP && occ);
+            shd_mask |= wave_uniform((uint32_t)ob | (uint32_t)(ob >> 32));
+            undecided = undecided || __builtin_amdgcn_ballot_w64(bad) != 0ull;
+        }
+        shd_avail = !undecided && nC <= 32u;
+        if (nC != 0u) {
+            const uint32_t kc2 = min(k, nC - 1u);
+            const uint32_t all = __float_as_uint(reinterpret_cast<const float*>(P.clusters + kCluF4 * kc2)[22]);
+            shd_cskip = wave_uniform((uint32_t)__builtin_amdgcn_ballot_w64(k < nC && (all & shd_mask) == 0u));
+        }
+    }
+    if (k == 0u) table[w] = make_uint4(cam_mask, shd_mask, shd_cskip, shd_avail ? 1u : 0u);
+}
+
+hipError_t launch_wave_masks(const KParams& P, const WaveGrid& g, uint4* table, hipStream_t stream) {
+    const uint32_t n = g.waves_x * g.waves_y, per_block = kBlockThreads / 64u;
+    if (n == 0) return hipSuccess;
+    hipLaunchKernelGGL(wave_masks_kernel<RT_WAVE_MASK_MULTI != 0>, dim3((n + per_block - 1) / per_block), dim3(kBlockThreads), 0, stream, P, table,
+                       g.waves_x, n, g.wave_w, g.wave_h);
+    return hipGetLastError();
+}
+
+}
diff --git a/gpuraytracer_amd/csrc/rt_kernel.hpp b/gpuraytracer_amd/csrc/rt_kernel.hpp
--- a/gpuraytracer_amd/csrc/rt_kernel.hpp
+++ b/gpuraytracer_amd/csrc/rt_kernel.hpp
@@ -95,7 +95,29 @@
     uint32_t pair_free;
     uint64_t light_mask;
     const float* halton_tab;
-};
+    const uint4* wave_masks;
+};
+
+struct WaveMask {
+    uint32_t cam_mask, shd_mask, shd_cskip, shd_avail;
+};
+static_assert(sizeof(WaveMask) == sizeof(uint4), "one dwordx4 load per wave");
+#ifndef RT_WAVE_MASK_MULTI
+#define RT_WAVE_MASK_MULTI 1
+#endif
+struct WaveGrid {
+    uint32_t L, wave_w, wave_h, grid_x, grid_y, waves_x, waves_y;
+};
+constexpr WaveGrid wave_grid(uint32_t W, uint32_t row_count, uint32_t row_step, uint32_t L, uint32_t WR,
+                             uint32_t WC) {
+    const uint32_t ww = L == 1 ? 8u : (row_step > 1 ? 64u / L : (L == 4 ? 4u : 2u));
+    const uint32_t wh = (64u / L) / ww;
+    const uint32_t gx = (W + WR * ww - 1) / (WR * ww), gy = (row_count + WC * wh - 1) / (WC * wh);
+    return WaveGrid{L, ww, wh, gx, gy, gx * WR, gy * WC};
+}
+constexpr WaveGrid clu_wave_grid(uint32_t W, uint32_t row_count, uint32_t row_step, uint32_t L) {
+    return wave_grid(W, row_count, row_step, L, 2u, 2u);
+}
 
 size_t kernel_lds_bytes(uint32_t n_tri, uint32_t n_pairs, uint32_t n_sph, uint32_t n_nodes);
 
@@ -150,6 +172,8 @@
 hipError_t launch_path_trace(const KParams& P, uint32_t bounces, SceneMem mem, hipStream_t stream,
                              LaunchInfo* info);
 KernelChoice choose_kernel(const SceneTables& t, bool sph_compact, uint32_t bounces, SceneMem mem, uint32_t walk);
+bool wave_mask_grid(const KParams& P, uint32_t bounces, SceneMem mem, uint32_t lanes_override, WaveGrid* g);
+hipError_t launch_wave_masks(const KParams& P, const WaveGrid& g, uint4* table, hipStream_t stream);
 hipError_t launch_path_counts(const KParams& P, const uint32_t* counts, uint32_t* totals, uint32_t bounces,
                               SceneMem mem, hipStream_t stream, LaunchInfo* info);
 hipError_t read_debug_stats(unsigned long long* out, int n);
diff --git a/gpuraytracer_amd/host.py b/gpuraytracer_amd/host.py
--- a/gpuraytracer_amd/host.py
+++ b/gpuraytracer_amd/host.py
@@ -10,7 +10,7 @@
                       RT_OUT_NONE, RT_OUT_RGBA8, RT_RAYS_ANY, RT_RAYS_EXACT, RT_UPDATE_REBUILD, TRI_BUILDS, WALKS,
                       AovBuffers, AovParams, BuildStats, CameraGPU, CreateOptions, DenoiseBuffers, DenoiseParams, LaunchInfo, MaterialGPU, MisParamsC, RayDomainInfo,
                       PathParamsC, PlanParams, PlanStats, RT_PLAN_RELATIVE, RenderParamsC,
-                      RtError, SceneDesc, SceneInfo, SphereGPU, SquareLightGPU, TileLayout, TriBvhDump, UpdateStats, float3,
+                      RtError, SceneDesc, SceneInfo, SphereGPU, SquareLightGPU, TileLayout, TriBvhDump, UpdateStats, WaveMask, float3,
                       lib)
 
 DEFAULT_SEED_KEY = 0x5EED00000000
@@ -35,6 +35,26 @@
     lib.rt_tonemap_rgba8(a.ctypes.data_as(ctypes.c_void_p), n,
                          out.ctypes.data_as(ctypes.c_void_p))
     return out
+
+
+WAVE_MASK_DTYPE = np.dtype([(n, np.uint32) for n in ("cam_mask", "shd_mask", "shd_cskip", "shd_available")] +
+                           [(n, np.int32) for n in ("x0", "x1", "y0", "y1")])
+assert WAVE_MASK_DTYPE.itemsize == ctypes.sizeof(WaveMask)
+
+
+def _wave_records(call) -> np.ndarray:
+    wx, wy = ctypes.c_uint32(), ctypes.c_uint32()
+    call(None, 0, wx, wy)
+    out = np.zeros((wy.value, wx.value), dtype=WAVE_MASK_DTYPE)
+    if out.size:
+        call(out.ctypes.data_as(ctypes.c_void_p), out.size, wx, wy)
+    return out
+
+
+def wave_rects(width: int, height: int, lanes: int, row_start: int = 0, row_step: int = 1,
+               row_count: int = 0) -> np.ndarray:
+    return _wave_records(lambda p, cap, wx, wy: _check(lib.rt_debug_wave_rects(
+        width, height, row_start, row_step, row_count, lanes, p, cap, ctypes.byref(wx), ctypes.byref(wy))))
 
 
 def _math_fn(fn: str, dim: int, where: str) -> tuple[int, int]:
@@ -903,6 +923,14 @@
         _check(lib.rt_last_launch(self._ctx, ctypes.byref(info)), self._ctx)
         return info.as_dict()
 
+    def wave_masks(self, params: RenderParams | None = None, lanes: int = 0):
+        p = (params or RenderParams()).c()
+        fills = ctypes.c_uint64()
+        rec = _wave_records(lambda ptr, cap, wx, wy: _check(lib.rt_debug_wave_masks(
+            self._ctx, ctypes.byref(p), lanes, ptr, cap, ctypes.byref(wx), ctypes.byref(wy), ctypes.byref(fills)),
+            self._ctx))
+        return rec, int(fills.value)
+
     def build_info(self) -> dict:
         b = BuildStats()
         _check(lib.rt_build_info(self._ctx, ctypes.byref(b)), self._ctx)
diff --git a/include/rtpt.h b/include/rtpt.h
--- a/include/rtpt.h
+++ b/include/rtpt.h
@@ -405,6 +405,19 @@
 int rt_debug_halton_table(float* table, uint32_t capacity, uint32_t* n_floats, uint32_t* offsets, uint32_t* sizes);
 int rt_debug_halton_table_device(const rt_ctx* ctx, float* table, uint32_t capacity);
 
+typedef struct rt_wave_mask {
+    uint32_t cam_mask;
+    uint32_t shd_mask;
+    uint32_t shd_cskip;
+    uint32_t shd_available;
+    int32_t x0, x1, y0, y1;
+} rt_wave_mask;
+int rt_debug_wave_rects(int32_t width, int32_t height, uint32_t row_start, uint32_t row_step, uint32_t row_count,
+                        uint32_t lanes_per_pixel, rt_wave_mask* masks, uint32_t capacity, uint32_t* waves_x,
+                        uint32_t* waves_y);
+int rt_debug_wave_masks(rt_ctx* ctx, const rt_render_params* params, uint32_t lanes_per_pixel, rt_wave_mask* masks,
+                        uint32_t capacity, uint32_t* waves_x, uint32_t* waves_y, uint64_t* fills);
+
 int rt_debug_light_mask(const rt_scene_desc* scene, uint64_t* mask, float* records, uint32_t capacity_triangles);
 
 void rt_tonemap_rgba8(const float* rgba32f, size_t n_pixels, uint8_t* rgba8);
```

After: 29980 Msamples/s (median of 6 runs). 1.03x the previous value.
